# SitaoLuan/ACM-GNN

Hardware: AMD Instinct MI355X
Metric: edges/sec ACM-GCN fwd+bwd on twitch-gamer (higher is better)
Workload: dtype f32; 1 GPU; twitch-gamer-shaped Chung-Lu graph: 168114 nodes, 6797557 undirected edges, nnz(A_low)=13763228, F_in=7, hidden=64, classes=2; 2-layer acmgcnp (variant=0, structure_info=0, attention LayerNorm on), dropout 0.1 (counter-based, masks regenerated in the kernels), AdamW (fused); step = fwd + NLL loss + bwd + optimizer update; parallelism=single-gpu, node_order=degree, launch=hipGraph replay of the captured step (1 consecutive steps per graph), operator_form=pattern-only P + row scale (shared by A_low and A_low^T), full=False, input_pipeline=True, checked=False

## Files before the change

### acm_gnn_amd/_lib.py

```python
import ctypes as C
import os
import threading

from . import build as _build

c_f32p = C.POINTER(C.c_float)
c_i32p = C.POINTER(C.c_int32)

ACM_OK = 0
STATUS_NAMES = {1: "ACM_EINVAL", 2: "ACM_ESHAPE", 3: "ACM_EHIP", 4: "ACM_EUNSUPPORTED", 5: "ACM_ENOMEM"}
ABI_VERSION = 29

EXPORTED_SYMBOLS = (
    "acm_version", "acm_last_error", "acm_tuning_get", "acm_tuning_set", "acm_csr_create", "acm_csr_transpose", "acm_csr_slice_rows",
    "acm_csr_destroy", "acm_csr_info", "acm_csr_build_streams", "acm_csr_build_item_streams", "acm_spmm_workspace_bytes", "acm_gemm_workspace_bytes",
    "acm_gemm", "acm_gemm_blocks", "acm_gemm_drop", "acm_proj3", "acm_gemm_split", "acm_proj_fwd", "acm_proj_fwd_at", "acm_proj_bwd_workspace_bytes", "acm_proj_bwd", "acm_spmm", "acm_spmm_v", "acm_spmm_ex", "acm_cast_bf16", "acm_conv_fwd", "acm_conv_bwd_local_workspace_bytes",
    "acm_conv_bwd_local", "acm_conv_bwd_spmm", "acm_conv_agg_fwd", "acm_conv_agg_bwd_workspace_bytes",
    "acm_conv_agg_bwd", "acm_nll_loss_workspace_bytes", "acm_nll_loss", "acm_adam_step", "acm_dropout",
    "acm_reduce_flush", "acm_conv_fwd_tail_workspace_bytes", "acm_conv_fwd_tail", "acm_shard_plan",
    "acm_conv_acmii_fwd_workspace_bytes", "acm_conv_acmii_fwd", "acm_linear_fwd", "acm_bias_act", "acm_bias_act_bwd_workspace_bytes", "acm_bias_act_bwd",
    "acm_acmii_table_bytes", "acm_acmii_table", "acm_conv_acmii_v_fwd", "acm_conv_acmii_v_bwd_workspace_bytes", "acm_conv_acmii_v_bwd",
    "acm_linear_bwd_workspace_bytes", "acm_linear_bwd", "acm_linear_fwd_add", "acm_linear_bwd_recompute",
    "acm_small_step_workspace_bytes", "acm_small_step", "acm_small_step_has_hidden", "acm_conv_head_fwd", "acm_conv_aggw_fwd", "acm_conv_aggw_bwd_workspace_bytes", "acm_conv_aggw_bwd",
    "acm_eval_metrics_workspace_bytes", "acm_eval_metrics",
    "acm_bce_loss_workspace_bytes", "acm_bce_loss", "acm_rocauc_scores", "acm_rocauc_workspace_bytes", "acm_rocauc",
    "acm_homophily_workspace_bytes", "acm_homophily_census", "acm_class_means_workspace_bytes", "acm_class_means", "acm_class_score",
    "acm_synth_regular", "acm_synth_uniform", "acm_synth_random_plan", "acm_synth_draw", "acm_synth_select_workspace_bytes", "acm_synth_select",
    "acm_synth_inter_count", "acm_synth_emit",
    "acm_gcn_fwd", "acm_gcn_bwd_workspace_bytes", "acm_gcn_bwd", "acm_gemm_act",
    "acm_select_step", "acm_copy_if",
    "acm_small_batch_table_bytes", "acm_small_batch_bind", "acm_small_batch_step", "acm_eval_metrics_batch", "acm_select_step_batch",
    "acm_bnorm_stats_workspace_bytes", "acm_bnorm_stats", "acm_bnorm_fold", "acm_bnorm_param_bwd", "acm_bnorm_bwd_workspace_bytes", "acm_bnorm_bwd",
    "acm_proj_blocks_fwd", "acm_proj_blocks_bwd_workspace_bytes", "acm_proj_blocks_bwd",
    "acm_csr_build_loss_rows", "acm_csr_loss_rows_info", "acm_conv_fwd_tail_rows",
)
LOSS_ROWS_SYMBOLS = ("acm_csr_build_loss_rows", "acm_csr_loss_rows_info", "acm_conv_fwd_tail_rows")


class Dropout(C.Structure):
    _fields_ = [("p", C.c_float), ("tag", C.c_int32), ("seed", C.c_uint64), ("step", C.c_void_p),
                ("row_offset", C.c_int64), ("step_offset", C.c_int64)]


class CsrInfo(C.Structure):
    _fields_ = [("n_rows", C.c_int64), ("n_cols", C.c_int64), ("nnz", C.c_int64),
                ("n_items", C.c_int64), ("n_long_rows", C.c_int64), ("n_partial_slots", C.c_int64),
                ("chunk", C.c_int32), ("max_degree", C.c_int32),
                ("indptr", C.c_void_p), ("indices", C.c_void_p), ("vals", C.c_void_p),
                ("src_pos", C.c_void_p),
                ("stream_steps", C.c_int64), ("stream_slices", C.c_int64),
                ("stream_waves", C.c_int32), ("stream_long_rows", C.c_int32),
                ("item_stream_waves", C.c_int32), ("reserved", C.c_int32), ("item_stream_batches", C.c_int64)]


class ConvFwd(C.Structure):
    _fields_ = [("f_out", C.c_int32), ("n_channels", C.c_int32), ("relu_after", C.c_int32),
                ("relu_mlp", C.c_int32), ("layernorm", C.c_int32), ("scale", C.c_float),
                ("row_offset", C.c_int64),
                ("g_low", C.c_void_p), ("ld_g_low", C.c_int64),
                ("g_high", C.c_void_p), ("ld_g_high", C.c_int64),
                ("g_struc", C.c_void_p), ("ld_g_struc", C.c_int64),
                ("s_high", C.c_void_p), ("ld_s_high", C.c_int64),
                ("s_mlp", C.c_void_p), ("ld_s_mlp", C.c_int64),
                ("s_struc", C.c_void_p), ("ld_s_struc", C.c_int64),
                ("deg", C.c_void_p),
                ("att_vec", C.c_void_p * 4), ("ln_weight", C.c_void_p * 4), ("ln_bias", C.c_void_p * 4),
                ("att_mix", C.c_void_p),
                ("out", C.c_void_p), ("ld_out", C.c_int64),
                ("pre", C.c_void_p), ("ld_pre", C.c_int64),
                ("att", C.c_void_p), ("post_scale", C.c_void_p), ("ld_post_scale", C.c_int64), ("post_relu", C.c_int32),
                ("gather_bf16", C.c_int32), ("row_scale", C.c_void_p), ("post_drop", Dropout)]


class ConvBwdLocal(C.Structure):
    _fields_ = [("f_out", C.c_int32), ("n_channels", C.c_int32), ("relu_after", C.c_int32),
                ("relu_mlp", C.c_int32), ("layernorm", C.c_int32), ("scale", C.c_float),
                ("grad_out", C.c_void_p), ("ld_grad_out", C.c_int64),
                ("pre", C.c_void_p), ("ld_pre", C.c_int64),
                ("s_mlp", C.c_void_p), ("ld_s_mlp", C.c_int64),
                ("deg", C.c_void_p),
                ("att_vec", C.c_void_p * 4), ("ln_weight", C.c_void_p * 4), ("ln_bias", C.c_void_p * 4),
                ("att_mix", C.c_void_p),
                ("g_low", C.c_void_p), ("ld_g_low", C.c_int64),
                ("g_high", C.c_void_p), ("ld_g_high", C.c_int64),
                ("g_mlp", C.c_void_p), ("ld_g_mlp", C.c_int64),
                ("g_struc", C.c_void_p), ("ld_g_struc", C.c_int64),
                ("d_att_vec", C.c_void_p * 4), ("d_ln_weight", C.c_void_p * 4),
                ("d_ln_bias", C.c_void_p * 4), ("d_att_mix", C.c_void_p),
                ("post_scale", C.c_void_p), ("ld_post_scale", C.c_int64), ("post_relu", C.c_int32),
                ("g_scale", C.c_void_p), ("post_drop", Dropout), ("defer", C.c_void_p)]


class ConvBwdSpmm(C.Structure):
    _fields_ = [("f_out", C.c_int32), ("row_offset", C.c_int64),
                ("g_low", C.c_void_p), ("ld_g_low", C.c_int64),
                ("g_high", C.c_void_p), ("ld_g_high", C.c_int64),
                ("g_struc", C.c_void_p), ("ld_g_struc", C.c_int64),
                ("s_high", C.c_void_p), ("ld_s_high", C.c_int64),
                ("s_struc", C.c_void_p), ("ld_s_struc", C.c_int64),
                ("inv_deg", C.c_void_p),
                ("mask_low", C.c_void_p), ("ld_mask_low", C.c_int64),
                ("mask_high", C.c_void_p), ("ld_mask_high", C.c_int64),
                ("dz_low", C.c_void_p), ("ld_dz_low", C.c_int64),
                ("dz_high", C.c_void_p), ("ld_dz_high", C.c_int64),
                ("d_struc", C.c_void_p), ("ld_d_struc", C.c_int64), ("self_scale", C.c_void_p),
                ("gather_bf16", C.c_int32)]


class ConvAggFwd(C.Structure):
    _fields_ = [("f_in", C.c_int32), ("f_pad", C.c_int32), ("f_out", C.c_int32), ("relu_after", C.c_int32),
                ("relu_mlp", C.c_int32), ("layernorm", C.c_int32), ("scale", C.c_float),
                ("xg", C.c_void_p), ("ld_xg", C.c_int64),
                ("xs", C.c_void_p), ("ld_xs", C.c_int64),
                ("w_low", C.c_void_p), ("w_high", C.c_void_p), ("w_mlp", C.c_void_p), ("ld_w", C.c_int64),
                ("att_vec", C.c_void_p * 4), ("ln_weight", C.c_void_p * 4), ("ln_bias", C.c_void_p * 4),
                ("att_mix", C.c_void_p),
                ("out", C.c_void_p), ("ld_out", C.c_int64),
                ("agg", C.c_void_p), ("ld_agg", C.c_int64),
                ("att", C.c_void_p), ("post_scale", C.c_void_p), ("ld_post_scale", C.c_int64), ("post_relu", C.c_int32),
                ("n_channels", C.c_int32), ("sg", C.c_void_p), ("ld_sg", C.c_int64), ("sg_bf16", C.c_int32),
                ("ss", C.c_void_p), ("ld_ss", C.c_int64), ("deg", C.c_void_p),
                ("ps", C.c_void_p), ("ld_ps", C.c_int64), ("row_scale", C.c_void_p), ("post_drop", Dropout),
                ("head_stats", C.c_void_p), ("ld_head_stats", C.c_int64),
                ("next_w_low", C.c_void_p), ("next_w_high", C.c_void_p), ("next_w_mlp", C.c_void_p), ("next_ld_w", C.c_int64),
                ("next_f", C.c_int32), ("next_relu", C.c_int32),
                ("next_zlh", C.c_void_p), ("ld_next_zlh", C.c_int64), ("next_zi", C.c_void_p), ("ld_next_zi", C.c_int64),
                ("agg_given", C.c_int32), ("reserved0", C.c_int32),
                ("agg_copy", C.c_void_p), ("ld_agg_copy", C.c_int64), ("xs_copy", C.c_void_p), ("ld_xs_copy", C.c_int64),
                ("next_x", C.c_void_p), ("ld_next_x", C.c_int64), ("next_drop", Dropout)]


class ConvAggBwd(C.Structure):
    _fields_ = [("f_in", C.c_int32), ("f_pad", C.c_int32), ("f_out", C.c_int32), ("relu_after", C.c_int32),
                ("relu_mlp", C.c_int32), ("layernorm", C.c_int32), ("scale", C.c_float),
                ("grad_out", C.c_void_p), ("ld_grad_out", C.c_int64),
                ("agg", C.c_void_p), ("ld_agg", C.c_int64),
                ("xs", C.c_void_p), ("ld_xs", C.c_int64),
                ("w_low", C.c_void_p), ("w_high", C.c_void_p), ("w_mlp", C.c_void_p), ("ld_w", C.c_int64),
                ("att_vec", C.c_void_p * 4), ("ln_weight", C.c_void_p * 4), ("ln_bias", C.c_void_p * 4),
                ("att_mix", C.c_void_p),
                ("d_params", C.c_void_p), ("post_scale", C.c_void_p), ("ld_post_scale", C.c_int64), ("post_relu", C.c_int32),
                ("n_channels", C.c_int32), ("ps", C.c_void_p), ("ld_ps", C.c_int64),
                ("ss", C.c_void_p), ("ld_ss", C.c_int64), ("deg", C.c_void_p),
                ("g_struc", C.c_void_p), ("ld_g_struc", C.c_int64), ("g_struc_scale", C.c_void_p),
                ("post_drop", Dropout), ("defer", C.c_void_p),
                ("head_stats", C.c_void_p), ("ld_head_stats", C.c_int64),
                ("out", C.c_void_p), ("ld_out", C.c_int64),
                ("next_a", C.c_void_p), ("next_xg", C.c_void_p), ("ld_next_xg", C.c_int64),
                ("next_row_scale", C.c_void_p), ("next_agg", C.c_void_p), ("ld_next_agg", C.c_int64),
                ("proj_dz", C.c_void_p), ("ld_proj_dz", C.c_int64),
                ("proj_w_low", C.c_void_p), ("proj_w_high", C.c_void_p), ("proj_w_mlp", C.c_void_p), ("proj_ld_w", C.c_int64),
                ("proj_f", C.c_int32), ("proj_d_w", C.c_void_p)]


class ConvAcmiiFwd(C.Structure):
    _fields_ = [("f_in", C.c_int32), ("f_pad", C.c_int32), ("f_out", C.c_int32), ("layernorm", C.c_int32),
                ("scale", C.c_float),
                ("xg", C.c_void_p), ("ld_xg", C.c_int64), ("xs", C.c_void_p), ("ld_xs", C.c_int64),
                ("w_low", C.c_void_p), ("w_high", C.c_void_p), ("w_mlp", C.c_void_p), ("ld_w", C.c_int64),
                ("att_vec", C.c_void_p * 4), ("ln_weight", C.c_void_p * 4), ("ln_bias", C.c_void_p * 4),
                ("att_mix", C.c_void_p),
                ("out", C.c_void_p), ("ld_out", C.c_int64), ("pre", C.c_void_p), ("ld_pre", C.c_int64),
                ("att", C.c_void_p), ("zlh", C.c_void_p), ("ld_zlh", C.c_int64), ("zi", C.c_void_p), ("ld_zi", C.c_int64),
                ("post_scale", C.c_void_p), ("ld_post_scale", C.c_int64), ("post_relu", C.c_int32),
                ("row_scale", C.c_void_p), ("post_drop", Dropout),
                ("n_channels", C.c_int32), ("ps", C.c_void_p), ("ld_ps", C.c_int64), ("ss", C.c_void_p), ("ld_ss", C.c_int64),
                ("deg", C.c_void_p)]


class ConvAcmiiBwd(C.Structure):
    _fields_ = [("f_in", C.c_int32), ("table", C.c_void_p),
                ("g_low", C.c_void_p), ("ld_g_low", C.c_int64), ("g_high", C.c_void_p), ("ld_g_high", C.c_int64),
                ("g_mlp", C.c_void_p), ("ld_g_mlp", C.c_int64), ("x", C.c_void_p), ("ld_x", C.c_int64),
                ("self_offset", C.c_int64), ("row_scale", C.c_void_p),
                ("d_w_low", C.c_void_p), ("d_w_high", C.c_void_p), ("d_w_mlp", C.c_void_p), ("ld_dw", C.c_int64),
                ("defer", C.c_void_p)]


class Loss(C.Structure):
    _fields_ = [("n_classes", C.c_int32), ("labels", C.c_void_p), ("row_weight", C.c_void_p),
                ("loss", C.c_void_p), ("dlogits", C.c_void_p), ("ld_dlogits", C.c_int64)]


class ReduceSeg(C.Structure):
    _fields_ = [("partial", C.c_void_p), ("nblk", C.c_int32), ("row_stride", C.c_int32),
                ("q0", C.c_int32), ("len", C.c_int32), ("dst", C.c_void_p),
                ("inner", C.c_int32), ("col_block", C.c_int32),
                ("outer_stride", C.c_int64), ("block_stride", C.c_int64),
                ("elem_stride", C.c_int32), ("reserved", C.c_int32)]


class ReduceList(C.Structure):
    _fields_ = [("n", C.c_int32), ("cap", C.c_int32), ("segs", C.POINTER(ReduceSeg))]


PROJ_BLOCKS_MAX = 8


class ProjBlocks(C.Structure):
    _fields_ = [("n_blocks", C.c_int32), ("f", C.c_int32), ("f_block", C.c_int32), ("f_in", C.c_int32),
                ("w_low", C.c_void_p), ("w_high", C.c_void_p), ("w_mlp", C.c_void_p), ("ldw", C.c_int64),
                ("h", C.c_void_p * PROJ_BLOCKS_MAX), ("ld_h", C.c_int64 * PROJ_BLOCKS_MAX),
                ("width", C.c_int32 * PROJ_BLOCKS_MAX), ("row0", C.c_int32 * PROJ_BLOCKS_MAX),
                ("d_h", C.c_void_p * PROJ_BLOCKS_MAX), ("ld_dh", C.c_int64 * PROJ_BLOCKS_MAX)]


class SpmmOpts(C.Structure):
    _fields_ = [("vals", C.c_void_p), ("row_scale", C.c_void_p), ("sub", C.c_void_p), ("ld_sub", C.c_int64),
                ("sub_scale", C.c_void_p), ("relu", C.c_int32), ("g_bf16", C.c_int32)]


class GcnFwd(C.Structure):
    _fields_ = [("width", C.c_int32), ("relu", C.c_int32), ("z", C.c_void_p), ("ld_z", C.c_int64), ("y", C.c_void_p), ("ld_y", C.c_int64),
                ("row_scale", C.c_void_p), ("drop", Dropout), ("f_next", C.c_int32), ("reserved", C.c_int32),
                ("w_next", C.c_void_p), ("ld_w_next", C.c_int64), ("z_next", C.c_void_p), ("ld_z_next", C.c_int64)]


class GcnBwd(C.Structure):
    _fields_ = [("width", C.c_int32), ("hidden", C.c_int32), ("dy", C.c_void_p), ("ld_dy", C.c_int64), ("h", C.c_void_p), ("ld_h", C.c_int64),
                ("w2", C.c_void_p), ("ld_w2", C.c_int64), ("keep_scale", C.c_float), ("relu", C.c_int32),
                ("g", C.c_void_p), ("ld_g", C.c_int64), ("dz", C.c_void_p), ("ld_dz", C.c_int64),
                ("d_w2", C.c_void_p), ("ld_dw2", C.c_int64), ("defer", C.c_void_p)]


class AdamTensor(C.Structure):
    _fields_ = [("param", C.c_void_p), ("grad", C.c_void_p), ("exp_avg", C.c_void_p), ("exp_avg_sq", C.c_void_p),
                ("step", C.c_void_p), ("numel", C.c_int64)]


class AdamConfig(C.Structure):
    _fields_ = [("lr", C.c_double), ("beta1", C.c_double), ("beta2", C.c_double), ("eps", C.c_double),
                ("weight_decay", C.c_double), ("decoupled", C.c_int32), ("also_advance", C.c_void_p),
                ("arrive", C.c_void_p), ("pending", C.c_void_p)]


class Select(C.Structure):
    _fields_ = [("rule", C.c_int32), ("early_stopping", C.c_int32), ("epochs", C.c_int32), ("reserved", C.c_int32),
                ("result", C.c_void_p), ("result_f64", C.c_void_p), ("train_loss", C.c_void_p),
                ("ctrl", C.c_void_p), ("best", C.c_void_p), ("history", C.c_void_p)]


class EvalMetricsSlot(C.Structure):
    _fields_ = [("logits", C.c_void_p), ("weights", C.c_void_p), ("labels", C.c_void_p), ("out", C.c_void_p),
                ("workspace", C.c_void_p)]


class CopyTensor(C.Structure):
    _fields_ = [("src", C.c_void_p), ("dst", C.c_void_p), ("numel", C.c_int64)]


SMALL_ROLES = 17
SR_W_LOW, SR_W_HIGH, SR_W_MLP, SR_V_LOW, SR_V_HIGH, SR_V_MLP, SR_V_STRUC = range(7)
SR_LNW_LOW, SR_LNW_HIGH, SR_LNW_MLP, SR_LNW_STRUC, SR_LNB_LOW, SR_LNB_HIGH, SR_LNB_MLP, SR_LNB_STRUC, SR_MIX, SR_STRUC = range(7, 17)


class SmallStep(C.Structure):
    _fields_ = [("n_classes", C.c_int32), ("n_channels", C.c_int32), ("relu_before", C.c_int32), ("layernorm", C.c_int32),
                ("scale", C.c_float), ("train", C.c_int32), ("update", C.c_int32), ("hidden", C.c_int32),
                ("t", (AdamTensor * SMALL_ROLES) * 2),
                ("x_vals", C.c_void_p), ("xt_src_pos", C.c_void_p), ("xt_vals", C.c_void_p), ("f_in", C.c_int32), ("reserved1", C.c_int32), ("drop_in", Dropout), ("drop_hidden", Dropout),
                ("row_scale", C.c_void_p), ("labels", C.c_void_p), ("row_weight", C.c_void_p), ("loss", C.c_void_p),
                ("logits", C.c_void_p), ("att1", C.c_void_p), ("att2", C.c_void_p),
                ("lr", C.c_double), ("beta1", C.c_double), ("beta2", C.c_double), ("eps", C.c_double),
                ("weight_decay", C.c_double), ("decoupled", C.c_int32), ("also_advance", C.c_void_p), ("arrive", C.c_void_p),
                ("workspace", C.c_void_p), ("workspace_bytes", C.c_size_t)]


SMALL_BATCH_MAX = 32

_lib = None
_lock = threading.Lock()


def _declare(lib):
    vp, i64, i32, sz = C.c_void_p, C.c_int64, C.c_int, C.c_size_t
    lib.acm_version.restype = C.c_int
    lib.acm_version.argtypes = []
    lib.acm_last_error.restype = C.c_char_p
    lib.acm_last_error.argtypes = []
    lib.acm_csr_create.argtypes = [i64, i64, i64, vp, vp, vp, i32, C.POINTER(vp)]
    lib.acm_csr_transpose.argtypes = [vp, i32, C.POINTER(vp)]
    lib.acm_csr_slice_rows.argtypes = [vp, i64, i64, i32, C.POINTER(vp)]
    lib.acm_csr_destroy.argtypes = [vp]
    lib.acm_csr_destroy.restype = None
    lib.acm_csr_info.argtypes = [vp, C.POINTER(CsrInfo)]
    lib.acm_csr_build_streams.argtypes = [vp, i32, i32]
    lib.acm_csr_build_item_streams.argtypes = [vp, i32]
    lib.acm_shard_plan.argtypes = [i64, vp, i32, i64, vp]
    lib.acm_conv_acmii_fwd_workspace_bytes.argtypes = [vp, C.POINTER(sz)]
    lib.acm_conv_acmii_fwd.argtypes = [vp, C.POINTER(ConvAcmiiFwd), vp, sz, vp]
    lib.acm_acmii_table_bytes.argtypes = [i64, C.POINTER(sz)]
    lib.acm_acmii_table.argtypes = [i64, i32, vp, i64, vp, vp, i64, vp, sz, vp]
    lib.acm_conv_acmii_v_fwd.argtypes = [vp, C.POINTER(ConvAcmiiFwd), vp, vp, sz, vp]
    lib.acm_conv_acmii_v_bwd_workspace_bytes.argtypes = [vp, C.POINTER(sz)]
    lib.acm_conv_acmii_v_bwd.argtypes = [vp, C.POINTER(ConvAcmiiBwd), vp, sz, vp]
    lib.acm_linear_fwd.argtypes = [i64, i64, i64, vp, i64, vp, i64, vp, i32, vp, vp, i64, vp, sz, vp]
    lib.acm_bias_act.argtypes = [i64, i32, vp, i64, vp, i32, vp, vp]
    lib.acm_linear_bwd_workspace_bytes.argtypes = [i64, i32, i32, C.POINTER(sz)]
    lib.acm_linear_bwd.argtypes = [i64, i32, i32, vp, i64, vp, i64, vp, i64, C.c_float, i32, vp, i64, vp, vp, sz, vp, vp]
    lib.acm_linear_fwd_add.argtypes = [i64, i32, i32, vp, i64, vp, i64, vp, i32, vp, vp, i64, vp, i64, vp]
    lib.acm_linear_bwd_recompute.argtypes = [i64, i32, i32, vp, i64, vp, i64, vp, i32, vp, vp, i64, vp, i64, vp, vp, sz, vp, vp]
    lib.acm_bias_act_bwd_workspace_bytes.argtypes = [i64, i32, C.POINTER(sz)]
    lib.acm_bias_act_bwd.argtypes = [i64, i32, vp, i64, vp, i64, C.c_float, i32, vp, i64, vp, vp, sz, vp, vp]
    lib.acm_spmm_workspace_bytes.argtypes = [vp, i32, C.POINTER(sz)]
    lib.acm_gemm_workspace_bytes.argtypes = [i32, i32, i64, i64, i64, C.POINTER(sz)]
    lib.acm_gemm.argtypes = [i32, i32, i64, i64, i64, vp, i64, vp, i64, vp, i64, i32, vp, sz, vp]
    lib.acm_proj_bwd_workspace_bytes.argtypes = [i64, i64, i32, C.POINTER(sz)]
    lib.acm_proj_fwd.argtypes = [i64, i64, i32, vp, i64, vp, vp, vp, i64, i32, vp, i64, vp, i64, vp]
    lib.acm_proj_fwd_at.argtypes = [i64, i64, i32, vp, i64, vp, vp, vp, i64, i32, vp, i64, i64, vp, i64, vp]
    lib.acm_proj_bwd.argtypes = [i64, i64, i32, vp, i64, vp, i64, vp, vp, vp, i64, vp, i64, vp, i64, i64, i64, vp, sz, vp, vp]
    lib.acm_proj_blocks_fwd.argtypes = [i64, C.POINTER(ProjBlocks), vp, i64, i32, i32, vp]
    lib.acm_proj_blocks_bwd_workspace_bytes.argtypes = [i64, C.POINTER(ProjBlocks), C.POINTER(sz)]
    lib.acm_proj_blocks_bwd.argtypes = [i64, C.POINTER(ProjBlocks), vp, i64, vp, i64, i64, i64, vp, sz, vp, vp]
    lib.acm_gemm_split.argtypes = [i32, i32, i64, i64, i64, vp, i64, vp, i64, vp, i64, i64, vp, i64, i32, vp, sz, vp]
    lib.acm_gemm_blocks.argtypes = [i32, i32, i64, i64, i64, vp, i64, vp, i64, vp, i64, i64, i64, i32, vp, sz, vp]
    lib.acm_gemm_drop.argtypes = [i32, i32, i64, i64, i64, vp, i64, vp, i64, vp, i64, i64, i64, i32, C.POINTER(Dropout), vp, sz, vp]
    lib.acm_proj3.argtypes = [i64, i64, vp, i64, vp, vp, vp, i64, i64, i64, vp, i64, i64, vp, i64, i32, C.POINTER(Dropout), vp]
    lib.acm_spmm.argtypes = [vp, vp, i64, i32, vp, i64, vp, sz, vp]
    lib.acm_spmm_v.argtypes = [vp, vp, vp, i64, i32, vp, i64, i32, vp, sz, vp]
    lib.acm_adam_step.argtypes = [i32, vp, vp, vp]
    lib.acm_dropout.argtypes = [i64, i64, vp, i64, vp, i64, i64, vp, vp]
    lib.acm_spmm_ex.argtypes = [vp, vp, i64, i32, vp, i64, vp, vp, sz, vp]
    lib.acm_cast_bf16.argtypes = [i64, i64, vp, i64, vp, i64, vp]
    lib.acm_conv_fwd.argtypes = [vp, C.POINTER(ConvFwd), vp, sz, vp]
    lib.acm_conv_head_fwd.argtypes = [i64, C.POINTER(ConvFwd), vp]
    lib.acm_conv_aggw_bwd_workspace_bytes.argtypes = [i64, i64, C.POINTER(C.c_size_t)]
    lib.acm_conv_aggw_bwd.argtypes = [i64, i64, i64, vp, i64, vp, i64, C.POINTER(ConvBwdLocal), vp, vp, vp, i64, vp, C.c_size_t, vp]
    lib.acm_conv_aggw_fwd.argtypes = [i64, i64, i64, vp, i64, vp, i64, vp, vp, vp, i64, vp, i64, C.POINTER(ConvFwd), vp]
    lib.acm_conv_bwd_local_workspace_bytes.argtypes = [i64, i32, i32, C.POINTER(sz)]
    lib.acm_conv_bwd_local.argtypes = [i64, C.POINTER(ConvBwdLocal), vp, sz, vp]
    lib.acm_conv_bwd_spmm.argtypes = [vp, C.POINTER(ConvBwdSpmm), vp, sz, vp]
    lib.acm_conv_agg_fwd.argtypes = [vp, C.POINTER(ConvAggFwd), vp, sz, vp]
    lib.acm_conv_agg_bwd_workspace_bytes.argtypes = [i64, i32, i32, C.POINTER(sz)]
    lib.acm_conv_agg_bwd.argtypes = [i64, C.POINTER(ConvAggBwd), vp, sz, vp]
    lib.acm_nll_loss_workspace_bytes.argtypes = [i64, C.POINTER(sz)]
    lib.acm_nll_loss.argtypes = [i64, i32, vp, i64, vp, vp, vp, vp, i64, vp, sz, vp, vp]
    lib.acm_eval_metrics_workspace_bytes.argtypes = [i64, i32, C.POINTER(sz)]
    lib.acm_eval_metrics.argtypes = [i64, i32, vp, i64, vp, vp, i64, i32, i32, vp, vp, sz, vp]
    lib.acm_bce_loss_workspace_bytes.argtypes = [i64, C.POINTER(sz)]
    lib.acm_bce_loss.argtypes = [i64, i32, vp, i64, vp, vp, vp, vp, i64, vp, sz, vp, vp]
    lib.acm_rocauc_scores.argtypes = [i64, i32, vp, i64, vp, vp]
    lib.acm_rocauc_workspace_bytes.argtypes = [i64, i32, C.POINTER(sz)]
    lib.acm_rocauc.argtypes = [i64, vp, vp, vp, vp, i64, i32, vp, vp, vp, sz, vp]
    lib.acm_homophily_workspace_bytes.argtypes = [i64, i64, i32, C.POINTER(sz)]
    lib.acm_homophily_census.argtypes = [vp, vp, i64, i32, vp, vp, vp, vp, vp, sz, vp]
    lib.acm_class_means_workspace_bytes.argtypes = [i64, i32, i32, C.POINTER(sz)]
    lib.acm_class_means.argtypes = [i64, i32, i32, vp, i64, vp, vp, i64, vp, vp, sz, vp]
    lib.acm_class_score.argtypes = [i64, i32, i32, vp, i64, vp, i64, vp, vp, vp, vp, vp]
    u64 = C.c_uint64
    lib.acm_synth_regular.argtypes = [i32, i64, i64, i64, u64, u64, i64, i64, vp, vp]
    lib.acm_synth_uniform.argtypes = [i64, i64, u64, u64, i64, vp, i64, vp]
    lib.acm_synth_random_plan.argtypes = [i32, i64, i64, C.c_double, C.POINTER(C.c_int64)]
    lib.acm_synth_draw.argtypes = [i32, i64, i64, i32, i32, u64, u64, i64, vp, vp]
    lib.acm_synth_select_workspace_bytes.argtypes = [i32, i64, C.POINTER(sz)]
    lib.acm_synth_select.argtypes = [i32, i64, vp, vp, vp, vp, i64, vp, vp, vp, vp, sz, vp]
    lib.acm_synth_inter_count.argtypes = [i32, i32, C.c_double, vp, vp, vp]
    lib.acm_synth_emit.argtypes = [i32, i32, i64, i32, i32, vp, vp, i64, vp, vp, vp]
    lib.acm_gcn_fwd.argtypes = [vp, C.POINTER(GcnFwd), vp, sz, vp]
    lib.acm_gcn_bwd_workspace_bytes.argtypes = [vp, i32, i32, C.POINTER(sz)]
    lib.acm_gcn_bwd.argtypes = [vp, C.POINTER(GcnBwd), vp, sz, vp]
    lib.acm_gemm_act.argtypes = [i64, i64, i64, vp, i64, vp, i64, i32, vp, vp, i64, vp, sz, vp]
    lib.acm_select_step.argtypes = [C.POINTER(Select), vp]
    lib.acm_copy_if.argtypes = [i32, vp, vp, vp]
    lib.acm_bnorm_stats_workspace_bytes.argtypes = [i64, i32, C.POINTER(sz)]
    lib.acm_bnorm_stats.argtypes = [i64, i32, vp, i64, vp, vp, C.c_float, C.c_float, i32, vp, vp, vp, vp, vp, sz, vp]
    lib.acm_bnorm_fold.argtypes = [i32, i32, vp, i64, vp, vp, vp, i64, vp, vp]
    lib.acm_bnorm_param_bwd.argtypes = [i32, i32, vp, i64, vp, vp, i64, vp, vp, i64, vp, vp, vp]
    lib.acm_bnorm_bwd_workspace_bytes.argtypes = [i64, i32, C.POINTER(sz)]
    lib.acm_bnorm_bwd.argtypes = [i64, i32, vp, i64, vp, i64, vp, vp, vp, C.c_float, i32, vp, i64, vp, vp, sz, vp, vp]
    lib.acm_reduce_flush.argtypes = [vp, vp]
    lib.acm_conv_fwd_tail_workspace_bytes.argtypes = [i64, i32, i32, C.POINTER(sz)]
    lib.acm_conv_fwd_tail.argtypes = [vp, C.POINTER(ConvFwd), C.POINTER(Loss), C.POINTER(ConvBwdLocal), vp, sz, vp, sz, vp]
    lib.acm_csr_build_loss_rows.argtypes = [vp, vp]
    lib.acm_csr_loss_rows_info.argtypes = [vp, C.POINTER(C.c_int64)]
    lib.acm_conv_fwd_tail_rows.argtypes = lib.acm_conv_fwd_tail.argtypes
    lib.acm_small_step_workspace_bytes.argtypes = [vp, vp, vp, C.POINTER(sz)]
    lib.acm_small_step.argtypes = [vp, vp, vp, C.POINTER(SmallStep), vp]
    lib.acm_small_step_has_hidden.argtypes = [i32]
    lib.acm_small_batch_table_bytes.argtypes = [i32, C.POINTER(sz)]
    lib.acm_small_batch_bind.argtypes = [vp, vp, vp, i32, C.POINTER(C.POINTER(SmallStep)), vp, sz, vp]
    lib.acm_small_batch_step.argtypes = [vp, vp, vp, i32, C.POINTER(SmallStep), vp, vp]
    lib.acm_eval_metrics_batch.argtypes = [i64, i32, i64, i64, i32, i32, i32, vp, sz, vp]
    lib.acm_select_step_batch.argtypes = [i32, vp, vp]
    for name in EXPORTED_SYMBOLS:
        fn = getattr(lib, name)
        if name not in ("acm_version", "acm_last_error", "acm_csr_destroy"):
            fn.restype = C.c_int


def library_path():
    return os.environ.get("ACM_HIP_LIBRARY", _build.LIB_PATH)


def load(build_if_missing=True):
    global _lib
    with _lock:
        if _lib is not None:
            return _lib
        path = library_path()
        if "ACM_HIP_LIBRARY" not in os.environ and build_if_missing:
            try:
                if _build.is_stale():
                    _build.build_library()
            except Exception as exc:
                if not os.path.exists(path):
                    raise RuntimeError(f"libacm_hip.so is not built and cannot be built here: {exc}")
        if not os.path.exists(path):
            raise RuntimeError(f"libacm_hip.so not found at {path}; run `python -m acm_gnn_amd.build`")
        lib = C.CDLL(path)
        _declare(lib)
        ver = lib.acm_version()
        if ver != ABI_VERSION:
            raise RuntimeError(f"libacm_hip.so ABI version {ver} != expected {ABI_VERSION}")
        _lib = lib
        return _lib


def check(status, what=""):
    if status != ACM_OK:
        msg = load().acm_last_error().decode(errors="replace")
        raise RuntimeError(f"{what or 'libacm_hip'} failed with {STATUS_NAMES.get(status, status)}: {msg}")
```

### acm_gnn_amd/csrc/acm_common.h

```cpp
#pragma once

#include <hip/hip_runtime.h>
#include <math.h>
#include <stdint.h>

#include "acm_dispatch.h"
#include "acm_hip.h"
#include "acm_items.h"

#define ACM_WAVE 64
#define ACM_NXCD 8
#define ACM_MIN_CHUNK 128
#define ACM_MAX_CHUNK 1024
#define ACM_GROUPS_IN_FLIGHT 8192
#define ACM_LN_EPS 1e-5f

void acm_set_error(const char* fmt, ...);
const acm_tuning_t& acm_tuning();
#define ACM_ROWS16_EPI 1
#define ACM_ROWS16_BWD 2
#define ACM_ROWS16_LOCAL 4
#define ACM_GEMM_ROWS 1
#define ACM_GEMM_BX3 2
#define ACM_GEMM_BX3_WIDE 4
#define ACM_GEMM_ROWS_ALWAYS 8

#define ACM_CHECK_HIP(expr)                                                            \
    do {                                                                               \
        hipError_t e__ = (expr);                                                       \
        if (e__ != hipSuccess) {                                                       \
            acm_set_error("%s -> %s (%s:%d)", #expr, hipGetErrorString(e__), __FILE__, \
                          __LINE__);                                                   \
            return ACM_EHIP;                                                           \
        }                                                                              \
    } while (0)

#define ACM_REQUIRE(cond, code, ...)    \
    do {                                \
        if (!(cond)) {                  \
            acm_set_error(__VA_ARGS__); \
            return (code);              \
        }                               \
    } while (0)

#define ACM_STREAM_SENTINEL 0x07FFFFFF
#define ACM_STREAM_PAD_STEPS 8
struct AcmStreams {
    int32_t* ids;
    int32_t* waves;
    int32_t* items;
    AcmLongRow* long_rows;
    int32_t* long_index;
    int32_t* counters;
    float* slots;
    int64_t total_steps, n_slices, n_long, n_slots;
    int32_t n_waves, lmax;
};

#define ACM_ITEM_STREAM_PAD 8
struct AcmItemStreams {
    int32_t* ids;
    int32_t* quads;
    int32_t* waves;
    int64_t total_batches, n_quads;
    int32_t n_waves;
};

struct AcmLossRows {
    AcmItem* items;
    AcmLongRow* long_rows;
    int32_t* long_index;
    int64_t n_items, n_long, n_slots, n_windows, n_multi;
    uint8_t* keep;
    int64_t kept_rows, kept_edges;
};

struct acm_csr {
    int64_t n_rows, n_cols, nnz;
    int32_t chunk, max_degree;
    int32_t* indptr;
    int32_t* indices;
    float* vals;
    int32_t* src_pos;
    AcmItem* items;
    int64_t n_items;
    AcmLongRow* long_rows;
    int32_t* long_index;
    int64_t n_long;
    int64_t n_slots;
    int64_t n_windows;
    int64_t n_multi;
    AcmStreams* streams;
    AcmItemStreams* item_streams;
    AcmLossRows* loss_rows;
    int device;
};

struct StreamView {
    const int32_t* ids;
    const int32_t* waves;
    const int32_t* items;
    const AcmLongRow* long_rows;
    const int32_t* long_index;
    int32_t* counters;
    float* slots;
    unsigned ids_bytes, slots_bytes;
    int n_waves;
};

struct CsrView {
    const AcmItem* items;
    int n_items;
    const AcmLongRow* long_rows;
    const int32_t* long_index;
    int n_long;
    int n_windows;
    int n_multi;
    const int32_t* indices;
    const float* vals;
};

struct GatherOverride {
    CsrView view;
    int64_t n_slots;
};

int acm_reduce_emit(acm_reduce_list_t* defer, const acm_reduce_seg_t* segs, int n, hipStream_t st);
int acm_reduce_check_segment(const acm_reduce_seg_t& sg, int index);

int acm_spmm_internal(const acm_csr* a, const void* G, int64_t ldg, int width, float* Y, int64_t ldy,
                      const acm_spmm_opts_t* o, void* workspace, size_t workspace_bytes, acm_stream_t stream,
                      bool* defer_fixup);
int acm_bwd_local_reduce(const acm_conv_bwd_local_t* p, const float* partial, int nblk, hipStream_t st);
int acm_bwd_local16(const acm_conv_bwd_local_t* p, int64_t n_rows, float* partial, int max_blocks, hipStream_t s);
int acm_agg_epi16(const acm_conv_agg_fwd_t* p, int64_t n_rows, bool* next_done, hipStream_t s);
struct GatherRole;
int acm_agg_bwd16(const acm_conv_agg_bwd_t* p, int64_t n_rows, float* partial, int max_blocks, hipStream_t s, const GatherRole* gr,
                  int gather_blocks);
int acm_acmii_fixup_launch(const acm_csr_t* a, const acm_conv_acmii_fwd_t* p, const float* partial, hipStream_t s);
bool acm_gemm_rows_nn_ok(int64_t M, int64_t N, int64_t K, const float* B, int64_t ldb);
int acm_gemm_rows_nn(int64_t M, int64_t N, int64_t K, const float* A, int64_t lda, const float* B, int64_t ldb, float* C,
                     int64_t ldc, int relu, const acm_dropout_t* drop, hipStream_t st);
bool acm_gemm_rows_tn_ok(int64_t n_rows, int64_t K, int64_t N);
int acm_gemm_rows_tn_blocks(int64_t n_rows);
int acm_gemm_rows_tn(int64_t n_rows, int64_t K, int64_t N, const float* X, int64_t ldx, const float* Dz, int64_t lddz,
                     float* slabs, int blocks, const acm_dropout_t* drop, hipStream_t st);
bool acm_gemm_bx3_nn_ok(int64_t M, int64_t N, int64_t K, const float* A, int64_t lda);
int acm_gemm_bx3_nn(int64_t M, int64_t N, int64_t K, const float* A, int64_t lda, const float* B, int64_t ldb, float* C,
                    int64_t ldc, int relu, const acm_dropout_t* drop, hipStream_t st);
bool acm_gemm_bx3_tn_ok(int64_t n_rows, int64_t K, int64_t N);
int acm_gemm_bx3_tn_blocks(int64_t n_rows, int64_t K);
int acm_gemm_bx3_tn(int64_t n_rows, int64_t K, int64_t N, const float* X, int64_t ldx, const float* Dz, int64_t lddz,
                    float* slabs, int blocks, const acm_dropout_t* drop, hipStream_t st);
int acm_linear_fwd_narrow(int64_t n_rows, int64_t f_in, int64_t f_out, const float* X, int64_t ldx, const float* W, int64_t ldw,
                          const float* bias, int relu, const acm_dropout_t* drop, float* Y, int64_t ldy, hipStream_t s,
                          const float* add, int64_t ld_add);

static inline CsrView acm_view(const acm_csr* a) {
    CsrView v;
    v.items = a->items;
    v.n_items = (int)a->n_items;
    v.long_rows = a->long_rows;
    v.long_index = a->long_index;
    v.n_long = (int)a->n_long;
    v.n_windows = (int)a->n_windows;
    v.n_multi = (int)a->n_multi;
    v.indices = a->indices;
    v.vals = a->vals;
    return v;
}

#ifdef __HIPCC__
template <int CTRL>
__device__ __forceinline__ float acm_dpp(float v) {
    return __int_as_float(__builtin_amdgcn_update_dpp(0, __float_as_int(v), CTRL, 0xf, 0xf, false));
}
typedef unsigned acm_u32x2 __attribute__((ext_vector_type(2)));
template <int W>
__device__ __forceinline__ float acm_group_sum(float v) {
    static_assert(W == 1 || W == 2 || W == 4 || W == 8 || W == 16 || W == 32 || W == 64, "group width");
    if (W >= 2) v += acm_dpp<0xB1>(v);
    if (W >= 4) v += acm_dpp<0x4E>(v);
    if (W >= 8) v += acm_dpp<0x141>(v);
    if (W >= 16) v += acm_dpp<0x140>(v);
    if (W >= 32) {
        const acm_u32x2 r = __builtin_amdgcn_permlane16_swap(__float_as_uint(v), __float_as_uint(v), false, false);
        v = __uint_as_float(r[0]) + __uint_as_float(r[1]);
    }
    if (W >= 64) {
        const acm_u32x2 r = __builtin_amdgcn_permlane32_swap(__float_as_uint(v), __float_as_uint(v), false, false);
        v = __uint_as_float(r[0]) + __uint_as_float(r[1]);
    }
    return v;
}

__device__ __forceinline__ float acm_cross_row_sum(float v) {
    acm_u32x2 r = __builtin_amdgcn_permlane16_swap(__float_as_uint(v), __float_as_uint(v), false, false);
    v = __uint_as_float(r[0]) + __uint_as_float(r[1]);
    r = __builtin_amdgcn_permlane32_swap(__float_as_uint(v), __float_as_uint(v), false, false);
    return __uint_as_float(r[0]) + __uint_as_float(r[1]);
}

__device__ __forceinline__ int acm_row_bcast(int v, int u) {
#define ACM_BC(U) case U: return __builtin_amdgcn_update_dpp(0, v, 0x150 + U, 0xf, 0xf, false)
    switch (u & 15) {
        ACM_BC(0); ACM_BC(1); ACM_BC(2); ACM_BC(3); ACM_BC(4); ACM_BC(5); ACM_BC(6); ACM_BC(7);
        ACM_BC(8); ACM_BC(9); ACM_BC(10); ACM_BC(11); ACM_BC(12); ACM_BC(13); ACM_BC(14);
        default: return __builtin_amdgcn_update_dpp(0, v, 0x15F, 0xf, 0xf, false);
    }
#undef ACM_BC
}

__device__ __forceinline__ int acm_uniform(int v) { return __builtin_amdgcn_readfirstlane(v); }
__device__ __forceinline__ float acm_lane_f(float v, int lane) {
    return __int_as_float(__builtin_amdgcn_readlane(__float_as_int(v), lane));
}

__device__ __forceinline__ float acm_nll_row(int C, const float* zi, int yi, float wi, float* di) {
    if (wi == 0.f) {
        for (int c = 0; c < C; ++c) di[c] = 0.f;
        return 0.f;
    }
    float m = -INFINITY;
    for (int c = 0; c < C; ++c) m = fmaxf(m, zi[c]);
    float s = 0.f;
    for (int c = 0; c < C; ++c) s += expf(zi[c] - m);
    const float lse = m + logf(s);
    const float inv = 1.0f / s;
    const float zy = zi[yi];
    for (int c = 0; c < C; ++c) di[c] = wi * (expf(zi[c] - m) * inv - (c == yi ? 1.f : 0.f));
    return wi * (lse - zy);
}

__device__ __forceinline__ float acm_bce_row(int C, const float* zi, int64_t yi, float wi, float* di) {
    if (wi == 0.f) {
        if (di)
            for (int c = 0; c < C; ++c) di[c] = 0.f;
        return 0.f;
    }
    const float s = wi / (float)C;
    float acc = 0.f;
    for (int c = 0; c < C; ++c) {
        const float z = zi[c];
        const bool hit = (int64_t)c == yi;
        const float e = expf(-fabsf(z));
        acc += fmaxf(z, 0.f) - (hit ? z : 0.f) + log1pf(e);
        if (di) {
            const float r = 1.0f / (1.0f + e);
            const float sig = z >= 0.f ? r : e * r;
            di[c] = s * (sig - (hit ? 1.f : 0.f));
        }
    }
    return s * acc;
}

struct AcmDropCtx {
    unsigned k0, k1, c2, c3, thresh, tag16;
    float inv_keep;
    long row_offset;
    bool on;
};

__device__ __forceinline__ AcmDropCtx acm_drop_ctx(const acm_dropout_t& d) {
    AcmDropCtx c;
    c.on = d.p > 0.f;
    const unsigned long long step = c.on ? (unsigned long long)(d.step[0] + d.step_offset) : 0ull;
    c.k0 = (unsigned)d.seed;
    c.k1 = (unsigned)(d.seed >> 32);
    c.c2 = (unsigned)step;
    c.c3 = (unsigned)(step >> 32);
    const double t = (double)d.p * 4294967296.0;
    c.thresh = t >= 4294967295.0 ? 0xFFFFFFFFu : (unsigned)t;
    c.tag16 = ((unsigned)d.tag) << 16;
    c.inv_keep = 1.0f / (1.0f - d.p);
    c.row_offset = (long)d.row_offset;
    return c;
}

__device__ __forceinline__ void acm_philox7(const AcmDropCtx& c, long row, int block, unsigned (&w)[4]) {
    unsigned x0 = (unsigned)(row + c.row_offset), x1 = (unsigned)block | c.tag16, x2 = c.c2, x3 = c.c3;
    unsigned k0 = c.k0, k1 = c.k1;
#pragma unroll
    for (int r = 0; r < 7; ++r) {
        const unsigned long long q0 = (unsigned long long)0xD2511F53u * x0, q1 = (unsigned long long)0xCD9E8D57u * x2;
        const unsigned hi0 = (unsigned)(q0 >> 32), lo0 = (unsigned)q0;
        const unsigned hi1 = (unsigned)(q1 >> 32), lo1 = (unsigned)q1;
        x0 = hi1 ^ x1 ^ k0;
        x1 = lo1;
        x2 = hi0 ^ x3 ^ k1;
        x3 = lo0;
        k0 += 0x9E3779B9u;
        k1 += 0xBB67AE85u;
    }
    w[0] = x0, w[1] = x1, w[2] = x2, w[3] = x3;
}

__device__ __forceinline__ float acm_drop1(const AcmDropCtx& c, long row, int col) {
    if (!c.on) return 1.f;
    unsigned w[4];
    acm_philox7(c, row, (col & 15) + 16 * (col >> 6), w);
    const int q = (col >> 4) & 3;
    const unsigned v = q == 0 ? w[0] : (q == 1 ? w[1] : (q == 2 ? w[2] : w[3]));
    return v >= c.thresh ? c.inv_keep : 0.f;
}

__device__ __forceinline__ void acm_drop4(const AcmDropCtx& c, long row, int m, float (&f)[4]) {
    if (!c.on) {
        f[0] = f[1] = f[2] = f[3] = 1.f;
        return;
    }
    unsigned w[4];
    acm_philox7(c, row, m, w);
#pragma unroll
    for (int i = 0; i < 4; ++i) f[i] = w[i] >= c.thresh ? c.inv_keep : 0.f;
}

#endif
```

### acm_gnn_amd/csrc/acm_csr.cpp

```cpp
#include <stdarg.h>
#include <stdio.h>
#include <string.h>

#include <stdlib.h>

#include <algorithm>
#include <functional>
#include <new>
#include <queue>
#include <string>
#include <utility>
#include <vector>

#include "acm_common.h"

static thread_local char g_err[512] = "";

void acm_set_error(const char* fmt, ...) {
    va_list ap;
    va_start(ap, fmt);
    vsnprintf(g_err, sizeof(g_err), fmt, ap);
    va_end(ap);
}

extern "C" int acm_version(void) { return ACM_ABI_VERSION; }
extern "C" const char* acm_last_error(void) { return g_err; }

namespace {
const acm_tuning_t kTuningDefaults = {0, 0, -1, 7, 1, 7, {0}};
struct TuningField { const char* name; int32_t acm_tuning_t::*field; };
const TuningField kTuningFields[] = {{"chunk", &acm_tuning_t::chunk},           {"wide_form", &acm_tuning_t::wide_form},
                                     {"bwd_split", &acm_tuning_t::bwd_split},   {"rows16", &acm_tuning_t::rows16},
                                     {"agg_fused", &acm_tuning_t::agg_fused},   {"gemm_forms", &acm_tuning_t::gemm_forms}};
const char* const kHostKeys[] = {"rewrites", "implicit", "relabel", "pipeline", "csr_features", "small_step", "mlp_stack", "loss_rows"};

const char* tuning_invalid(const acm_tuning_t& t) {
    if (t.chunk != 0 && (t.chunk < 8 || t.chunk > 4096 || (t.chunk & (t.chunk - 1)))) return "chunk";
    if (t.wide_form < 0 || t.wide_form > 3) return "wide_form";
    if (t.bwd_split < -1 || t.bwd_split > 1) return "bwd_split";
    if (t.rows16 < 0 || t.rows16 > 7) return "rows16";
    if (t.agg_fused < 0 || t.agg_fused > 1) return "agg_fused";
    if (t.gemm_forms < 0 || t.gemm_forms > 15) return "gemm_forms";
    return nullptr;
}

acm_tuning_t tuning_from_environment() {
    acm_tuning_t t = kTuningDefaults;
    const char* env = getenv("ACM_TUNING");
    if (!env) return t;
    std::string text(env);
    size_t pos = 0;
    while (pos < text.size()) {
        size_t end = text.find(',', pos);
        if (end == std::string::npos) end = text.size();
        const std::string item = text.substr(pos, end - pos);
        pos = end + 1;
        if (item.empty()) continue;
        const size_t eq = item.find('=');
        const std::string key = item.substr(0, eq), val = eq == std::string::npos ? "" : item.substr(eq + 1);
        bool known = false;
        for (const char* h : kHostKeys) known = known || key == h;
        for (const TuningField& f : kTuningFields) {
            if (key != f.name) continue;
            known = true;
            char* stop = nullptr;
            const long v = strtol(val.c_str(), &stop, 0);
            acm_tuning_t probe = t;
            probe.*(f.field) = (int32_t)v;
            if (val.empty() || *stop || tuning_invalid(probe)) fprintf(stderr, "libacm_hip: ACM_TUNING: bad value '%s' ignored\n", item.c_str());
            else t = probe;
        }
        if (!known) fprintf(stderr, "libacm_hip: ACM_TUNING: unknown key '%s' ignored\n", key.c_str());
    }
    return t;
}
const acm_tuning_t g_tuning_loaded = tuning_from_environment();
acm_tuning_t g_tuning = g_tuning_loaded;
}

const acm_tuning_t& acm_tuning() { return g_tuning; }

extern "C" int acm_tuning_get(acm_tuning_t* out) {
    ACM_REQUIRE(out, ACM_EINVAL, "acm_tuning_get: NULL argument");
    *out = g_tuning;
    return ACM_OK;
}

extern "C" int acm_tuning_set(const acm_tuning_t* in) {
    if (!in) {
        g_tuning = g_tuning_loaded;
        return ACM_OK;
    }
    const char* bad = tuning_invalid(*in);
    ACM_REQUIRE(!bad, ACM_EINVAL, "acm_tuning_set: field '%s' out of range", bad);
    g_tuning = *in;
    for (int32_t& r : g_tuning.reserved) r = 0;
    return ACM_OK;
}

namespace {

void free_streams(AcmStreams* t) {
    if (!t) return;
    for (void* q : {(void*)t->ids, (void*)t->waves, (void*)t->items, (void*)t->long_rows,
                    (void*)t->long_index, (void*)t->counters, (void*)t->slots})
        if (q) (void)hipFree(q);
    delete t;
}

void free_item_streams(AcmItemStreams* t) {
    if (!t) return;
    for (void* q : {(void*)t->ids, (void*)t->quads, (void*)t->waves})
        if (q) (void)hipFree(q);
    delete t;
}

void free_loss_rows(AcmLossRows* t) {
    if (!t) return;
    for (void* q : {(void*)t->items, (void*)t->long_rows, (void*)t->long_index, (void*)t->keep})
        if (q) (void)hipFree(q);
    delete t;
}

void free_handle(acm_csr* a) {
    if (!a) return;
    free_loss_rows(a->loss_rows);
    if (a->indptr) (void)hipFree(a->indptr);
    if (a->indices) (void)hipFree(a->indices);
    if (a->vals) (void)hipFree(a->vals);
    if (a->long_index) (void)hipFree(a->long_index);
    if (a->src_pos) (void)hipFree(a->src_pos);
    if (a->items) (void)hipFree(a->items);
    if (a->long_rows) (void)hipFree(a->long_rows);
    free_streams(a->streams);
    free_item_streams(a->item_streams);
    delete a;
}


int finish_handle(acm_csr* a, const std::vector<int32_t>& h_indptr, int chunk) {
    const int env_chunk = acm_tuning().chunk;
    int auto_chunk = ACM_MIN_CHUNK;
    while (auto_chunk < ACM_MAX_CHUNK && 2 * (int64_t)auto_chunk <= a->nnz / ACM_GROUPS_IN_FLIGHT) auto_chunk *= 2;
    a->chunk = chunk > 0 ? chunk : (env_chunk > 0 ? env_chunk : auto_chunk);
    std::vector<AcmItem> items;
    std::vector<AcmLongRow> longs;
    build_items(h_indptr, a->chunk, items, longs, a->n_slots, a->max_degree, a->n_windows, a->n_multi);
    a->n_items = (int64_t)items.size();
    a->n_long = (int64_t)longs.size();
    if (a->n_items) {
        ACM_CHECK_HIP(hipMalloc((void**)&a->items, items.size() * sizeof(AcmItem)));
        ACM_CHECK_HIP(hipMemcpy(a->items, items.data(), items.size() * sizeof(AcmItem),
                                hipMemcpyHostToDevice));
    }
    if (a->n_long) {
        ACM_CHECK_HIP(hipMalloc((void**)&a->long_rows, longs.size() * sizeof(AcmLongRow)));
        ACM_CHECK_HIP(hipMemcpy(a->long_rows, longs.data(), longs.size() * sizeof(AcmLongRow),
                                hipMemcpyHostToDevice));
        std::vector<int32_t> index((size_t)a->n_rows, -1);
        for (size_t i = 0; i < longs.size(); ++i) index[(size_t)longs[i].row] = (int32_t)i;
        ACM_CHECK_HIP(hipMalloc((void**)&a->long_index, index.size() * sizeof(int32_t)));
        ACM_CHECK_HIP(hipMemcpy(a->long_index, index.data(), index.size() * sizeof(int32_t), hipMemcpyHostToDevice));
    }
    return ACM_OK;
}

acm_csr* new_handle(int64_t n_rows, int64_t n_cols, int64_t nnz) {
    acm_csr* a = new (std::nothrow) acm_csr();
    if (!a) return nullptr;
    memset(a, 0, sizeof(*a));
    a->n_rows = n_rows;
    a->n_cols = n_cols;
    a->nnz = nnz;
    (void)hipGetDevice(&a->device);
    return a;
}

int alloc_arrays(acm_csr* a, bool with_vals = true) {
    ACM_CHECK_HIP(hipMalloc((void**)&a->indptr, (size_t)(a->n_rows + 1) * sizeof(int32_t)));
    const size_t m = (size_t)std::max<int64_t>(a->nnz, 1);
    ACM_CHECK_HIP(hipMalloc((void**)&a->indices, m * sizeof(int32_t)));
    if (with_vals) ACM_CHECK_HIP(hipMalloc((void**)&a->vals, m * sizeof(float)));
    return ACM_OK;
}

}

extern "C" int acm_csr_create(int64_t n_rows, int64_t n_cols, int64_t nnz,
                              const int32_t* indptr_dev, const int32_t* indices_dev,
                              const float* vals_dev, int chunk, acm_csr_t** out) {
    ACM_REQUIRE(out, ACM_EINVAL, "acm_csr_create: out is NULL");
    *out = nullptr;
    ACM_REQUIRE(indptr_dev, ACM_EINVAL, "acm_csr_create: indptr is NULL");
    ACM_REQUIRE(nnz == 0 || indices_dev, ACM_EINVAL, "acm_csr_create: indices NULL with nnz > 0");
    ACM_REQUIRE(n_rows >= 0 && n_cols >= 0 && nnz >= 0, ACM_ESHAPE, "acm_csr_create: negative size");
    ACM_REQUIRE(n_rows < INT32_MAX && n_cols < INT32_MAX && nnz < INT32_MAX, ACM_EUNSUPPORTED,
                "acm_csr_create: sizes must fit int32 (rows %lld cols %lld nnz %lld)",
                (long long)n_rows, (long long)n_cols, (long long)nnz);
    ACM_CHECK_HIP(hipDeviceSynchronize());
    std::vector<int32_t> h_indptr((size_t)n_rows + 1);
    ACM_CHECK_HIP(hipMemcpy(h_indptr.data(), indptr_dev, h_indptr.size() * sizeof(int32_t),
                            hipMemcpyDeviceToHost));
    ACM_REQUIRE(h_indptr[0] == 0 && h_indptr[n_rows] == nnz, ACM_ESHAPE,
                "acm_csr_create: indptr[0]=%d indptr[n]=%d but nnz=%lld", h_indptr[0],
                h_indptr[n_rows], (long long)nnz);
    for (int64_t r = 0; r < n_rows; ++r)
        ACM_REQUIRE(h_indptr[r] <= h_indptr[r + 1], ACM_ESHAPE,
                    "acm_csr_create: indptr not monotone at row %lld", (long long)r);
    if (nnz) {
        std::vector<int32_t> h_idx((size_t)nnz);
        ACM_CHECK_HIP(hipMemcpy(h_idx.data(), indices_dev, (size_t)nnz * sizeof(int32_t),
                                hipMemcpyDeviceToHost));
        for (int64_t k = 0; k < nnz; ++k)
            ACM_REQUIRE(h_idx[k] >= 0 && h_idx[k] < n_cols, ACM_ESHAPE,
                        "acm_csr_create: column id %d out of range at position %lld", h_idx[k],
                        (long long)k);
    }
    acm_csr* a = new_handle(n_rows, n_cols, nnz);
    ACM_REQUIRE(a, ACM_ENOMEM, "acm_csr_create: host allocation failed");
    int st = alloc_arrays(a, vals_dev != nullptr);
    if (st == ACM_OK) {
        hipError_t e = hipMemcpy(a->indptr, indptr_dev, (size_t)(n_rows + 1) * sizeof(int32_t),
                                 hipMemcpyDeviceToDevice);
        if (e == hipSuccess && nnz)
            e = hipMemcpy(a->indices, indices_dev, (size_t)nnz * sizeof(int32_t),
                          hipMemcpyDeviceToDevice);
        if (e == hipSuccess && nnz && vals_dev)
            e = hipMemcpy(a->vals, vals_dev, (size_t)nnz * sizeof(float), hipMemcpyDeviceToDevice);
        if (e != hipSuccess) {
            acm_set_error("acm_csr_create: device copy failed: %s", hipGetErrorString(e));
            st = ACM_EHIP;
        }
    }
    if (st == ACM_OK) st = finish_handle(a, h_indptr, chunk);
    if (st != ACM_OK) {
        free_handle(a);
        return st;
    }
    *out = a;
    return ACM_OK;
}

extern "C" int acm_csr_transpose(const acm_csr_t* a, int chunk, acm_csr_t** out) {
    ACM_REQUIRE(a && out, ACM_EINVAL, "acm_csr_transpose: NULL argument");
    *out = nullptr;
    ACM_CHECK_HIP(hipDeviceSynchronize());
    const int64_t n = a->n_rows, m = a->n_cols, nnz = a->nnz;
    std::vector<int32_t> ip((size_t)n + 1), ix((size_t)nnz);
    std::vector<float> v((size_t)nnz);
    ACM_CHECK_HIP(hipMemcpy(ip.data(), a->indptr, ip.size() * sizeof(int32_t), hipMemcpyDeviceToHost));
    if (nnz) {
        ACM_CHECK_HIP(hipMemcpy(ix.data(), a->indices, (size_t)nnz * sizeof(int32_t), hipMemcpyDeviceToHost));
        if (a->vals) ACM_CHECK_HIP(hipMemcpy(v.data(), a->vals, (size_t)nnz * sizeof(float), hipMemcpyDeviceToHost));
    }
    std::vector<int32_t> tp((size_t)m + 1, 0), tx((size_t)nnz), tpos((size_t)nnz);
    std::vector<float> tv((size_t)nnz);
    for (int64_t k = 0; k < nnz; ++k) ++tp[(size_t)ix[k] + 1];
    for (int64_t c = 0; c < m; ++c) tp[c + 1] += tp[c];
    std::vector<int32_t> cur(tp.begin(), tp.end() - 1);
    for (int64_t r = 0; r < n; ++r)
        for (int32_t k = ip[r]; k < ip[r + 1]; ++k) {
            const int32_t pos = cur[ix[k]]++;
            tx[pos] = (int32_t)r;
            tv[pos] = v[k];
            tpos[pos] = k;
        }
    acm_csr* t = new_handle(m, n, nnz);
    ACM_REQUIRE(t, ACM_ENOMEM, "acm_csr_transpose: host allocation failed");
    int st = alloc_arrays(t, a->vals != nullptr);
    if (st == ACM_OK) {
        hipError_t e = hipMemcpy(t->indptr, tp.data(), tp.size() * sizeof(int32_t), hipMemcpyHostToDevice);
        if (e == hipSuccess && nnz)
            e = hipMemcpy(t->indices, tx.data(), (size_t)nnz * sizeof(int32_t), hipMemcpyHostToDevice);
        if (e == hipSuccess && nnz && t->vals)
            e = hipMemcpy(t->vals, tv.data(), (size_t)nnz * sizeof(float), hipMemcpyHostToDevice);
        if (e == hipSuccess) e = hipMalloc((void**)&t->src_pos, (size_t)(nnz > 0 ? nnz : 1) * sizeof(int32_t));
        if (e == hipSuccess && nnz)
            e = hipMemcpy(t->src_pos, tpos.data(), (size_t)nnz * sizeof(int32_t), hipMemcpyHostToDevice);
        if (e != hipSuccess) {
            acm_set_error("acm_csr_transpose: upload failed: %s", hipGetErrorString(e));
            st = ACM_EHIP;
        }
    }
    if (st == ACM_OK) st = finish_handle(t, tp, chunk);
    if (st != ACM_OK) {
        free_handle(t);
        return st;
    }
    *out = t;
    return ACM_OK;
}

extern "C" int acm_csr_slice_rows(const acm_csr_t* a, int64_t row_begin, int64_t row_end, int chunk,
                                  acm_csr_t** out) {
    ACM_REQUIRE(a && out, ACM_EINVAL, "acm_csr_slice_rows: NULL argument");
    *out = nullptr;
    ACM_REQUIRE(0 <= row_begin && row_begin <= row_end && row_end <= a->n_rows, ACM_ESHAPE,
                "acm_csr_slice_rows: bad range [%lld,%lld) of %lld rows", (long long)row_begin,
                (long long)row_end, (long long)a->n_rows);
    ACM_CHECK_HIP(hipDeviceSynchronize());
    const int64_t n = row_end - row_begin;
    std::vector<int32_t> ip((size_t)n + 1);
    ACM_CHECK_HIP(hipMemcpy(ip.data(), a->indptr + row_begin, ip.size() * sizeof(int32_t),
                            hipMemcpyDeviceToHost));
    const int32_t base = ip[0];
    for (auto& x : ip) x -= base;
    const int64_t nnz = ip[n];
    acm_csr* s = new_handle(n, a->n_cols, nnz);
    ACM_REQUIRE(s, ACM_ENOMEM, "acm_csr_slice_rows: host allocation failed");
    int st = alloc_arrays(s, a->vals != nullptr);
    if (st == ACM_OK) {
        hipError_t e = hipMemcpy(s->indptr, ip.data(), ip.size() * sizeof(int32_t), hipMemcpyHostToDevice);
        if (e == hipSuccess && nnz)
            e = hipMemcpy(s->indices, a->indices + base, (size_t)nnz * sizeof(int32_t), hipMemcpyDeviceToDevice);
        if (e == hipSuccess && nnz && a->vals)
            e = hipMemcpy(s->vals, a->vals + base, (size_t)nnz * sizeof(float), hipMemcpyDeviceToDevice);
        if (e != hipSuccess) {
            acm_set_error("acm_csr_slice_rows: copy failed: %s", hipGetErrorString(e));
            st = ACM_EHIP;
        }
    }
    if (st == ACM_OK) st = finish_handle(s, ip, chunk);
    if (st != ACM_OK) {
        free_handle(s);
        return st;
    }
    *out = s;
    return ACM_OK;
}

extern "C" void acm_csr_destroy(acm_csr_t* a) { free_handle(a); }

extern "C" int acm_shard_plan(int64_t n_rows, const int64_t* indptr, int world, int64_t row_cost, int64_t* bounds) {
    ACM_REQUIRE(indptr && bounds, ACM_EINVAL, "acm_shard_plan: NULL argument");
    ACM_REQUIRE(n_rows >= 0 && world >= 1 && row_cost >= 0, ACM_ESHAPE, "acm_shard_plan: n_rows %lld world %d row_cost %lld",
                (long long)n_rows, world, (long long)row_cost);
    ACM_REQUIRE(indptr[0] == 0, ACM_EINVAL, "acm_shard_plan: indptr[0] must be 0");
    auto cost = [&](int64_t r) { return (__int128)indptr[r] + (__int128)row_cost * r; };
    const __int128 total = cost(n_rows);
    bounds[0] = 0;
    for (int p = 1; p < world; ++p) {
        const __int128 target = total * p / world;
        int64_t lo = bounds[p - 1], hi = n_rows;
        while (lo < hi) {
            const int64_t mid = lo + (hi - lo) / 2;
            if (cost(mid) >= target) hi = mid; else lo = mid + 1;
        }
        int64_t r = lo;
        if (r > bounds[p - 1] && target - cost(r - 1) < cost(r) - target) --r;
        bounds[p] = r;
    }
    bounds[world] = n_rows;
    return ACM_OK;
}


namespace {

template <class T>
int upload(T** dev, const std::vector<T>& host, size_t min_elems = 1) {
    const size_t n = std::max(host.size(), min_elems);
    ACM_CHECK_HIP(hipMalloc((void**)dev, n * sizeof(T)));
    if (!host.empty()) ACM_CHECK_HIP(hipMemcpy(*dev, host.data(), host.size() * sizeof(T), hipMemcpyHostToDevice));
    return ACM_OK;
}

}

extern "C" int acm_csr_build_streams(acm_csr_t* a, int n_waves, int lmax) {
    ACM_REQUIRE(a, ACM_EINVAL, "acm_csr_build_streams: NULL handle");
    if (a->streams) return ACM_OK;
    ACM_REQUIRE(a->vals == nullptr, ACM_EUNSUPPORTED, "acm_csr_build_streams: pattern-only operators only");
    ACM_REQUIRE(a->n_cols < ACM_STREAM_SENTINEL, ACM_EUNSUPPORTED, "acm_csr_build_streams: %lld columns", (long long)a->n_cols);
    if (lmax <= 0) lmax = 512;
    ACM_REQUIRE(lmax % 32 == 0 && lmax <= 4096, ACM_EINVAL, "acm_csr_build_streams: lmax %d must be a multiple of 32, at most 4096", lmax);
    ACM_CHECK_HIP(hipDeviceSynchronize());
    const int64_t n = a->n_rows, nnz = a->nnz;
    std::vector<int32_t> ip((size_t)n + 1), ix((size_t)nnz);
    ACM_CHECK_HIP(hipMemcpy(ip.data(), a->indptr, ip.size() * sizeof(int32_t), hipMemcpyDeviceToHost));
    if (nnz) ACM_CHECK_HIP(hipMemcpy(ix.data(), a->indices, (size_t)nnz * sizeof(int32_t), hipMemcpyDeviceToHost));
    struct Item { int32_t row, begin, len, slot; };
    std::vector<Item> items;
    items.reserve((size_t)n + (size_t)(nnz / lmax) + 16);
    std::vector<AcmLongRow> longs;
    int64_t n_slots = 0;
    for (int64_t r = 0; r < n; ++r) {
        const int32_t b = ip[r], deg = ip[r + 1] - ip[r];
        if (deg <= lmax) {
            items.push_back({(int32_t)r, b, deg, -1});
            continue;
        }
        const int32_t pieces = (deg + lmax - 1) / lmax;
        const int32_t per = (((deg + pieces - 1) / pieces) + 31) / 32 * 32;
        AcmLongRow lr = {(int32_t)r, (int32_t)n_slots, 0, 0};
        for (int32_t q = 0; q * per < deg; ++q) items.push_back({(int32_t)r, b + q * per, std::min(per, deg - q * per), (int32_t)n_slots++});
        lr.slot_end = (int32_t)n_slots;
        longs.push_back(lr);
    }
    std::stable_sort(items.begin(), items.end(), [](const Item& x, const Item& y) { return x.len > y.len; });
    const int64_t n_items = (int64_t)items.size(), n_slices = (n_items + 3) / 4;
    std::vector<int32_t> sl_steps((size_t)n_slices);
    int64_t total_steps = 0;
    for (int64_t s = 0; s < n_slices; ++s) {
        int32_t longest = 0;
        for (int64_t i = s * 4; i < std::min(n_items, s * 4 + 4); ++i) longest = std::max(longest, items[(size_t)i].len);
        sl_steps[(size_t)s] = std::max(1, (longest + 31) / 32);
        total_steps += sl_steps[(size_t)s];
    }
    ACM_REQUIRE((total_steps + ACM_STREAM_PAD_STEPS) * 512 < (int64_t)0xFFFFFFF0u, ACM_EUNSUPPORTED,
                "acm_csr_build_streams: %lld steps exceed 32-bit stream offsets", (long long)total_steps);
    if (n_waves <= 0) {
        int cus = 256;
        (void)hipDeviceGetAttribute(&cus, hipDeviceAttributeMultiprocessorCount, a->device);
        n_waves = cus * 4 * 5;
    }
    if ((int64_t)n_waves > n_slices) n_waves = (int)std::max<int64_t>(n_slices, 1);
    n_waves = (n_waves + 3) / 4 * 4;
    const int64_t epi_cost = 1;
    std::vector<int32_t> wave_of((size_t)n_slices);
    {
        typedef std::pair<int64_t, int32_t> Load;
        std::priority_queue<Load, std::vector<Load>, std::greater<Load>> heap;
        for (int32_t w = 0; w < n_waves; ++w) heap.push({0, w});
        for (int64_t s = 0; s < n_slices; ++s) {
            Load l = heap.top();
            heap.pop();
            wave_of[(size_t)s] = l.second;
            l.first += 4 * (int64_t)sl_steps[(size_t)s] + epi_cost;
            heap.push(l);
        }
    }
    std::vector<int32_t> count((size_t)n_waves + 1, 0);
    for (int64_t s = 0; s < n_slices; ++s) ++count[(size_t)wave_of[(size_t)s] + 1];
    for (int32_t w = 0; w < n_waves; ++w) count[(size_t)w + 1] += count[(size_t)w];
    std::vector<int32_t> pos_of((size_t)n_slices), cur(count.begin(), count.end() - 1);
    for (int64_t s = 0; s < n_slices; ++s) pos_of[(size_t)s] = cur[(size_t)wave_of[(size_t)s]]++;
    {
        {
            std::vector<int32_t> slice_at((size_t)n_slices);
            for (int64_t s = 0; s < n_slices; ++s) slice_at[(size_t)pos_of[(size_t)s]] = (int32_t)s;
            for (int32_t w = 0; w < n_waves; ++w) {
                const int32_t b = count[(size_t)w], m = count[(size_t)w + 1] - b;
                uint64_t state = 0x9E3779B97F4A7C15ull * (uint64_t)(w + 1);
                for (int32_t i = m - 1; i > 0; --i) {
                    state = state * 6364136223846793005ull + 1442695040888963407ull;
                    const int32_t j = (int32_t)((state >> 33) % (uint64_t)(i + 1));
                    std::swap(slice_at[(size_t)(b + i)], slice_at[(size_t)(b + j)]);
                }
            }
            for (int64_t q = 0; q < n_slices; ++q) pos_of[(size_t)slice_at[(size_t)q]] = (int32_t)q;
        }
    }
    std::vector<int32_t> h_steps((size_t)n_slices + 2, 1), h_items(((size_t)n_slices + 2) * 16, -1), step_base((size_t)n_slices + 1, 0);
    for (int64_t s = 0; s < n_slices; ++s) h_steps[(size_t)pos_of[(size_t)s]] = sl_steps[(size_t)s];
    for (int64_t q = 0; q < n_slices; ++q) step_base[(size_t)q + 1] = step_base[(size_t)q] + h_steps[(size_t)q];
    std::vector<int32_t> h_waves((size_t)n_waves * 4);
    for (int32_t w = 0; w < n_waves; ++w) {
        const int32_t b = count[(size_t)w], e = count[(size_t)w + 1];
        h_waves[(size_t)w * 4 + 0] = b;
        h_waves[(size_t)w * 4 + 1] = e;
        h_waves[(size_t)w * 4 + 2] = step_base[(size_t)b];
        h_waves[(size_t)w * 4 + 3] = step_base[(size_t)e] - step_base[(size_t)b];
    }
    std::vector<int32_t> h_ids(((size_t)total_steps + ACM_STREAM_PAD_STEPS) * 128, ACM_STREAM_SENTINEL);
    for (int64_t s = 0; s < n_slices; ++s) {
        const size_t q = (size_t)pos_of[(size_t)s];
        for (int g = 0; g < 4; ++g) {
            const int64_t i = s * 4 + g;
            if (i >= n_items) break;
            const Item& it = items[(size_t)i];
            h_items[q * 16 + 4 * g + 0] = it.row;
            h_items[q * 16 + 4 * g + 1] = it.slot;
            int32_t* dst = h_ids.data() + (size_t)step_base[q] * 128 + (size_t)g * 32;
            for (int32_t k = 0; k < it.len; ++k) dst[(size_t)(k >> 5) * 128 + (k & 31)] = ix[(size_t)it.begin + k];
        }
    }
    for (size_t q = 0; q < (size_t)n_slices + 2; ++q)
        for (int g = 0; g < 4; ++g) h_items[q * 16 + 4 * g + 2] = h_steps[q], h_items[q * 16 + 4 * g + 3] = 0;
    AcmStreams* t = new (std::nothrow) AcmStreams();
    ACM_REQUIRE(t, ACM_ENOMEM, "acm_csr_build_streams: host allocation failed");
    memset(t, 0, sizeof(*t));
    t->total_steps = total_steps;
    t->n_slices = n_slices;
    t->n_long = (int64_t)longs.size();
    t->n_slots = n_slots;
    t->n_waves = n_waves;
    t->lmax = lmax;
    int st = upload(&t->ids, h_ids);
    if (st == ACM_OK) st = upload(&t->waves, h_waves);
    if (st == ACM_OK) st = upload(&t->items, h_items);
    if (st == ACM_OK && !longs.empty()) {
        st = upload(&t->long_rows, longs);
        std::vector<int32_t> index((size_t)n, -1);
        for (size_t i = 0; i < longs.size(); ++i) index[(size_t)longs[i].row] = (int32_t)i;
        if (st == ACM_OK) st = upload(&t->long_index, index);
        if (st == ACM_OK && hipMalloc((void**)&t->counters, longs.size() * sizeof(int32_t)) != hipSuccess) st = ACM_EHIP;
        if (st == ACM_OK && hipMemset(t->counters, 0, longs.size() * sizeof(int32_t)) != hipSuccess) st = ACM_EHIP;
        if (st == ACM_OK && hipMalloc((void**)&t->slots, (size_t)n_slots * 8 * sizeof(float)) != hipSuccess) st = ACM_EHIP;
        if (st == ACM_EHIP) acm_set_error("acm_csr_build_streams: device allocation failed");
    }
    if (st != ACM_OK) {
        free_streams(t);
        return st;
    }
    a->streams = t;
    return ACM_OK;
}

extern "C" int acm_csr_build_item_streams(acm_csr_t* a, int n_waves) {
    ACM_REQUIRE(a, ACM_EINVAL, "acm_csr_build_item_streams: NULL handle");
    if (a->item_streams) return ACM_OK;
    ACM_REQUIRE(a->vals == nullptr, ACM_EUNSUPPORTED, "acm_csr_build_item_streams: pattern-only operators only");
    ACM_REQUIRE(a->n_items > 0 && a->nnz > 0, ACM_EUNSUPPORTED, "acm_csr_build_item_streams: empty operator");
    ACM_REQUIRE(a->n_cols < ((int64_t)1 << 31) - 1, ACM_EUNSUPPORTED, "acm_csr_build_item_streams: %lld columns", (long long)a->n_cols);
    ACM_CHECK_HIP(hipDeviceSynchronize());
    const int64_t n_items = a->n_items, nnz = a->nnz;
    std::vector<AcmItem> items((size_t)n_items);
    std::vector<AcmLongRow> longs((size_t)a->n_long);
    std::vector<int32_t> ix((size_t)nnz), lidx;
    ACM_CHECK_HIP(hipMemcpy(items.data(), a->items, items.size() * sizeof(AcmItem), hipMemcpyDeviceToHost));
    ACM_CHECK_HIP(hipMemcpy(ix.data(), a->indices, ix.size() * sizeof(int32_t), hipMemcpyDeviceToHost));
    if (a->n_long) {
        ACM_REQUIRE(a->long_index, ACM_EUNSUPPORTED, "acm_csr_build_item_streams: handle without a long-row index");
        lidx.resize((size_t)a->n_rows);
        ACM_CHECK_HIP(hipMemcpy(longs.data(), a->long_rows, longs.size() * sizeof(AcmLongRow), hipMemcpyDeviceToHost));
        ACM_CHECK_HIP(hipMemcpy(lidx.data(), a->long_index, lidx.size() * sizeof(int32_t), hipMemcpyDeviceToHost));
    }
    const int64_t n_quads = (n_items + 3) / 4;
    std::vector<int32_t> qb((size_t)n_quads, 0);
    int64_t total = 0;
    for (int64_t i = 0; i < n_items; ++i) {
        const int32_t nb = (items[(size_t)i].end - items[(size_t)i].begin + 31) / 32;
        qb[(size_t)(i / 4)] += nb;
        total += nb;
    }
    ACM_REQUIRE((total + ACM_ITEM_STREAM_PAD) * 128 < ((int64_t)1 << 32), ACM_EUNSUPPORTED,
                "acm_csr_build_item_streams: %lld batches exceed 32-bit stream offsets", (long long)total);
    if (n_waves <= 0) {
        int cus = 256;
        (void)hipDeviceGetAttribute(&cus, hipDeviceAttributeMultiprocessorCount, a->device);
        n_waves = cus * 8;
    }
    if ((int64_t)n_waves > n_quads) n_waves = (int)n_quads;
    n_waves = (n_waves + 3) / 4 * 4;
    const int64_t quad_cost = 10;
    std::vector<int32_t> order((size_t)n_quads), wave_of((size_t)n_quads);
    for (int64_t q = 0; q < n_quads; ++q) order[(size_t)q] = (int32_t)q;
    std::stable_sort(order.begin(), order.end(), [&](int32_t x, int32_t y) { return qb[(size_t)x] > qb[(size_t)y]; });
    {
        typedef std::pair<int64_t, int32_t> Load;
        std::priority_queue<Load, std::vector<Load>, std::greater<Load>> heap;
        for (int32_t w = 0; w < n_waves; ++w) heap.push({0, w});
        for (int64_t o = 0; o < n_quads; ++o) {
            Load l = heap.top();
            heap.pop();
            wave_of[(size_t)order[(size_t)o]] = l.second;
            l.first += qb[(size_t)order[(size_t)o]] + quad_cost;
            heap.push(l);
        }
    }
    std::vector<int32_t> count((size_t)n_waves + 1, 0);
    for (int64_t q = 0; q < n_quads; ++q) ++count[(size_t)wave_of[(size_t)q] + 1];
    for (int32_t w = 0; w < n_waves; ++w) count[(size_t)w + 1] += count[(size_t)w];
    std::vector<int32_t> cur(count.begin(), count.end() - 1), quad_at((size_t)n_quads);
    for (int64_t o = 0; o < n_quads; ++o) quad_at[(size_t)cur[(size_t)wave_of[(size_t)order[(size_t)o]]]++] = order[(size_t)o];
    const int32_t zero_row = (int32_t)a->n_cols;
    std::vector<int32_t> h_quads((size_t)n_quads * 16, 0), h_waves((size_t)n_waves * 4, 0),
        h_ids(((size_t)total + ACM_ITEM_STREAM_PAD) * 32, zero_row);
    int64_t batch = 0;
    for (int32_t w = 0; w < n_waves; ++w) {
        h_waves[(size_t)w * 4 + 0] = count[(size_t)w];
        h_waves[(size_t)w * 4 + 1] = count[(size_t)w + 1];
        h_waves[(size_t)w * 4 + 2] = (int32_t)batch;
        for (int32_t pos = count[(size_t)w]; pos < count[(size_t)w + 1]; ++pos) {
            const int64_t q = quad_at[(size_t)pos];
            for (int g = 0; g < 4; ++g) {
                int32_t* d = h_quads.data() + (size_t)pos * 16 + 4 * g;
                const int64_t i = q * 4 + g;
                d[1] = -1;
                if (i >= n_items) continue;
                const AcmItem& it = items[(size_t)i];
                const int32_t len = it.end - it.begin, nb = (len + 31) / 32;
                bool owner = it.slot < 0;
                if (!owner) owner = longs[(size_t)lidx[(size_t)it.row]].slot_begin == it.slot;
                d[0] = it.row, d[1] = it.slot, d[2] = nb, d[3] = 1 | (owner ? 2 : 0);
                for (int32_t k = 0; k < len; ++k) h_ids[(size_t)batch * 32 + (size_t)k] = ix[(size_t)it.begin + (size_t)k];
                batch += nb;
            }
        }
        h_waves[(size_t)w * 4 + 3] = (int32_t)batch - h_waves[(size_t)w * 4 + 2];
    }
    AcmItemStreams* t = new (std::nothrow) AcmItemStreams();
    ACM_REQUIRE(t, ACM_ENOMEM, "acm_csr_build_item_streams: host allocation failed");
    memset(t, 0, sizeof(*t));
    t->total_batches = total;
    t->n_quads = n_quads;
    t->n_waves = n_waves;
    int st = upload(&t->ids, h_ids);
    if (st == ACM_OK) st = upload(&t->quads, h_quads);
    if (st == ACM_OK) st = upload(&t->waves, h_waves);
    if (st != ACM_OK) {
        free_item_streams(t);
        return st;
    }
    a->item_streams = t;
    return ACM_OK;
}

extern "C" int acm_csr_build_loss_rows(acm_csr_t* a, const uint8_t* keep_dev) {
    ACM_REQUIRE(a && keep_dev, ACM_EINVAL, "acm_csr_build_loss_rows: NULL argument");
    ACM_REQUIRE(a->n_rows == a->n_cols, ACM_EUNSUPPORTED, "acm_csr_build_loss_rows: a square operator (%lld x %lld)",
                (long long)a->n_rows, (long long)a->n_cols);
    ACM_CHECK_HIP(hipDeviceSynchronize());
    const int64_t n = a->n_rows;
    std::vector<int32_t> ip((size_t)n + 1);
    std::vector<uint8_t> keep((size_t)std::max<int64_t>(n, 1), 0);
    ACM_CHECK_HIP(hipMemcpy(ip.data(), a->indptr, ip.size() * sizeof(int32_t), hipMemcpyDeviceToHost));
    if (n) ACM_CHECK_HIP(hipMemcpy(keep.data(), keep_dev, (size_t)n, hipMemcpyDeviceToHost));
    AcmLossRowsHost h;
    acm_loss_rows_host(ip, keep.data(), a->chunk, h);
    AcmLossRows* t = new (std::nothrow) AcmLossRows();
    ACM_REQUIRE(t, ACM_ENOMEM, "acm_csr_build_loss_rows: host allocation failed");
    memset(t, 0, sizeof(*t));
    t->n_items = (int64_t)h.items.size();
    t->n_long = (int64_t)h.longs.size();
    t->n_slots = h.n_slots;
    t->n_windows = h.n_windows;
    t->n_multi = h.n_multi;
    t->kept_rows = h.kept_rows;
    t->kept_edges = h.kept_edges;
    int st = upload(&t->keep, keep);
    if (st == ACM_OK) st = upload(&t->items, h.items);
    if (st == ACM_OK && !h.longs.empty()) st = upload(&t->long_rows, h.longs);
    if (st == ACM_OK && !h.longs.empty()) st = upload(&t->long_index, h.long_index);
    if (st != ACM_OK) {
        free_loss_rows(t);
        return st;
    }
    free_loss_rows(a->loss_rows);
    a->loss_rows = t;
    return ACM_OK;
}

extern "C" int acm_csr_loss_rows_info(const acm_csr_t* a, int64_t* out) {
    ACM_REQUIRE(a && out, ACM_EINVAL, "acm_csr_loss_rows_info: NULL argument");
    const AcmLossRows* t = a->loss_rows;
    out[0] = t ? t->kept_rows : 0;
    out[1] = t ? t->n_items : 0;
    out[2] = t ? t->n_slots : 0;
    out[3] = t ? t->kept_edges : 0;
    return ACM_OK;
}

extern "C" int acm_csr_info(const acm_csr_t* a, acm_csr_info_t* info) {
    ACM_REQUIRE(a && info, ACM_EINVAL, "acm_csr_info: NULL argument");
    info->n_rows = a->n_rows;
    info->n_cols = a->n_cols;
    info->nnz = a->nnz;
    info->n_items = a->n_items;
    info->n_long_rows = a->n_long;
    info->n_partial_slots = a->n_slots;
    info->chunk = a->chunk;
    info->max_degree = a->max_degree;
    info->indptr = a->indptr;
    info->indices = a->indices;
    info->vals = a->vals;
    info->src_pos = a->src_pos;
    info->stream_steps = a->streams ? a->streams->total_steps : 0;
    info->stream_slices = a->streams ? a->streams->n_slices : 0;
    info->stream_waves = a->streams ? a->streams->n_waves : 0;
    info->stream_long_rows = a->streams ? (int32_t)a->streams->n_long : 0;
    info->item_stream_waves = a->item_streams ? a->item_streams->n_waves : 0;
    info->reserved = 0;
    info->item_stream_batches = a->item_streams ? a->item_streams->total_batches : 0;
    return ACM_OK;
}

extern "C" int acm_spmm_workspace_bytes(const acm_csr_t* a, int width, size_t* bytes) {
    ACM_REQUIRE(a && bytes, ACM_EINVAL, "acm_spmm_workspace_bytes: NULL argument");
    ACM_REQUIRE(width > 0, ACM_ESHAPE, "acm_spmm_workspace_bytes: width must be positive");
    *bytes = (size_t)a->n_slots * (size_t)width * sizeof(float);
    return ACM_OK;
}
```

### acm_gnn_amd/csrc/acm_gather_device.h

```cpp
#pragma once
#include <type_traits>

#include "acm_conv_device.h"

template <class L>
struct Owns {
    static __device__ __forceinline__ bool lane_stores(const L&) { return true; }
};
template <int FP>
struct Owns<LaySerial<FP>> {
    static __device__ __forceinline__ bool lane_stores(const LaySerial<FP>& l) { return l.lead; }
};
template <>
struct Owns<LayPair32> {
    static __device__ __forceinline__ bool lane_stores(const LayPair32& l) { return l.lane < 32; }
};
template <int NB>
struct Owns<LayVec16<NB>> {
    static __device__ __forceinline__ bool lane_stores(const LayVec16<NB>& l) { return l.lane < 16; }
};

template <bool BF16>
__device__ __forceinline__ float load_gathered(const float* rowp_f32_units, long row_elems, int col) {
    if (BF16) {
        const unsigned short* p = reinterpret_cast<const unsigned short*>(rowp_f32_units) + row_elems + col;
        return __uint_as_float(((unsigned)*p) << 16);
    }
    return rowp_f32_units[row_elems + col];
}

template <int NREG, int NG, int UNR, bool BF16>
__device__ __forceinline__ void gather_wide(const GatherSrc& g, int F, const int32_t* __restrict__ indices,
                                            const float* __restrict__ vals, int begin, int end,
                                            int lane, float (&acc)[NG][NREG]) {
    for (int base = begin; base < end; base += 64) {
        const int kk = base + lane;
        int my_j = 0;
        float my_a = 0.f;
        if (kk < end) {
            my_j = indices[kk];
            my_a = vals ? vals[kk] : 1.f;
        }
        const int cnt = min(64, end - base);
        int t = 0;
        for (; t + UNR <= cnt; t += UNR) {
            float z[UNR][NG][NREG];
            float a[UNR];
#pragma unroll
            for (int u = 0; u < UNR; ++u) {
                const int j = __builtin_amdgcn_readlane(my_j, t + u);
                a[u] = acm_lane_f(my_a, t + u);
#pragma unroll
                for (int c = 0; c < NG; ++c) {
                    const long roff = (long)j * g.ld[c];
#pragma unroll
                    for (int r = 0; r < NREG; ++r) {
                        const int col = lane + 64 * r;
                        z[u][c][r] = (col < F) ? load_gathered<BF16>(g.p[c], roff, col) : 0.f;
                    }
                }
            }
#pragma unroll
            for (int u = 0; u < UNR; ++u)
#pragma unroll
                for (int c = 0; c < NG; ++c)
#pragma unroll
                    for (int r = 0; r < NREG; ++r) acc[c][r] = fmaf(a[u], z[u][c][r], acc[c][r]);
        }
        for (; t < cnt; ++t) {
            const int j = __builtin_amdgcn_readlane(my_j, t);
            const float a = acm_lane_f(my_a, t);
#pragma unroll
            for (int c = 0; c < NG; ++c) {
                const long roff = (long)j * g.ld[c];
#pragma unroll
                for (int r = 0; r < NREG; ++r) {
                    const int col = lane + 64 * r;
                    const float z = (col < F) ? load_gathered<BF16>(g.p[c], roff, col) : 0.f;
                    acc[c][r] = fmaf(a, z, acc[c][r]);
                }
            }
        }
    }
}

template <int NREG, int NG, class Epi, bool BF16 = false>
__global__ __launch_bounds__(256) void spmm_wide_kernel(CsrView csr, GatherSrc g, int F,
                                                        typename Epi::Args ea, float* __restrict__ partial) {
    const int lane = threadIdx.x & 63;
    const int w = acm_uniform(blockIdx.x * 4 + (threadIdx.x >> 6));
    if (w >= csr.n_items) return;
    const AcmItem it = csr.items[w];
    const int row = acm_uniform(it.row), begin = acm_uniform(it.begin), end = acm_uniform(it.end),
              slot = acm_uniform(it.slot);
    float acc[NG][NREG];
#pragma unroll
    for (int c = 0; c < NG; ++c)
#pragma unroll
        for (int r = 0; r < NREG; ++r) acc[c][r] = 0.f;
    constexpr int UNR = (NG * NREG >= 8) ? 2 : (NG * NREG >= 4 ? 4 : 8);
    gather_wide<NREG, NG, UNR, BF16>(g, F, csr.indices, csr.vals, begin, end, lane, acc);
    if (slot < 0) {
        LayWide<NREG> lay{lane};
        Epi::template apply<LayWide<NREG>, NG>(ea, row, lay, F, acc);
    } else {
        float* ps = partial + (long)slot * (NG * F);
#pragma unroll
        for (int c = 0; c < NG; ++c)
#pragma unroll
            for (int r = 0; r < NREG; ++r) {
                const int col = lane + 64 * r;
                if (col < F) ps[c * F + col] = acc[c][r];
            }
    }
}

template <int NG, class Epi, bool BF16>
__global__ __launch_bounds__(256) void spmm_pair_kernel(CsrView csr, GatherSrc g, int F, typename Epi::Args ea,
                                                        float* __restrict__ partial) {
    const int lane = threadIdx.x & 63, half = lane >> 5, l32 = lane & 31;
    const int w = acm_uniform(blockIdx.x * 4 + (threadIdx.x >> 6));
    if (w >= csr.n_items) return;
    const AcmItem it = csr.items[w];
    const int row = acm_uniform(it.row), begin = acm_uniform(it.begin), end = acm_uniform(it.end),
              slot = acm_uniform(it.slot);
    float acc[NG][2];
#pragma unroll
    for (int c = 0; c < NG; ++c) acc[c][0] = acc[c][1] = 0.f;
    const bool col_ok = 2 * l32 < F;
    constexpr int UNR = 4;
    for (int base = begin; base < end; base += 64) {
        const int kk = base + lane;
        int my_j = 0;
        float my_a = 0.f;
        if (kk < end) {
            my_j = csr.indices[kk];
            my_a = csr.vals ? csr.vals[kk] : 1.f;
        }
        const int cnt = min(64, end - base);
        for (int t = 0; t < cnt; t += 2 * UNR) {
            unsigned zz[UNR][NG];
            float2 zf[UNR][NG];
            float a[UNR];
            bool ok[UNR];
#pragma unroll
            for (int u = 0; u < UNR; ++u) {
                const int t0 = t + 2 * u;
                const bool have0 = t0 < cnt, have1 = t0 + 1 < cnt;
                const int j0 = __builtin_amdgcn_readlane(my_j, have0 ? t0 : 0);
                const int j1 = __builtin_amdgcn_readlane(my_j, have1 ? t0 + 1 : 0);
                const float a0 = acm_lane_f(my_a, have0 ? t0 : 0), a1 = acm_lane_f(my_a, have1 ? t0 + 1 : 0);
                const int j = half ? j1 : j0;
                a[u] = half ? a1 : a0;
                ok[u] = (half ? have1 : have0) && col_ok;
#pragma unroll
                for (int c = 0; c < NG; ++c) {
                    if (BF16) {
                        const unsigned* rowp = reinterpret_cast<const unsigned*>(
                            reinterpret_cast<const unsigned short*>(g.p[c]) + (long)j * g.ld[c]);
                        zz[u][c] = rowp[col_ok ? l32 : 0];
                    } else {
                        const float2* rowp = reinterpret_cast<const float2*>(g.p[c] + (long)j * g.ld[c]);
                        zf[u][c] = rowp[col_ok ? l32 : 0];
                    }
                }
            }
#pragma unroll
            for (int u = 0; u < UNR; ++u)
#pragma unroll
                for (int c = 0; c < NG; ++c) {
                    const float lo = BF16 ? __uint_as_float(zz[u][c] << 16) : zf[u][c].x;
                    const float hi = BF16 ? __uint_as_float(zz[u][c] & 0xFFFF0000u) : zf[u][c].y;
                    acc[c][0] = ok[u] ? fmaf(a[u], lo, acc[c][0]) : acc[c][0];
                    acc[c][1] = ok[u] ? fmaf(a[u], hi, acc[c][1]) : acc[c][1];
                }
        }
    }
#pragma unroll
    for (int c = 0; c < NG; ++c)
#pragma unroll
        for (int i = 0; i < 2; ++i) {
            const acm_u32x2 r = __builtin_amdgcn_permlane32_swap(__float_as_uint(acc[c][i]), __float_as_uint(acc[c][i]),
                                                                 false, false);
            acc[c][i] = __uint_as_float(r[0]) + __uint_as_float(r[1]);
        }
    if (slot < 0) {
        LayPair32 lay{lane};
        Epi::template apply<LayPair32, NG>(ea, row, lay, F, acc);
    } else if (lane < 32) {
        float* ps = partial + (long)slot * (NG * F);
#pragma unroll
        for (int c = 0; c < NG; ++c)
#pragma unroll
            for (int i = 0; i < 2; ++i) {
                const int col = 2 * l32 + i;
                if (col < F) ps[c * F + col] = acc[c][i];
            }
    }
}

template <int NG, int NB, int UNR, int BLK, bool B16 = false>
__device__ __forceinline__ void gather_vec_block(const GatherSrc& g, const unsigned (&ldb)[3], const unsigned (&blk_off)[NB],
                                                 unsigned ok_mask, int my_j, float my_a, float (&acc)[NG][4 * NB]) {
    float4 z[UNR][NG][NB];
    float a[UNR];
#pragma unroll
    for (int uu = 0; uu < UNR; ++uu) {
        const unsigned j = (unsigned)acm_row_bcast(my_j, BLK * UNR + uu);
        a[uu] = __int_as_float(acm_row_bcast(__float_as_int(my_a), BLK * UNR + uu));
#pragma unroll
        for (int c = 0; c < NG; ++c) {
            const char* rp = reinterpret_cast<const char*>(g.p[c]) + (size_t)(j * ldb[c]);
#pragma unroll
            for (int b = 0; b < NB; ++b) {
                if (B16) {
                    const uint2 w = *reinterpret_cast<const uint2*>(rp + blk_off[b]);
                    z[uu][c][b] = make_float4(__uint_as_float(w.x << 16), __uint_as_float(w.x & 0xFFFF0000u),
                                              __uint_as_float(w.y << 16), __uint_as_float(w.y & 0xFFFF0000u));
                } else {
                    z[uu][c][b] = *reinterpret_cast<const float4*>(rp + blk_off[b]);
                }
            }
        }
    }
#pragma unroll
    for (int uu = 0; uu < UNR; ++uu) {
        const float av = a[uu];
#pragma unroll
        for (int c = 0; c < NG; ++c)
#pragma unroll
            for (int b = 0; b < NB; ++b) {
                const bool live = ((ok_mask >> b) & 1u) && av != 0.f;
                acc[c][4 * b + 0] = live ? fmaf(av, z[uu][c][b].x, acc[c][4 * b + 0]) : acc[c][4 * b + 0];
                acc[c][4 * b + 1] = live ? fmaf(av, z[uu][c][b].y, acc[c][4 * b + 1]) : acc[c][4 * b + 1];
                acc[c][4 * b + 2] = live ? fmaf(av, z[uu][c][b].z, acc[c][4 * b + 2]) : acc[c][4 * b + 2];
                acc[c][4 * b + 3] = live ? fmaf(av, z[uu][c][b].w, acc[c][4 * b + 3]) : acc[c][4 * b + 3];
            }
    }
}

template <int NG, int NB, class Epi, bool B16 = false>
__global__ __launch_bounds__(256) void spmm_vec_kernel(CsrView csr, GatherSrc g, int F, typename Epi::Args ea,
                                                       float* __restrict__ partial) {
    constexpr int UNR = (NG * NB >= 4) ? 2 : 4;
    const int lane = threadIdx.x & 63, m = lane & 15, q = lane >> 4;
    const int w = acm_uniform(blockIdx.x * 4 + (threadIdx.x >> 6));
    if (w >= csr.n_items) return;
    const AcmItem it = csr.items[w];
    const int row = acm_uniform(it.row), begin = acm_uniform(it.begin), end = acm_uniform(it.end),
              slot = acm_uniform(it.slot);
    float acc[NG][4 * NB];
#pragma unroll
    for (int c = 0; c < NG; ++c)
#pragma unroll
        for (int i = 0; i < 4 * NB; ++i) acc[c][i] = 0.f;
    unsigned blk_off[NB], ok_mask = 0;
#pragma unroll
    for (int b = 0; b < NB; ++b) {
        const bool ok = 64 * b + 4 * m < F;
        blk_off[b] = ok ? (B16 ? 128u * b + 8u * m : 256u * b + 16u * m) : 0u;
        ok_mask |= ok ? (1u << b) : 0u;
    }
    unsigned ldb[3];
#pragma unroll
    for (int c = 0; c < 3; ++c) ldb[c] = c < NG ? (unsigned)g.ld[c] * (B16 ? 2u : 4u) : 0u;
    const int pos = 4 * m + q;
    for (int base = begin; base < end; base += 64) {
        const int cnt = min(64, end - base);
        int my_j = 0;
        float my_a = 0.f;
        if (pos < cnt) {
            my_j = csr.indices[base + pos];
            my_a = csr.vals ? csr.vals[base + pos] : 1.f;
        }
        const int steps = (cnt + 3) >> 2;
#define ACM_VEC_BLK(B)                                                                                          \
        if (B * UNR < steps) gather_vec_block<NG, NB, UNR, B, B16>(g, ldb, blk_off, ok_mask, my_j, my_a, acc)
        ACM_VEC_BLK(0);
        ACM_VEC_BLK(1);
        ACM_VEC_BLK(2);
        ACM_VEC_BLK(3);
        if (UNR == 2) {
            ACM_VEC_BLK(4);
            ACM_VEC_BLK(5);
            ACM_VEC_BLK(6);
            ACM_VEC_BLK(7);
        }
#undef ACM_VEC_BLK
    }
#pragma unroll
    for (int c = 0; c < NG; ++c)
#pragma unroll
        for (int i = 0; i < 4 * NB; ++i) acc[c][i] = acm_cross_row_sum(acc[c][i]);
    if (slot < 0) {
        LayVec16<NB> lay{lane};
        Epi::template apply<LayVec16<NB>, NG>(ea, row, lay, F, acc);
    } else if (q == 0) {
        float* ps = partial + (long)slot * (NG * F);
#pragma unroll
        for (int c = 0; c < NG; ++c)
#pragma unroll
            for (int i = 0; i < 4 * NB; ++i) {
                const int col = 64 * (i >> 2) + 4 * m + (i & 3);
                if (col < F) ps[c * F + col] = acc[c][i];
            }
    }
}

template <int NREG, int NG, class Epi>
__global__ __launch_bounds__(256) void spmm_fixup_kernel(CsrView csr, int F, typename Epi::Args ea,
                                                         const float* __restrict__ partial) {
    const int lane = threadIdx.x & 63;
    const int w = acm_uniform(blockIdx.x * 4 + (threadIdx.x >> 6));
    if (w >= csr.n_long) return;
    const AcmLongRow lr = csr.long_rows[w];
    const int row = acm_uniform(lr.row), sb = acm_uniform(lr.slot_begin), se = acm_uniform(lr.slot_end);
    float acc[NG][NREG];
#pragma unroll
    for (int c = 0; c < NG; ++c)
#pragma unroll
        for (int r = 0; r < NREG; ++r) acc[c][r] = 0.f;
    int s = sb;
    for (; s + 4 <= se; s += 4) {
        float v[4][NG][NREG];
#pragma unroll
        for (int u = 0; u < 4; ++u) {
            const float* ps = partial + (long)(s + u) * (NG * F);
#pragma unroll
            for (int c = 0; c < NG; ++c)
#pragma unroll
                for (int r = 0; r < NREG; ++r) {
                    const int col = lane + 64 * r;
                    v[u][c][r] = col < F ? ps[c * F + col] : 0.f;
                }
        }
#pragma unroll
        for (int u = 0; u < 4; ++u)
#pragma unroll
            for (int c = 0; c < NG; ++c)
#pragma unroll
                for (int r = 0; r < NREG; ++r) acc[c][r] += v[u][c][r];
    }
    for (; s < se; ++s) {
        const float* ps = partial + (long)s * (NG * F);
#pragma unroll
        for (int c = 0; c < NG; ++c)
#pragma unroll
            for (int r = 0; r < NREG; ++r) {
                const int col = lane + 64 * r;
                if (col < F) acc[c][r] += ps[c * F + col];
            }
    }
    LayWide<NREG> lay{lane};
    Epi::template apply<LayWide<NREG>, NG>(ea, row, lay, F, acc);
}

template <int FP>
__device__ __forceinline__ void load_row(const float* __restrict__ p, int F, bool vec, float (&z)[FP]) {
    if (vec) {
        if (FP == 2) {
            const float2 v = *reinterpret_cast<const float2*>(p);
            z[0] = v.x;
            z[1] = v.y;
        } else {
#pragma unroll
            for (int q = 0; q < FP / 4; ++q) {
                const float4 v = reinterpret_cast<const float4*>(p)[q];
                z[4 * q + 0] = v.x;
                z[4 * q + 1] = v.y;
                z[4 * q + 2] = v.z;
                z[4 * q + 3] = v.w;
            }
        }
    } else {
#pragma unroll
        for (int f = 0; f < FP; ++f) z[f] = (f < F) ? p[f] : 0.f;
    }
}

constexpr int NARROW_MAX_BLOCKS = 8192;
constexpr int NARROW_U = 2;

template <int FP, int NG, int GS, bool MERGED, class Epi, int U = NARROW_U>
__global__ __launch_bounds__(256) void spmm_narrow_kernel(CsrView csr, GatherSrc g, int F, int vecmask,
                                                               typename Epi::Args ea, float* __restrict__ partial) {
    constexpr int GPB = 256 / GS;
    constexpr bool COOP = GS == ACM_WINDOW && GPB == ACM_WINDOW;
    __shared__ float coop_lds[COOP ? ACM_WINDOW * NG * FP : 1];
    const int gl = threadIdx.x % GS;
    const int G = gridDim.x * GPB;
    int w = blockIdx.x * GPB + threadIdx.x / GS;
    if (w >= csr.n_items) return;
    AcmItem it = csr.items[w];
    int k0 = it.begin;
    const bool unit = csr.vals == nullptr;
    bool v[U];
    int j[U];
    float a[U];
#pragma unroll
    for (int u = 0; u < U; ++u) {
        const int k = k0 + gl + u * GS;
        v[u] = k < it.end;
        j[u] = v[u] ? csr.indices[k] : 0;
        a[u] = v[u] ? (unit ? 1.f : csr.vals[k]) : 0.f;
    }
    while (true) {
        const int wn = w + G;
        const bool has_next = wn < csr.n_items;
        AcmItem itn = it;
        if (has_next) itn = csr.items[wn];
        float acc[NG][FP];
#pragma unroll
        for (int c = 0; c < NG; ++c)
#pragma unroll
            for (int f = 0; f < FP; ++f) acc[c][f] = 0.f;
        while (true) {
            float z[U][NG][FP];
#pragma unroll
            for (int u = 0; u < U; ++u) {
                if (MERGED) {
                    float t[2 * FP];
                    load_row<2 * FP>(g.p[0] + (long)j[u] * g.ld[0], 2 * FP, true, t);
#pragma unroll
                    for (int f = 0; f < FP; ++f) {
                        z[u][0][f] = t[f];
                        if (NG > 1) z[u][1 % NG][f] = t[FP + f];
                    }
#pragma unroll
                    for (int c = 2; c < NG; ++c) load_row<FP>(g.p[c] + (long)j[u] * g.ld[c], F, (vecmask >> c) & 1, z[u][c]);
                } else {
#pragma unroll
                    for (int c = 0; c < NG; ++c) load_row<FP>(g.p[c] + (long)j[u] * g.ld[c], F, (vecmask >> c) & 1, z[u][c]);
                }
            }
            const int k1 = k0 + U * GS;
            const bool more = k1 < it.end;
            const int pb = more ? k1 : itn.begin;
            const int pe = more ? it.end : (has_next ? itn.end : pb);
            bool nv[U];
            int nj[U];
            float na[U];
#pragma unroll
            for (int u = 0; u < U; ++u) {
                const int k = pb + gl + u * GS;
                nv[u] = k < pe;
                nj[u] = nv[u] ? csr.indices[k] : 0;
                na[u] = nv[u] ? (unit ? 1.f : csr.vals[k]) : 0.f;
            }
#pragma unroll
            for (int c = 0; c < NG; ++c)
#pragma unroll
                for (int f = 0; f < FP; ++f)
#pragma unroll
                    for (int u = 0; u < U; ++u) acc[c][f] = v[u] ? fmaf(a[u], z[u][c][f], acc[c][f]) : acc[c][f];
#pragma unroll
            for (int u = 0; u < U; ++u) j[u] = nj[u], a[u] = na[u], v[u] = nv[u];
            if (!more) break;
            k0 = k1;
        }
#pragma unroll
        for (int c = 0; c < NG; ++c)
#pragma unroll
            for (int f = 0; f < FP; ++f) acc[c][f] = acm_group_sum<GS>(acc[c][f]);
        if (COOP && w / ACM_WINDOW < csr.n_windows) {
            const int g = threadIdx.x / GS;
            if (gl == 0) {
#pragma unroll
                for (int c = 0; c < NG; ++c)
#pragma unroll
                    for (int f = 0; f < FP; ++f) coop_lds[(g * NG + c) * FP + f] = acc[c][f];
            }
            __syncthreads();
            const AcmLongRow lr = csr.long_rows[csr.long_index[it.row]];
            const bool multi = lr.windows > 1;
            if (multi ? g == 0 : it.slot == lr.slot_begin) {
                const int pieces = multi ? ACM_WINDOW : lr.slot_end - lr.slot_begin;
#pragma unroll
                for (int c = 0; c < NG; ++c)
#pragma unroll
                    for (int f = 0; f < FP; ++f) {
                        float t = 0.f;
                        for (int q = 0; q < pieces; ++q) t += coop_lds[((g + q) * NG + c) * FP + f];
                        acc[c][f] = t;
                    }
                if (!multi) {
                    LaySerial<FP> lay{gl == 0};
                    Epi::template apply<LaySerial<FP>, NG>(ea, it.row, lay, F, acc);
                } else if (gl == 0) {
                    float* ps = partial + (long)it.slot * (NG * F);
#pragma unroll
                    for (int c = 0; c < NG; ++c)
#pragma unroll
                        for (int f = 0; f < FP; ++f)
                            if (f < F) ps[c * F + f] = acc[c][f];
                }
            }
            __syncthreads();
        } else if (it.slot < 0) {
            LaySerial<FP> lay{gl == 0};
            Epi::template apply<LaySerial<FP>, NG>(ea, it.row, lay, F, acc);
        } else if (gl == 0) {
            float* ps = partial + (long)it.slot * (NG * F);
#pragma unroll
            for (int c = 0; c < NG; ++c)
#pragma unroll
                for (int f = 0; f < FP; ++f)
                    if (f < F) ps[c * F + f] = acc[c][f];
        }
        if (!has_next) break;
        it = itn;
        w = wn;
        k0 = it.begin;
    }
}

template <int FP, int NG, class Epi>
__global__ __launch_bounds__(256) void spmm_fixup_narrow_kernel(CsrView csr, int F, typename Epi::Args ea,
                                                                const float* __restrict__ partial) {
    const int m = threadIdx.x & 15;
    const int w = blockIdx.x * 16 + (threadIdx.x >> 4);
    if (w >= csr.n_long) return;
    const AcmLongRow lr = csr.long_rows[w];
    float acc[NG][FP];
#pragma unroll
    for (int c = 0; c < NG; ++c)
#pragma unroll
        for (int f = 0; f < FP; ++f) acc[c][f] = 0.f;
    for (int s = lr.slot_begin + m; s < lr.slot_end; s += 16) {
        const float* ps = partial + (long)s * (NG * F);
#pragma unroll
        for (int c = 0; c < NG; ++c)
#pragma unroll
            for (int f = 0; f < FP; ++f)
                if (f < F) acc[c][f] += ps[c * F + f];
    }
#pragma unroll
    for (int c = 0; c < NG; ++c)
#pragma unroll
        for (int f = 0; f < FP; ++f) acc[c][f] = acm_group_sum<16>(acc[c][f]);
    LaySerial<FP> lay{m == 0};
    Epi::template apply<LaySerial<FP>, NG>(ea, lr.row, lay, F, acc);
}

template <int FP, int NG, class Epi>
__global__ __launch_bounds__(256) void spmm_fixup_windows_kernel(CsrView csr, int F, typename Epi::Args ea,
                                                                 const float* __restrict__ partial) {
    const int m = threadIdx.x & 15;
    const int w = blockIdx.x * 16 + (threadIdx.x >> 4);
    if (w >= csr.n_long) return;
    const AcmLongRow lr = csr.long_rows[w];
    if (lr.windows <= 1) return;
    float acc[NG][FP];
    const float* ps = partial + (long)(lr.slot_begin + ACM_WINDOW * m) * (NG * F);
#pragma unroll
    for (int c = 0; c < NG; ++c)
#pragma unroll
        for (int f = 0; f < FP; ++f) acc[c][f] = (m < lr.windows && f < F) ? ps[c * F + f] : 0.f;
#pragma unroll
    for (int c = 0; c < NG; ++c)
#pragma unroll
        for (int f = 0; f < FP; ++f) acc[c][f] = acm_group_sum<16>(acc[c][f]);
    LaySerial<FP> lay{m == 0};
    Epi::template apply<LaySerial<FP>, NG>(ea, lr.row, lay, F, acc);
}

template <class Epi>
__global__ __launch_bounds__(256) void spmm_narrow_pair3_kernel(CsrView csr, const float* __restrict__ table, typename Epi::Args ea,
                                                                float* __restrict__ partial) {
    constexpr int FP = 2, NG = 3, GPB = 16, U = 4, STEP = 8 * U;
    static_assert(GPB == ACM_WINDOW, "one window of work items per workgroup round");
    __shared__ float coop[ACM_WINDOW * 8];
    const int gl = threadIdx.x & 15, e = gl >> 1, h = gl & 1;
    const int G = gridDim.x * GPB;
    int w = blockIdx.x * GPB + (threadIdx.x >> 4);
    if (w >= csr.n_items) return;
    const bool unit = csr.vals == nullptr;
    const float* th = table + 4 * h;
    AcmItem it = csr.items[w];
    int k0 = it.begin;
    int j[U];
    float a[U];
    bool v[U];
#pragma unroll
    for (int u = 0; u < U; ++u) {
        const int k = k0 + e + 8 * u;
        v[u] = k < it.end;
        j[u] = v[u] ? csr.indices[k] : 0;
        a[u] = v[u] ? (unit ? 1.f : csr.vals[k]) : 0.f;
    }
    while (true) {
        const int wn = w + G;
        const bool has_next = wn < csr.n_items;
        AcmItem itn = it;
        if (has_next) itn = csr.items[wn];
        float acc[4] = {0.f, 0.f, 0.f, 0.f};
        while (true) {
            float4 z[U];
#pragma unroll
            for (int u = 0; u < U; ++u) z[u] = *reinterpret_cast<const float4*>(th + (long)j[u] * 8);
            const int k1 = k0 + STEP;
            const bool more = k1 < it.end;
            const int pb = more ? k1 : itn.begin;
            const int pe = more ? it.end : (has_next ? itn.end : pb);
            int nj[U];
            float na[U];
            bool nv[U];
#pragma unroll
            for (int u = 0; u < U; ++u) {
                const int k = pb + e + 8 * u;
                nv[u] = k < pe;
                nj[u] = nv[u] ? csr.indices[k] : 0;
                na[u] = nv[u] ? (unit ? 1.f : csr.vals[k]) : 0.f;
            }
#pragma unroll
            for (int u = 0; u < U; ++u) {
                acc[0] = v[u] ? fmaf(a[u], z[u].x, acc[0]) : acc[0];
                acc[1] = v[u] ? fmaf(a[u], z[u].y, acc[1]) : acc[1];
                acc[2] = v[u] ? fmaf(a[u], z[u].z, acc[2]) : acc[2];
                acc[3] = v[u] ? fmaf(a[u], z[u].w, acc[3]) : acc[3];
            }
#pragma unroll
            for (int u = 0; u < U; ++u) j[u] = nj[u], a[u] = na[u], v[u] = nv[u];
            if (!more) break;
            k0 = k1;
        }
#pragma unroll
        for (int i = 0; i < 4; ++i) {
            acc[i] += acm_dpp<0x4E>(acc[i]);
            acc[i] += acm_dpp<0x124>(acc[i]);
            acc[i] += acm_dpp<0x128>(acc[i]);
        }
        bool finish = it.slot < 0;
        if (w / ACM_WINDOW < csr.n_windows) {
            const int g = threadIdx.x >> 4;
            if (gl < 2) {
#pragma unroll
                for (int i = 0; i < 4; ++i) coop[g * 8 + 4 * h + i] = acc[i];
            }
            __syncthreads();
            const AcmLongRow lr = csr.long_rows[csr.long_index[it.row]];
            const bool multi = lr.windows > 1;
            finish = multi ? g == 0 : it.slot == lr.slot_begin;
            if (finish && gl < 2) {
                const int pieces = multi ? ACM_WINDOW : lr.slot_end - lr.slot_begin;
#pragma unroll
                for (int i = 0; i < 4; ++i) {
                    float t = 0.f;
                    for (int q = 0; q < pieces; ++q) t += coop[(g + q) * 8 + 4 * h + i];
                    acc[i] = t;
                }
                if (multi) {
                    float* ps = partial + (long)it.slot * (NG * FP) + 4 * h;
                    ps[0] = acc[0], ps[1] = acc[1];
                    if (h == 0) ps[2] = acc[2], ps[3] = acc[3];
                }
            }
            if (multi) finish = false;
            __syncthreads();
        }
        const float s0 = acm_dpp<0xB1>(acc[0]), s1 = acm_dpp<0xB1>(acc[1]);
        if (finish) {
            float out[NG][FP] = {{acc[0], acc[1]}, {acc[2], acc[3]}, {s0, s1}};
            LaySerial<FP> lay{gl == 0};
            Epi::template apply<LaySerial<FP>, NG>(ea, it.row, lay, 2, out);
        }
        if (!has_next) break;
        it = itn;
        w = wn;
        k0 = it.begin;
    }
}

template <int V>
using acm_int = std::integral_constant<int, V>;
inline auto acm_fp_of(int F) { return acm_one_of<2, 4, 8>(F <= 2 ? 2 : (F <= 4 ? 4 : 8)); }
inline int acm_fp(int F) { return acm_fp_of(F).v; }
inline auto acm_nreg_of(int F) { return acm_one_of<1, 2, 4>(F <= 64 ? 1 : (F <= 128 ? 2 : 4)); }
inline auto acm_nb_of(int F) { return acm_one_of<1, 2, 3, 4>(F <= 64 ? 1 : (F <= 128 ? 2 : (F <= 192 ? 3 : 4))); }
inline auto acm_k_of(int k) { return acm_one_of<3, 4>(k); }
inline auto acm_lanes_of(int lanes) { return acm_one_of<8, 16, 32>(lanes); }

inline int narrow_lanes(int64_t n_rows, int64_t nnz) {
    const double avg = (double)nnz / (double)(n_rows > 0 ? n_rows : 1);
    return avg <= 12.0 ? 8 : (avg <= 160.0 ? 16 : 32);
}
inline bool narrow_finishes_long_rows(const acm_csr* a) { return narrow_lanes(a->n_rows, a->nnz) == ACM_WINDOW; }

struct GatherForm {
    enum Kind { NARROW, PAIR3, VEC16, VEC, PAIR_BF16, PAIR_F32, WIDE } kind;
    int lanes;
    int vecmask;
    bool merged;
};

inline GatherForm choose_gather_form(int64_t n_rows, int64_t n_cols, int64_t nnz, int64_t n_long, const int32_t* long_index,
                                     const GatherSrc& g, int NG, int F, bool bf16, int form, bool fused_head) {
    GatherForm f = {GatherForm::WIDE, 0, 0, false};
    if (F <= 8) {
        const int FP = acm_fp(F);
        for (int c = 0; c < NG; ++c) {
            const size_t al = (FP == 2) ? 8 : 16;
            const bool ok = (F == FP || g.ld[c] >= FP) && (((uintptr_t)g.p[c]) % al == 0) &&
                            ((g.ld[c] * sizeof(float)) % al == 0);
            f.vecmask |= ok ? (1 << c) : 0;
        }
        f.lanes = narrow_lanes(n_rows, nnz);
        if (NG == 3 && F == 2 && f.lanes == 16 && !bf16 && g.p[1] == g.p[0] + 2 && g.p[2] == g.p[0] + 4 && g.ld[0] == 8 && g.ld[1] == 8 &&
            g.ld[2] == 8 && ((uintptr_t)g.p[0]) % 32 == 0 && (n_long == 0 || long_index != nullptr)) {
            f.kind = GatherForm::PAIR3;
            return f;
        }
        f.merged = NG >= 2 && g.p[1] == g.p[0] + FP && g.ld[0] == g.ld[1] &&
                   ((uintptr_t)g.p[0]) % (8 * FP) == 0 && (g.ld[0] * sizeof(float)) % (8 * FP) == 0;
        f.kind = GatherForm::NARROW;
        return f;
    }
    bool pair32 = !bf16 && F > 32 && F <= 64 && F % 2 == 0 && (size_t)n_cols * F * NG * sizeof(float) <= (8u << 20);
    for (int c = 0; c < NG && pair32; ++c) pair32 = ((uintptr_t)g.p[c]) % 8 == 0 && g.ld[c] % 2 == 0;
    const bool l2_resident = (size_t)n_cols * F * NG * sizeof(float) <= (8u << 20);
    bool vec = !bf16 && F % 4 == 0 && form != 1 &&
               ((NG == 1 && nnz >= 16 * n_rows) || (l2_resident && NG > 1 && nnz >= 4 * n_rows) || form == 2);
    for (int c = 0; c < NG && vec; ++c)
        vec = ((uintptr_t)g.p[c]) % 16 == 0 && g.ld[c] % 4 == 0 &&
              (uint64_t)n_cols * (uint64_t)g.ld[c] * 4u < (1ull << 32);
    if (vec && form != 3) pair32 = false;
    const bool head_beyond_cache = fused_head && (size_t)n_cols * F * NG * 2u > ((size_t)256 << 20);
    bool vec16 = bf16 && F % 4 == 0 && form != 1 && form != 3 &&
                 ((NG == 1 && nnz >= 16 * n_rows) || (NG > 1 && nnz >= 4 * n_rows && !head_beyond_cache) ||
                  form == 2);
    for (int c = 0; c < NG && vec16; ++c)
        vec16 = ((uintptr_t)g.p[c]) % 8 == 0 && g.ld[c] % 4 == 0 && (uint64_t)n_cols * (uint64_t)g.ld[c] * 2u < (1ull << 32);
    f.kind = vec16 ? GatherForm::VEC16 : (vec && !pair32) ? GatherForm::VEC : bf16 ? GatherForm::PAIR_BF16 : pair32 ? GatherForm::PAIR_F32 : GatherForm::WIDE;
    return f;
}

template <class E, class = void> struct epi_wide_only : std::false_type {};
template <class E> struct epi_wide_only<E, std::void_t<decltype(E::kWideOnly)>> : std::bool_constant<E::kWideOnly> {};

template <int NG, class Epi>
void launch_pair3(int grid, hipStream_t st, const CsrView& v, const float* table, const typename Epi::Args& ea, float* partial) {
    if constexpr (NG == 3) hipLaunchKernelGGL((spmm_narrow_pair3_kernel<Epi>), dim3(grid), dim3(256), 0, st, v, table, ea, partial);
}

template <int NG, class Epi>
int finish_window_rows(const acm_csr* a, const CsrView& v, int F, const typename Epi::Args& ea, const float* partial, hipStream_t st) {
    if (v.n_multi == 0) return ACM_OK;
    const int grid = (int)((v.n_long + 15) / 16);
    acm_pick([&](auto fp) {
        hipLaunchKernelGGL((spmm_fixup_windows_kernel<fp(), NG, Epi>), dim3(grid), dim3(256), 0, st, v, F, ea, partial);
        return ACM_OK;
    }, acm_fp_of(F));
    ACM_CHECK_HIP(hipGetLastError());
    return ACM_OK;
}

template <int NG, class Epi>
int launch_gather(const acm_csr* a, const GatherSrc& g, int F, const typename Epi::Args& ea,
                  void* workspace, size_t ws_bytes, hipStream_t st, const char* who,
                  const float* vals_override = nullptr, bool bf16 = false, bool defer_fixup = false,
                  const GatherOverride* over = nullptr) {
    const int64_t n_slots = over ? over->n_slots : a->n_slots;
    const size_t need = (size_t)n_slots * (size_t)(NG * F) * sizeof(float);
    ACM_REQUIRE(ws_bytes >= need && (need == 0 || workspace), ACM_ENOMEM,
                "%s: workspace %zu B < required %zu B", who, ws_bytes, need);
    float* partial = (float*)workspace;
    CsrView v = over ? over->view : acm_view(a);
    if (vals_override) v.vals = vals_override;
    const int64_t n_items = v.n_items, n_long = v.n_long;
    if (n_items == 0) return ACM_OK;
    ACM_REQUIRE(!bf16 || (F > 8 && F <= 64 && F % 2 == 0), ACM_EUNSUPPORTED,
                "%s: bf16 gathered operands are implemented for even 8 < F <= 64", who);
    if (bf16) {
        bool aligned = true;
        for (int c = 0; c < NG; ++c) aligned = aligned && ((uintptr_t)g.p[c]) % 4 == 0 && g.ld[c] % 2 == 0;
        ACM_REQUIRE(aligned, ACM_EINVAL, "%s: bf16 operands must be 4-byte aligned with an even leading dimension", who);
    }
    ACM_REQUIRE(F <= 256, ACM_EUNSUPPORTED, "%s: F = %d > 256 columns per channel", who, F);
    const GatherForm form = choose_gather_form(a->n_rows, a->n_cols, a->nnz, a->n_long, a->long_index, g, NG, F, bf16,
                                               acm_tuning().wide_form, Epi::kFusedHead);
    auto wide = [&](auto kernel) { hipLaunchKernelGGL(kernel, dim3((int)((n_items + 3) / 4)), dim3(256), 0, st, v, g, F, ea, partial); };
    if constexpr (epi_wide_only<Epi>::value)
        ACM_REQUIRE(F > 8, ACM_EUNSUPPORTED, "%s: this epilogue exists for more than 8 columns (got %d)", who, F);
    int rc = ACM_OK;
    switch (form.kind) {
    case GatherForm::PAIR3: {
      if constexpr (!epi_wide_only<Epi>::value) {
        int grid = (int)((n_items + 15) / 16);
        if (grid > NARROW_MAX_BLOCKS) grid = NARROW_MAX_BLOCKS;
        launch_pair3<NG, Epi>(grid, st, v, g.p[0], ea, partial);
        ACM_CHECK_HIP(hipGetLastError());
        return finish_window_rows<NG, Epi>(a, v, F, ea, partial, st);
      }
      break;
    }
    case GatherForm::NARROW:
      if constexpr (!epi_wide_only<Epi>::value)
        rc = acm_pick([&](auto fp, auto gs) {
            constexpr int FP = decltype(fp)::value, GS = decltype(gs)::value, gpb = 256 / GS;
            int grid = (int)((n_items + gpb - 1) / gpb);
            if (grid > NARROW_MAX_BLOCKS) grid = NARROW_MAX_BLOCKS;
            if (form.merged)
                hipLaunchKernelGGL((spmm_narrow_kernel<FP, NG, GS, (NG >= 2), Epi>), dim3(grid), dim3(256), 0, st, v, g, F,
                                   form.vecmask, ea, partial);
            else
                hipLaunchKernelGGL((spmm_narrow_kernel<FP, NG, GS, false, Epi>), dim3(grid), dim3(256), 0, st, v, g, F,
                                   form.vecmask, ea, partial);
            return ACM_OK;
        }, acm_fp_of(F), acm_lanes_of(form.lanes));
        break;
    case GatherForm::VEC16: wide(spmm_vec_kernel<NG, 1, Epi, true>); break;
    case GatherForm::VEC: acm_pick([&](auto nb) { wide(spmm_vec_kernel<NG, nb(), Epi>); return ACM_OK; }, acm_nb_of(F)); break;
    case GatherForm::PAIR_BF16: wide(spmm_pair_kernel<NG, Epi, true>); break;
    case GatherForm::PAIR_F32: wide(spmm_pair_kernel<NG, Epi, false>); break;
    case GatherForm::WIDE: acm_pick([&](auto nreg) { wide(spmm_wide_kernel<nreg(), NG, Epi>); return ACM_OK; }, acm_nreg_of(F)); break;
    }
    ACM_REQUIRE(rc == ACM_OK, ACM_EUNSUPPORTED, "%s: no narrow gather for %d lanes per item", who, form.lanes);
    ACM_CHECK_HIP(hipGetLastError());
    if constexpr (!epi_wide_only<Epi>::value)
        if (F <= 8 && narrow_finishes_long_rows(a)) return finish_window_rows<NG, Epi>(a, v, F, ea, partial, st);
    if (defer_fixup || !n_long) return ACM_OK;
    if (F <= 8) {
      if constexpr (!epi_wide_only<Epi>::value)
        acm_pick([&](auto fp) {
            hipLaunchKernelGGL((spmm_fixup_narrow_kernel<fp(), NG, Epi>), dim3((int)((n_long + 15) / 16)), dim3(256), 0, st, v, F, ea,
                               partial);
            return ACM_OK;
        }, acm_fp_of(F));
    } else {
        acm_pick([&](auto nreg) {
            hipLaunchKernelGGL((spmm_fixup_kernel<nreg(), NG, Epi>), dim3((int)((n_long + 3) / 4)), dim3(256), 0, st, v, F, ea, partial);
            return ACM_OK;
        }, acm_nreg_of(F));
    }
    ACM_CHECK_HIP(hipGetLastError());
    return ACM_OK;
}
```

### acm_gnn_amd/csrc/acm_gcn.hip

```cpp
#include "acm_gather_device.h"

namespace {

struct EpiGcnFwd {
    static constexpr bool kFusedHead = false;
    static constexpr bool kWideOnly = true;
    struct Args {
        float* y;
        long ldy;
        int relu, col0;
        const float* row_scale;
        acm_dropout_t drop;
        const float* w_next;
        long ld_w;
        int f_next;
        float* z_next;
        long ld_zn;
    };
    template <class L, int NG>
    static __device__ __forceinline__ void apply(const Args& a, int row, const L& lay, int F, const float (&acc)[NG][L::NV]) {
        const float os = a.row_scale ? a.row_scale[row] : 1.f;
        const AcmDropCtx dc = acm_drop_ctx(a.drop);
        const bool stores = Owns<L>::lane_stores(lay);
        float v[L::NV];
#pragma unroll
        for (int i = 0; i < L::NV; ++i) {
            const int col = lay.col(i);
            const bool ok = col < F;
            float t = os * acc[0][i];
            if (a.relu) t = fmaxf(t, 0.f);
            if (dc.on && ok) t *= acm_drop1(dc, row, a.col0 + col);
            v[i] = ok ? t : 0.f;
            if (ok && stores) a.y[(long)row * a.ldy + col] = t;
        }
        if (a.f_next > 0) {
            for (int j = 0; j < a.f_next; ++j) {
                float part = 0.f;
#pragma unroll
                for (int i = 0; i < L::NV; ++i) {
                    const int col = lay.col(i);
                    if (col < F) part = fmaf(v[i], a.w_next[(long)(a.col0 + col) * a.ld_w + j], part);
                }
                const float t = lay.rsum(part);
                if (stores && lay.leader()) a.z_next[(long)row * a.ld_zn + j] = t;
            }
        }
    }
};

struct GcnBwdRec {
    const float* h;
    long ldh;
    const float* w2;
    long ldw2;
    float keep_scale;
    int relu, hidden;
    float* g;
    long ldg;
    float* dz;
    long lddz;
    float* part;
    long group_stride;
};

struct EpiGcnBwd {
    struct Args {
        const GcnBwdRec* rec;
        int gs, slab_base;
    };
    template <class L, int NG>
    static __device__ __forceinline__ void apply(const Args& k, int row, const L&, int F, const float (&acc)[NG][L::NV]) {
        const GcnBwdRec a = *k.rec;
        const int tid = blockIdx.x * 256 + threadIdx.x;
        const int gl = tid % k.gs;
        float* ps = a.part + (long)(k.slab_base + tid / k.gs) * 32;
        if (gl == 0 && a.dz) {
#pragma unroll
            for (int c = 0; c < L::NV; ++c)
                if (c < F) a.dz[(long)row * a.lddz + c] = acc[0][c];
        }
        for (int hc = gl; hc < a.hidden; hc += k.gs) {
            const float hv = a.h[(long)row * a.ldh + hc];
            float dh = 0.f;
#pragma unroll
            for (int c = 0; c < L::NV; ++c)
                if (c < F) dh = fmaf(acc[0][c], a.w2[(long)hc * a.ldw2 + c], dh);
            float gv = dh;
            if (a.relu) gv = hv > 0.f ? dh * a.keep_scale : 0.f;
            else if (a.keep_scale != 1.f) gv = hv != 0.f ? dh * a.keep_scale : 0.f;
            a.g[(long)row * a.ldg + hc] = gv;
#pragma unroll
            for (int c = 0; c < L::NV; ++c)
                if (c < F) {
                    const int q = hc * F + c;
                    float* p = ps + (long)(q >> 5) * a.group_stride + (q & 31);
                    *p = fmaf(hv, acc[0][c], *p);
                }
        }
    }
};

__global__ __launch_bounds__(256) void gcn_bwd_prepare_kernel(GcnBwdRec r, GcnBwdRec* dst, float4* slabs, long n4) {
    if (blockIdx.x == 0 && threadIdx.x == 0) *dst = r;
    for (long q = (long)blockIdx.x * 256 + threadIdx.x; q < n4; q += (long)gridDim.x * 256) slabs[q] = make_float4(0.f, 0.f, 0.f, 0.f);
}

constexpr size_t GCN_BWD_REC_BYTES = 256;
constexpr int GCN_BWD_MAX_BLOCKS = 256;
constexpr int GCN_BWD_MAX_HIDDEN = 256;

struct GcnBwdPlan {
    int gs, grid, fix_blocks;
    long slabs, groups;
    size_t gather_bytes, partial_bytes;
};

GcnBwdPlan gcn_bwd_plan(const acm_csr* a, int width, int hidden) {
    GcnBwdPlan p;
    p.gs = narrow_lanes(a->n_rows, a->nnz);
    if (acm_fp(width) == 8 && p.gs == 16) p.gs = 32;
    const int gpb = 256 / p.gs;
    long grid = (a->n_items + gpb - 1) / gpb;
    if (grid > GCN_BWD_MAX_BLOCKS) grid = GCN_BWD_MAX_BLOCKS;
    if (grid < 1) grid = 1;
    p.grid = (int)grid;
    const bool fix = p.gs == ACM_WINDOW ? a->n_multi > 0 : a->n_long > 0;
    p.fix_blocks = fix ? (int)((a->n_long + 15) / 16) : 0;
    p.slabs = (long)p.grid * gpb + (long)p.fix_blocks * 16;
    p.groups = ((long)hidden * width + 31) / 32;
    p.gather_bytes = (((size_t)a->n_slots * (size_t)width * sizeof(float)) + 255) / 256 * 256;
    p.partial_bytes = (size_t)p.groups * (size_t)p.slabs * 32 * sizeof(float);
    return p;
}

int check_drop(const acm_dropout_t& d, const char* who) {
    ACM_REQUIRE(d.p == 0.f || (d.p > 0.f && d.p < 1.f && d.step), ACM_EINVAL, "%s: bad dropout spec", who);
    return ACM_OK;
}

}

extern "C" int acm_gcn_fwd(const acm_csr_t* a, const acm_gcn_fwd_t* p, void* workspace, size_t workspace_bytes,
                           acm_stream_t stream) {
    ACM_REQUIRE(p, ACM_EINVAL, "acm_gcn_fwd: NULL parameter block");
    ACM_REQUIRE(p->width > 0 && p->ld_z >= p->width && p->ld_y >= p->width, ACM_ESHAPE,
                "acm_gcn_fwd: width %d ld_z %lld ld_y %lld", p->width, (long long)p->ld_z, (long long)p->ld_y);
    ACM_REQUIRE(p->f_next >= 0 && p->f_next <= 8, ACM_EUNSUPPORTED, "acm_gcn_fwd: f_next %d (the fused projection takes 0..8 columns)",
                p->f_next);
    ACM_REQUIRE(p->f_next == 0 || p->width <= 256, ACM_EUNSUPPORTED, "acm_gcn_fwd: the fused projection needs width <= 256 (got %d)",
                p->width);
    ACM_REQUIRE(p->f_next == 0 || (p->ld_w_next >= p->f_next && p->ld_z_next >= p->f_next), ACM_ESHAPE,
                "acm_gcn_fwd: ld_w_next %lld ld_z_next %lld below f_next %d", (long long)p->ld_w_next, (long long)p->ld_z_next, p->f_next);
    ACM_REQUIRE(a && p->z && p->y && (p->f_next == 0 || (p->w_next && p->z_next)), ACM_EINVAL, "acm_gcn_fwd: NULL argument");
    const int st = check_drop(p->drop, "acm_gcn_fwd");
    if (st != ACM_OK) return st;
    if (!p->relu && p->drop.p == 0.f && p->f_next == 0) {
        const acm_spmm_opts_t o = {nullptr, p->row_scale, nullptr, 0, nullptr, 0, 0};
        return acm_spmm_internal(a, p->z, p->ld_z, p->width, p->y, p->ld_y, &o, workspace, workspace_bytes, stream, nullptr);
    }
    ACM_REQUIRE(p->width > 8, ACM_EUNSUPPORTED, "acm_gcn_fwd: a post-op (ReLU / dropout / next projection) needs more than 8 columns "
                "(got %d): compose acm_spmm_ex + acm_bias_act + acm_gemm", p->width);
    int wd = 0;
    for (int c0 = 0; c0 < p->width; c0 += wd) {
        const int left = p->width - c0;
        wd = left <= 256 ? left : (left - 256 <= 8 ? 128 : 256);
        const GatherSrc g = {{p->z + c0, nullptr, nullptr}, {(long)p->ld_z, 0, 0}};
        const EpiGcnFwd::Args ea = {p->y + c0, (long)p->ld_y, p->relu, c0, p->row_scale, p->drop,
                                    p->f_next ? p->w_next : nullptr, (long)p->ld_w_next, p->f_next, p->z_next, (long)p->ld_z_next};
        const int rc = launch_gather<1, EpiGcnFwd>(a, g, wd, ea, workspace, workspace_bytes, (hipStream_t)stream, "acm_gcn_fwd");
        if (rc != ACM_OK) return rc;
    }
    return ACM_OK;
}

static int gcn_bwd_check(const acm_gcn_bwd_t* p) {
    ACM_REQUIRE(p, ACM_EINVAL, "acm_gcn_bwd: NULL parameter block");
    ACM_REQUIRE(p->width >= 1 && p->width <= 8, ACM_EUNSUPPORTED,
                "acm_gcn_bwd: width %d (a narrow dY of 1..8 columns; wider layers compose acm_spmm_ex and the GEMMs)", p->width);
    ACM_REQUIRE(p->hidden >= 1 && p->hidden <= GCN_BWD_MAX_HIDDEN, ACM_EUNSUPPORTED, "acm_gcn_bwd: hidden %d (1..%d)", p->hidden,
                GCN_BWD_MAX_HIDDEN);
    return ACM_OK;
}

extern "C" int acm_gcn_bwd_workspace_bytes(const acm_csr_t* a_t, int width, int hidden, size_t* bytes) {
    const acm_gcn_bwd_t shape = {width, hidden};
    const int st = gcn_bwd_check(&shape);
    if (st != ACM_OK) return st;
    ACM_REQUIRE(a_t && bytes, ACM_EINVAL, "acm_gcn_bwd_workspace_bytes: NULL argument");
    const GcnBwdPlan pl = gcn_bwd_plan(a_t, width, hidden);
    *bytes = pl.gather_bytes + GCN_BWD_REC_BYTES + pl.partial_bytes;
    return ACM_OK;
}

extern "C" int acm_gcn_bwd(const acm_csr_t* a, const acm_gcn_bwd_t* p, void* workspace, size_t workspace_bytes,
                           acm_stream_t stream) {
    int st = gcn_bwd_check(p);
    if (st != ACM_OK) return st;
    ACM_REQUIRE(p->ld_dy >= p->width && p->ld_h >= p->hidden && p->ld_g >= p->hidden && p->ld_w2 >= p->width &&
                    p->ld_dw2 >= p->width && (!p->dz || p->ld_dz >= p->width) && p->keep_scale >= 1.f, ACM_ESHAPE,
                "acm_gcn_bwd: leading dimensions (ld_dy %lld ld_h %lld ld_g %lld ld_w2 %lld ld_dw2 %lld ld_dz %lld) / keep_scale",
                (long long)p->ld_dy, (long long)p->ld_h, (long long)p->ld_g, (long long)p->ld_w2, (long long)p->ld_dw2,
                (long long)p->ld_dz);
    ACM_REQUIRE(a && p->dy && p->h && p->w2 && p->g && p->d_w2, ACM_EINVAL, "acm_gcn_bwd: NULL argument");
    const int F = p->width;
    const GcnBwdPlan pl = gcn_bwd_plan(a, F, p->hidden);
    const size_t need = pl.gather_bytes + GCN_BWD_REC_BYTES + pl.partial_bytes;
    ACM_REQUIRE(workspace && workspace_bytes >= need && ((uintptr_t)workspace) % 16 == 0, ACM_ENOMEM,
                "acm_gcn_bwd: workspace %zu B < required %zu B (or not 16-byte aligned)", workspace_bytes, need);
    static_assert(sizeof(GcnBwdRec) <= GCN_BWD_REC_BYTES, "record slot");
    hipStream_t s = (hipStream_t)stream;
    float* partial = (float*)workspace;
    GcnBwdRec* rec = (GcnBwdRec*)((char*)workspace + pl.gather_bytes);
    float* slabs = (float*)((char*)rec + GCN_BWD_REC_BYTES);
    {
        const GcnBwdRec r = {p->h, (long)p->ld_h, p->w2, (long)p->ld_w2, p->keep_scale, p->relu, p->hidden, p->g, (long)p->ld_g,
                             p->dz, (long)p->ld_dz, slabs, pl.slabs * 32};
        const long n4 = (long)(pl.partial_bytes / 16);
        long blocks = (n4 + 255) / 256;
        blocks = blocks < 1 ? 1 : (blocks > 1024 ? 1024 : blocks);
        hipLaunchKernelGGL(gcn_bwd_prepare_kernel, dim3((unsigned)blocks), dim3(256), 0, s, r, rec, (float4*)slabs, n4);
        ACM_CHECK_HIP(hipGetLastError());
    }
    if (a->n_items > 0) {
        const CsrView v = acm_view(a);
        const GatherSrc g = {{p->dy, nullptr, nullptr}, {(long)p->ld_dy, 0, 0}};
        const GatherForm form = choose_gather_form(a->n_rows, a->n_cols, a->nnz, a->n_long, a->long_index, g, 1, F, false, 0, false);
        EpiGcnBwd::Args ea = {rec, pl.gs, 0};
        const int rc = acm_pick([&](auto fp, auto gs) {
            constexpr int FP = decltype(fp)::value, GS = decltype(gs)::value;
            if constexpr (!(FP == 8 && GS == 16))
                hipLaunchKernelGGL((spmm_narrow_kernel<FP, 1, GS, false, EpiGcnBwd>), dim3(pl.grid), dim3(256), 0, s, v, g, F,
                                   form.vecmask, ea, partial);
            return ACM_OK;
        }, acm_fp_of(F), acm_lanes_of(pl.gs));
        ACM_REQUIRE(rc == ACM_OK, ACM_EUNSUPPORTED, "acm_gcn_bwd: no narrow gather for %d lanes per item", pl.gs);
        ACM_CHECK_HIP(hipGetLastError());
        if (pl.fix_blocks) {
            ea.gs = 16;
            ea.slab_base = pl.grid * (256 / pl.gs);
            const bool windows = pl.gs == ACM_WINDOW;
            acm_pick([&](auto fp) {
                if (windows)
                    hipLaunchKernelGGL((spmm_fixup_windows_kernel<fp(), 1, EpiGcnBwd>), dim3(pl.fix_blocks), dim3(256), 0, s, v, F, ea, partial);
                else
                    hipLaunchKernelGGL((spmm_fixup_narrow_kernel<fp(), 1, EpiGcnBwd>), dim3(pl.fix_blocks), dim3(256), 0, s, v, F, ea, partial);
                return ACM_OK;
            }, acm_fp_of(F));
            ACM_CHECK_HIP(hipGetLastError());
        }
    }
    const int len = p->hidden * F;
    const acm_reduce_seg_t seg = {slabs, (int)pl.slabs, 32, 0, len, p->d_w2, F, 0, p->ld_dw2, 0, (int)(pl.slabs * 32), 0};
    return acm_reduce_emit(p->defer, &seg, 1, s);
}
```

### acm_gnn_amd/csrc/acm_items.h

```cpp
#pragma once
#include <stdint.h>

#include <algorithm>
#include <vector>

#define ACM_WINDOW 16

struct AcmItem {
    int32_t row, begin, end, slot;
};
struct AcmLongRow {
    int32_t row, slot_begin, slot_end, windows;
};

inline void build_items(const std::vector<int32_t>& indptr, int chunk, std::vector<AcmItem>& items,
                        std::vector<AcmLongRow>& longs, int64_t& n_slots, int32_t& max_deg, int64_t& n_windows, int64_t& n_multi,
                        const uint8_t* keep = nullptr) {
    const int64_t n = (int64_t)indptr.size() - 1;
    items.clear();
    longs.clear();
    items.reserve(n + n / 8);
    n_slots = 0;
    max_deg = 0;
    n_multi = 0;
    for (int64_t r = 0; r < n; ++r) {
        const int32_t b = indptr[r], e = indptr[r + 1];
        const int32_t deg = e - b;
        max_deg = std::max(max_deg, deg);
        if (deg <= chunk || (keep && !keep[r])) continue;
        int32_t pieces = (deg + chunk - 1) / chunk;
        int32_t windows = 0;
        if (pieces > ACM_WINDOW && (deg + ACM_WINDOW - 1) / ACM_WINDOW > 4 * chunk) {
            windows = (deg + 2 * ACM_WINDOW * chunk - 1) / (2 * ACM_WINDOW * chunk);
            if (windows > ACM_WINDOW) windows = ACM_WINDOW;
            pieces = windows * ACM_WINDOW;
        } else if (pieces > ACM_WINDOW) {
            pieces = ACM_WINDOW;
        }
        const int32_t room = ACM_WINDOW - (int32_t)(items.size() % ACM_WINDOW);
        if ((room < pieces || windows) && room < ACM_WINDOW) {
            AcmLongRow& prev = longs.back();
            for (int32_t q = 0; q < room; ++q) items.push_back({prev.row, indptr[prev.row + 1], indptr[prev.row + 1], (int32_t)n_slots++});
            prev.slot_end = (int32_t)n_slots;
        }
        const int32_t per = (deg + pieces - 1) / pieces;
        AcmLongRow lr = {(int32_t)r, (int32_t)n_slots, 0, windows};
        for (int32_t q = 0; q < pieces; ++q) {
            const int32_t s = std::min(e, b + q * per);
            items.push_back({(int32_t)r, s, std::min(e, s + per), (int32_t)n_slots++});
        }
        lr.slot_end = (int32_t)n_slots;
        n_multi += windows > 1;
        longs.push_back(lr);
    }
    if (!longs.empty() && items.size() % ACM_WINDOW) {
        AcmLongRow& prev = longs.back();
        while (items.size() % ACM_WINDOW) items.push_back({prev.row, indptr[prev.row + 1], indptr[prev.row + 1], (int32_t)n_slots++});
        prev.slot_end = (int32_t)n_slots;
    }
    n_windows = (int64_t)items.size() / ACM_WINDOW;
    for (int64_t r = 0; r < n; ++r)
        if (indptr[r + 1] - indptr[r] <= chunk && !(keep && !keep[r])) items.push_back({(int32_t)r, indptr[r], indptr[r + 1], -1});
}

struct AcmLossRowsHost {
    std::vector<AcmItem> items;
    std::vector<AcmLongRow> longs;
    std::vector<int32_t> long_index;
    int64_t n_slots = 0, n_windows = 0, n_multi = 0;
    int64_t kept_rows = 0, kept_edges = 0;
};

inline void acm_loss_rows_host(const std::vector<int32_t>& indptr, const uint8_t* keep, int chunk, AcmLossRowsHost& out) {
    const int64_t n = (int64_t)indptr.size() - 1;
    out = AcmLossRowsHost();
    for (int64_t r = 0; r < n; ++r)
        if (keep[r]) {
            ++out.kept_rows;
            out.kept_edges += indptr[r + 1] - indptr[r];
        }
    int32_t max_deg = 0;
    build_items(indptr, chunk, out.items, out.longs, out.n_slots, max_deg, out.n_windows, out.n_multi, keep);
    if (!out.longs.empty()) {
        out.long_index.assign((size_t)n, -1);
        for (size_t i = 0; i < out.longs.size(); ++i) out.long_index[(size_t)out.longs[i].row] = (int32_t)i;
    }
}
```

### acm_gnn_amd/tuning.py

```python
import contextlib
import ctypes as C
import os
import threading

KERNEL_KEYS = ("chunk", "wide_form", "bwd_split", "rows16", "agg_fused", "gemm_forms")
HOST_DEFAULTS = {"rewrites": 15, "implicit": 1, "relabel": -1, "pipeline": 8192, "csr_features": 256, "small_step": 16384,
                 "mlp_stack": 1, "loss_rows": 1}
HOST_RANGES = {"rewrites": (0, 15), "implicit": (0, 1), "relabel": (-1, 1), "pipeline": (0, 1 << 31), "csr_features": (0, 1 << 31),
               "small_step": (0, 16384), "mlp_stack": (0, 1), "loss_rows": (0, 1)}

REWRITE_AGG_FIRST = 1
REWRITE_ACMII_RECOMPUTE = 2
REWRITE_ACMII_MASK = 4
REWRITE_AGGW_FUSED = 8
ROWS16_EPI, ROWS16_BWD, ROWS16_LOCAL = 1, 2, 4
GEMM_ROWS, GEMM_BX3, GEMM_BX3_WIDE, GEMM_ROWS_ALWAYS = 1, 2, 4, 8


class Tuning(C.Structure):
    _fields_ = [(k, C.c_int32) for k in KERNEL_KEYS] + [("reserved", C.c_int32 * 10)]


class _Host:
    __slots__ = tuple(HOST_DEFAULTS)

    def __init__(self, **kw):
        for k, v in HOST_DEFAULTS.items():
            setattr(self, k, int(kw.get(k, v)))

    def as_dict(self):
        return {k: getattr(self, k) for k in HOST_DEFAULTS}


def parse(text):
    kern, host = {}, {}
    for item in (text or "").split(","):
        item = item.strip()
        if not item:
            continue
        key, sep, val = item.partition("=")
        if not sep:
            raise ValueError(f"ACM_TUNING: '{item}' is not key=value")
        try:
            v = int(val, 0)
        except ValueError:
            raise ValueError(f"ACM_TUNING: '{item}': the value must be an integer") from None
        if key in KERNEL_KEYS:
            kern[key] = v
        elif key in HOST_DEFAULTS:
            lo, hi = HOST_RANGES[key]
            if not lo <= v <= hi:
                raise ValueError(f"ACM_TUNING: {key}={v} outside {lo}..{hi}")
            host[key] = v
        else:
            raise ValueError(f"ACM_TUNING: unknown key '{key}' (known: {', '.join(KERNEL_KEYS + tuple(HOST_DEFAULTS))})")
    return kern, host


def parse_lenient(text, report=None):
    import sys
    report = report or (lambda msg: sys.stderr.write(f"acm_gnn_amd: {msg} (ignored)\n"))
    kern, host = {}, {}
    for item in (text or "").split(","):
        if not item.strip():
            continue
        try:
            k, h = parse(item)
        except ValueError as exc:
            report(str(exc))
            continue
        kern.update(k)
        host.update(h)
    return kern, host


LEGACY_ENV = ("ACM_GATHER_DTYPE", "ACM_EVAL_AGG_CACHE", "ACM_CHUNK", "ACM_WIDE_FORM", "ACM_BWD_SPLIT", "ACM_AGG_FUSED", "ACM_PIPELINE",
              "ACM_IMPLICIT", "ACM_RELABEL", "ACM_REWRITES", "ACM_ROWS16", "ACM_GEMM_FORMS")


def _report_legacy(environ, report=None):
    import sys
    report = report or (lambda msg: sys.stderr.write(f"acm_gnn_amd: {msg}\n"))
    found = [k for k in LEGACY_ENV if k in environ]
    if found:
        report(f"{', '.join(found)}: environment switches of earlier rounds are no longer read; use ACM_TUNING=\"key=value,...\"")
    return found


_LOADED_HOST = parse_lenient(os.environ.get("ACM_TUNING", ""))[1]
_report_legacy(os.environ)
HOST = _Host(**_LOADED_HOST)
_lock = threading.RLock()
_kernel_cache = None
_kernel_touched = False


def kernel():
    global _kernel_cache
    if _kernel_cache is None:
        from . import _lib
        t = Tuning()
        _lib.check(_lib.load().acm_tuning_get(C.byref(t)), "acm_tuning_get")
        _kernel_cache = {k: int(getattr(t, k)) for k in KERNEL_KEYS}
    return _kernel_cache


def set_kernel(**kw):
    global _kernel_cache, _kernel_touched
    from . import _lib
    with _lock:
        _kernel_touched = True
        cur = dict(kernel())
        for k, v in kw.items():
            if k not in KERNEL_KEYS:
                raise KeyError(k)
            cur[k] = int(v)
        t = Tuning()
        for k, v in cur.items():
            setattr(t, k, v)
        _lib.check(_lib.load().acm_tuning_set(C.byref(t)), "acm_tuning_set")
        _kernel_cache = None


def apply(**kw):
    host_kw = {k: v for k, v in kw.items() if k in HOST_DEFAULTS}
    kern_kw = {k: v for k, v in kw.items() if k in KERNEL_KEYS}
    unknown = set(kw) - set(host_kw) - set(kern_kw)
    if unknown:
        raise KeyError(f"unknown tuning switch(es): {sorted(unknown)}")
    for k, v in host_kw.items():
        lo, hi = HOST_RANGES[k]
        if not lo <= int(v) <= hi:
            raise ValueError(f"{k}={v} outside {lo}..{hi}")
    with _lock:
        for k, v in host_kw.items():
            setattr(HOST, k, int(v))
        if kern_kw:
            set_kernel(**kern_kw)


def reset(kernel_too=True):
    global _kernel_cache, _kernel_touched
    with _lock:
        for k, v in HOST_DEFAULTS.items():
            setattr(HOST, k, int(_LOADED_HOST.get(k, v)))
        if kernel_too and _kernel_touched:
            from . import _lib
            _lib.check(_lib.load().acm_tuning_set(None), "acm_tuning_set")
            _kernel_touched = False
        _kernel_cache = None


def invalidate():
    global _kernel_cache
    _kernel_cache = None


def gemm_forms():
    return kernel()["gemm_forms"]


@contextlib.contextmanager
def override(**kw):
    host_kw = {k: v for k, v in kw.items() if k in HOST_DEFAULTS}
    kern_kw = {k: v for k, v in kw.items() if k in KERNEL_KEYS}
    unknown = set(kw) - set(host_kw) - set(kern_kw)
    if unknown:
        raise KeyError(f"unknown tuning switch(es): {sorted(unknown)}")
    for k, v in host_kw.items():
        lo, hi = HOST_RANGES[k]
        if not lo <= int(v) <= hi:
            raise ValueError(f"{k}={v} outside {lo}..{hi}")
    with _lock:
        old_host = HOST.as_dict()
        old_kern = dict(kernel()) if kern_kw else None
        try:
            for k, v in host_kw.items():
                setattr(HOST, k, int(v))
            if kern_kw:
                set_kernel(**kern_kw)
            yield
        finally:
            for k, v in old_host.items():
                setattr(HOST, k, v)
            if old_kern is not None:
                set_kernel(**old_kern)


def env_for_child(**kw):
    cur = dict(HOST.as_dict())
    try:
        cur.update(kernel())
    except Exception:
        pass
    cur.update({k: int(v) for k, v in kw.items()})
    return ",".join(f"{k}={v}" for k, v in cur.items())
```

### include/acm_hip.h

```cpp
#ifndef ACM_HIP_H
#define ACM_HIP_H

#include <stddef.h>
#include <stdint.h>

#ifdef __cplusplus
extern "C" {
#endif

#define ACM_ABI_VERSION 29

typedef enum {
    ACM_OK = 0,
    ACM_EINVAL = 1,
    ACM_ESHAPE = 2,
    ACM_EHIP = 3,
    ACM_EUNSUPPORTED = 4,
    ACM_ENOMEM = 5,
} acm_status_t;

typedef struct acm_csr acm_csr_t;
typedef void* acm_stream_t;

int acm_version(void);
const char* acm_last_error(void);

typedef struct {
    int32_t chunk;
    int32_t wide_form;
    int32_t bwd_split;
    int32_t rows16;
    int32_t agg_fused;
    int32_t gemm_forms;
    int32_t reserved[10];
} acm_tuning_t;
int acm_tuning_get(acm_tuning_t* out);
int acm_tuning_set(const acm_tuning_t* in);

int acm_csr_create(int64_t n_rows, int64_t n_cols, int64_t nnz,
                   const int32_t* indptr_dev, const int32_t* indices_dev,
                   const float* vals_dev, int chunk, acm_csr_t** out);
int acm_csr_transpose(const acm_csr_t* a, int chunk, acm_csr_t** out);
int acm_csr_slice_rows(const acm_csr_t* a, int64_t row_begin, int64_t row_end,
                       int chunk, acm_csr_t** out);
void acm_csr_destroy(acm_csr_t* a);

int acm_shard_plan(int64_t n_rows, const int64_t* indptr_host, int world, int64_t row_cost,
                   int64_t* bounds_host);

typedef struct {
    int64_t n_rows, n_cols, nnz;
    int64_t n_items;
    int64_t n_long_rows;
    int64_t n_partial_slots;
    int32_t chunk;
    int32_t max_degree;
    const int32_t* indptr;
    const int32_t* indices;
    const float* vals;
    const int32_t* src_pos;
    int64_t stream_steps;
    int64_t stream_slices;
    int32_t stream_waves;
    int32_t stream_long_rows;
    int32_t item_stream_waves;
    int32_t reserved;
    int64_t item_stream_batches;
} acm_csr_info_t;
int acm_csr_info(const acm_csr_t* a, acm_csr_info_t* info);

int acm_csr_build_streams(acm_csr_t* a, int n_waves, int lmax);

int acm_csr_build_item_streams(acm_csr_t* a, int n_waves);

int acm_csr_build_loss_rows(acm_csr_t* a, const uint8_t* keep_dev);
int acm_csr_loss_rows_info(const acm_csr_t* a, int64_t* out);

int acm_spmm_workspace_bytes(const acm_csr_t* a, int width, size_t* bytes);

int acm_gemm_workspace_bytes(int transA, int transB, int64_t M, int64_t N, int64_t K,
                             size_t* bytes);
int acm_gemm(int transA, int transB, int64_t M, int64_t N, int64_t K,
             const float* A, int64_t lda, const float* B, int64_t ldb,
             float* C, int64_t ldc, int relu, void* workspace, size_t workspace_bytes,
             acm_stream_t stream);

int acm_gemm_blocks(int transA, int transB, int64_t M, int64_t N, int64_t K,
                    const float* A, int64_t lda, const float* B, int64_t ldb,
                    float* C, int64_t ldc, int64_t c_col_block, int64_t c_block_stride, int relu,
                    void* workspace, size_t workspace_bytes, acm_stream_t stream);

typedef struct {
    float    p;
    int32_t  tag;
    uint64_t seed;
    const int64_t* step;
    int64_t  row_offset;
    int64_t  step_offset;
} acm_dropout_t;

int acm_dropout(int64_t n_rows, int64_t n_cols, const float* src, int64_t ld_src,
                float* dst, int64_t ld_dst, int64_t dst_cols, const acm_dropout_t* d, acm_stream_t stream);

int acm_gemm_drop(int transA, int transB, int64_t M, int64_t N, int64_t K,
                  const float* A, int64_t lda, const float* B, int64_t ldb,
                  float* C, int64_t ldc, int64_t c_col_block, int64_t c_block_stride, int relu,
                  const acm_dropout_t* a_drop, void* workspace, size_t workspace_bytes, acm_stream_t stream);

int acm_proj3(int64_t n_rows, int64_t K, const float* X, int64_t ldx,
              const float* w_low, const float* w_high, const float* w_mlp, int64_t ld_w, int64_t f, int64_t f_block,
              float* C, int64_t ldc, int64_t split_col, float* C2, int64_t ldc2, int relu,
              const acm_dropout_t* x_drop, acm_stream_t stream);

typedef struct {
    const float* partial;
    int32_t nblk, row_stride;
    int32_t q0, len;
    float*  dst;
    int32_t inner;
    int32_t col_block;
    int64_t outer_stride, block_stride;
    int32_t elem_stride;
    int32_t reserved;
} acm_reduce_seg_t;

typedef struct {
    int32_t n, cap;
    acm_reduce_seg_t* segs;
} acm_reduce_list_t;

int acm_reduce_flush(acm_reduce_list_t* list, acm_stream_t stream);

int acm_gemm_split(int transA, int transB, int64_t M, int64_t N, int64_t K,
                   const float* A, int64_t lda, const float* B, int64_t ldb,
                   float* C, int64_t ldc, int64_t split_col, float* C2, int64_t ldc2, int relu,
                   void* workspace, size_t workspace_bytes, acm_stream_t stream);

int acm_proj_fwd(int64_t n_rows, int64_t f_in, int f_out, const float* X, int64_t ldx,
                 const float* w_low, const float* w_high, const float* w_mlp, int64_t ldw, int relu,
                 float* Z_lh, int64_t ld_lh, float* Z_i, int64_t ld_i, acm_stream_t stream);
int acm_proj_fwd_at(int64_t n_rows, int64_t f_in, int f_out, const float* X, int64_t ldx,
                    const float* w_low, const float* w_high, const float* w_mlp, int64_t ldw, int relu,
                    float* Z_lh, int64_t ld_lh, int64_t h_col, float* Z_i, int64_t ld_i, acm_stream_t stream);
int acm_proj_bwd_workspace_bytes(int64_t n_rows, int64_t f_in, int n_out, size_t* bytes);
int acm_proj_bwd(int64_t n_rows, int64_t f_in, int n_out, const float* X, int64_t ldx,
                 const float* dZ, int64_t lddz, const float* w_low, const float* w_high, const float* w_mlp, int64_t ldw,
                 float* dX, int64_t lddx, float* dW, int64_t lddw, int64_t dw_col_block, int64_t dw_block_stride,
                 void* workspace, size_t workspace_bytes, acm_reduce_list_t* defer, acm_stream_t stream);

#define ACM_PROJ_BLOCKS_MAX 8
typedef struct {
    int32_t n_blocks;
    int32_t f, f_block;
    int32_t f_in;
    const float* w_low;
    const float* w_high;
    const float* w_mlp;
    int64_t ldw;
    const float* h[ACM_PROJ_BLOCKS_MAX];
    int64_t ld_h[ACM_PROJ_BLOCKS_MAX];
    int32_t width[ACM_PROJ_BLOCKS_MAX];
    int32_t row0[ACM_PROJ_BLOCKS_MAX];
    float* d_h[ACM_PROJ_BLOCKS_MAX];
    int64_t ld_dh[ACM_PROJ_BLOCKS_MAX];
} acm_proj_blocks_t;
int acm_proj_blocks_fwd(int64_t n_rows, const acm_proj_blocks_t* p, float* Z, int64_t ldz, int accumulate, int relu,
                        acm_stream_t stream);
int acm_proj_blocks_bwd_workspace_bytes(int64_t n_rows, const acm_proj_blocks_t* p, size_t* bytes);
int acm_proj_blocks_bwd(int64_t n_rows, const acm_proj_blocks_t* p, const float* dZ, int64_t lddz, float* dW, int64_t lddw,
                        int64_t dw_col_block, int64_t dw_block_stride, void* workspace, size_t workspace_bytes,
                        acm_reduce_list_t* defer, acm_stream_t stream);

int acm_linear_fwd(int64_t n_rows, int64_t f_in, int64_t f_out, const float* X, int64_t ldx,
                   const float* W, int64_t ldw, const float* bias, int relu, const acm_dropout_t* drop,
                   float* Y, int64_t ldy, void* workspace, size_t workspace_bytes, acm_stream_t stream);
int acm_bias_act(int64_t n_rows, int f, float* Y, int64_t ldy, const float* bias, int relu,
                 const acm_dropout_t* drop, acm_stream_t stream);
int acm_bias_act_bwd_workspace_bytes(int64_t n_rows, int f, size_t* bytes);
int acm_bias_act_bwd(int64_t n_rows, int f, const float* Y, int64_t ldy, const float* dY, int64_t lddy,
                     float keep_scale, int relu, float* G, int64_t ldg, float* d_bias,
                     void* workspace, size_t workspace_bytes, acm_reduce_list_t* defer, acm_stream_t stream);
int acm_linear_bwd_workspace_bytes(int64_t n_rows, int f_in, int f_out, size_t* bytes);
int acm_linear_bwd(int64_t n_rows, int f_in, int f_out, const float* X, int64_t ldx, const float* Y, int64_t ldy,
                   const float* dY, int64_t lddy, float keep_scale, int relu, float* dW, int64_t lddw, float* d_bias,
                   void* workspace, size_t workspace_bytes, acm_reduce_list_t* defer, acm_stream_t stream);
int acm_linear_fwd_add(int64_t n_rows, int f_in, int f_out, const float* X, int64_t ldx, const float* W, int64_t ldw,
                       const float* bias, int relu, const acm_dropout_t* drop, const float* add, int64_t ld_add,
                       float* Y, int64_t ldy, acm_stream_t stream);
int acm_linear_bwd_recompute(int64_t n_rows, int f_in, int f_out, const float* X, int64_t ldx, const float* W, int64_t ldw,
                             const float* bias, int relu, const acm_dropout_t* drop, const float* dY, int64_t lddy,
                             float* dW, int64_t lddw, float* d_bias, void* workspace, size_t workspace_bytes,
                             acm_reduce_list_t* defer, acm_stream_t stream);

int acm_spmm(const acm_csr_t* a, const float* G, int64_t ldg, int width,
             float* Y, int64_t ldy, void* workspace, size_t workspace_bytes,
             acm_stream_t stream);

int acm_spmm_v(const acm_csr_t* a, const float* vals, const float* G, int64_t ldg, int width,
               float* Y, int64_t ldy, int relu, void* workspace, size_t workspace_bytes,
               acm_stream_t stream);

typedef struct {
    const float* vals;
    const float* row_scale;
    const float* sub; int64_t ld_sub;
    const float* sub_scale;
    int32_t relu;
    int32_t g_bf16;
} acm_spmm_opts_t;

int acm_spmm_ex(const acm_csr_t* a, const void* G, int64_t ldg, int width, float* Y, int64_t ldy,
                const acm_spmm_opts_t* opts, void* workspace, size_t workspace_bytes, acm_stream_t stream);

int acm_cast_bf16(int64_t n_rows, int64_t n_cols, const float* src, int64_t ld_src,
                  uint16_t* dst, int64_t ld_dst, acm_stream_t stream);

typedef struct {
    int32_t f_out;
    int32_t n_channels;
    int32_t relu_after;
    int32_t relu_mlp;
    int32_t layernorm;
    float   scale;
    int64_t row_offset;

    const float* g_low;   int64_t ld_g_low;
    const float* g_high;  int64_t ld_g_high;
    const float* g_struc; int64_t ld_g_struc;
    const float* s_high;  int64_t ld_s_high;
    const float* s_mlp;   int64_t ld_s_mlp;
    const float* s_struc; int64_t ld_s_struc;
    const float* deg;

    const float* att_vec[4];
    const float* ln_weight[4];
    const float* ln_bias[4];
    const float* att_mix;

    float* out;  int64_t ld_out;
    float* pre;  int64_t ld_pre;
    float* att;
    const float* post_scale; int64_t ld_post_scale;
    int32_t post_relu;
    int32_t gather_bf16;
    const float* row_scale;
    acm_dropout_t post_drop;
} acm_conv_fwd_t;

int acm_conv_fwd(const acm_csr_t* a_low, const acm_conv_fwd_t* p,
                 void* workspace, size_t workspace_bytes, acm_stream_t stream);

int acm_conv_head_fwd(int64_t n_rows, const acm_conv_fwd_t* p, acm_stream_t stream);

int acm_conv_aggw_fwd(int64_t n_rows, int64_t f_in, int64_t f_pad, const float* agg, int64_t ld_agg, const float* xs,
                      int64_t ld_xs, const float* w_low, const float* w_high, const float* w_mlp, int64_t ld_w,
                      float* zi, int64_t ld_zi, const acm_conv_fwd_t* p, acm_stream_t stream);

typedef struct {
    int32_t f_out, n_channels, relu_after, relu_mlp, layernorm;
    float   scale;
    const float* grad_out; int64_t ld_grad_out;
    const float* pre;      int64_t ld_pre;
    const float* s_mlp;    int64_t ld_s_mlp;
    const float* deg;
    const float* att_vec[4];
    const float* ln_weight[4];
    const float* ln_bias[4];
    const float* att_mix;
    float* g_low;   int64_t ld_g_low;
    float* g_high;  int64_t ld_g_high;
    float* g_mlp;   int64_t ld_g_mlp;
    float* g_struc; int64_t ld_g_struc;
    float* d_att_vec[4];
    float* d_ln_weight[4];
    float* d_ln_bias[4];
    float* d_att_mix;
    const float* post_scale; int64_t ld_post_scale;
    int32_t post_relu;
    const float* g_scale;
    acm_dropout_t post_drop;
    acm_reduce_list_t* defer;
} acm_conv_bwd_local_t;

int acm_conv_bwd_local_workspace_bytes(int64_t n_rows, int f_out, int n_channels, size_t* bytes);
int acm_conv_bwd_local(int64_t n_rows, const acm_conv_bwd_local_t* p,
                       void* workspace, size_t workspace_bytes, acm_stream_t stream);

int acm_conv_aggw_bwd_workspace_bytes(int64_t n_rows, int64_t f_pad, size_t* bytes);
int acm_conv_aggw_bwd(int64_t n_rows, int64_t f_in, int64_t f_pad, const float* agg, int64_t ld_agg, const float* xs,
                      int64_t ld_xs, const acm_conv_bwd_local_t* p, float* d_w_low, float* d_w_high, float* d_w_mlp,
                      int64_t ld_dw, void* workspace, size_t workspace_bytes, acm_stream_t stream);

typedef struct {
    int32_t f_out;
    int64_t row_offset;
    const float* g_low;   int64_t ld_g_low;
    const float* g_high;  int64_t ld_g_high;
    const float* g_struc; int64_t ld_g_struc;
    const float* s_high;  int64_t ld_s_high;
    const float* s_struc; int64_t ld_s_struc;
    const float* inv_deg;
    const float* mask_low;  int64_t ld_mask_low;
    const float* mask_high; int64_t ld_mask_high;
    float* dz_low;   int64_t ld_dz_low;
    float* dz_high;  int64_t ld_dz_high;
    float* d_struc;  int64_t ld_d_struc;
    const float* self_scale;
    int32_t gather_bf16;
} acm_conv_bwd_spmm_t;

int acm_conv_bwd_spmm(const acm_csr_t* a_low_t, const acm_conv_bwd_spmm_t* p,
                      void* workspace, size_t workspace_bytes, acm_stream_t stream);


typedef struct {
    int32_t f_in, f_pad;
    int32_t f_out, relu_after, relu_mlp, layernorm;
    float   scale;
    const float* xg; int64_t ld_xg;
    const float* xs; int64_t ld_xs;
    const float* w_low; const float* w_high; const float* w_mlp; int64_t ld_w;
    const float* att_vec[4];
    const float* ln_weight[4];
    const float* ln_bias[4];
    const float* att_mix;
    float* out; int64_t ld_out;
    float* agg; int64_t ld_agg;
    float* att;
    const float* post_scale; int64_t ld_post_scale;
    int32_t post_relu;
    int32_t n_channels;
    const void*  sg; int64_t ld_sg;
    int32_t sg_bf16;
    const float* ss; int64_t ld_ss;
    const float* deg;
    float* ps; int64_t ld_ps;
    const float* row_scale;
    acm_dropout_t post_drop;
    float* head_stats; int64_t ld_head_stats;
    const float* next_w_low; const float* next_w_high; const float* next_w_mlp; int64_t next_ld_w;
    int32_t next_f, next_relu;
    float* next_zlh; int64_t ld_next_zlh;
    float* next_zi;  int64_t ld_next_zi;
    int32_t agg_given;
    int32_t reserved0;
    float* agg_copy; int64_t ld_agg_copy;
    float* xs_copy;  int64_t ld_xs_copy;
    const float* next_x; int64_t ld_next_x;
    acm_dropout_t next_drop;
} acm_conv_agg_fwd_t;

int acm_conv_agg_fwd(const acm_csr_t* a_low, const acm_conv_agg_fwd_t* p,
                     void* workspace, size_t workspace_bytes, acm_stream_t stream);

typedef struct {
    int32_t f_in, f_pad, f_out, relu_after, relu_mlp, layernorm;
    float   scale;
    const float* grad_out; int64_t ld_grad_out;
    const float* agg; int64_t ld_agg;
    const float* xs;  int64_t ld_xs;
    const float* w_low; const float* w_high; const float* w_mlp; int64_t ld_w;
    const float* att_vec[4];
    const float* ln_weight[4];
    const float* ln_bias[4];
    const float* att_mix;
    float* d_params;
    const float* post_scale; int64_t ld_post_scale;
    int32_t post_relu;
    int32_t n_channels;
    const float* ps; int64_t ld_ps;
    const float* ss; int64_t ld_ss;
    const float* deg;
    float* g_struc; int64_t ld_g_struc;
    const float* g_struc_scale;
    acm_dropout_t post_drop;
    acm_reduce_list_t* defer;
    const float* head_stats; int64_t ld_head_stats;
    const float* out; int64_t ld_out;
    const acm_csr_t* next_a;
    const float* next_xg; int64_t ld_next_xg;
    const float* next_row_scale;
    float* next_agg; int64_t ld_next_agg;
    const float* proj_dz; int64_t ld_proj_dz;
    const float* proj_w_low; const float* proj_w_high; const float* proj_w_mlp; int64_t proj_ld_w;
    int32_t proj_f;
    float* proj_d_w;
} acm_conv_agg_bwd_t;

int acm_conv_agg_bwd_workspace_bytes(int64_t n_rows, int f_in, int f_out, size_t* bytes);
int acm_conv_agg_bwd(int64_t n_rows, const acm_conv_agg_bwd_t* p,
                     void* workspace, size_t workspace_bytes, acm_stream_t stream);

typedef struct {
    int32_t f_in, f_pad, f_out;
    int32_t layernorm;
    float   scale;
    const float* xg; int64_t ld_xg;
    const float* xs; int64_t ld_xs;
    const float* w_low; const float* w_high; const float* w_mlp; int64_t ld_w;
    const float* att_vec[4];
    const float* ln_weight[4];
    const float* ln_bias[4];
    const float* att_mix;
    float* out; int64_t ld_out;
    float* pre; int64_t ld_pre;
    float* att;
    float* zlh; int64_t ld_zlh;
    float* zi;  int64_t ld_zi;
    const float* post_scale; int64_t ld_post_scale;
    int32_t post_relu;
    const float* row_scale;
    acm_dropout_t post_drop;
    int32_t n_channels;
    const float* ps; int64_t ld_ps;
    const float* ss; int64_t ld_ss;
    const float* deg;
} acm_conv_acmii_fwd_t;

int acm_conv_acmii_fwd_workspace_bytes(const acm_csr_t* a_low, size_t* bytes);
int acm_conv_acmii_fwd(const acm_csr_t* a_low, const acm_conv_acmii_fwd_t* p,
                       void* workspace, size_t workspace_bytes, acm_stream_t stream);

typedef struct {
    int32_t f_in;
    const void* table;
    const float* g_low;  int64_t ld_g_low;
    const float* g_high; int64_t ld_g_high;
    const float* g_mlp;  int64_t ld_g_mlp;
    const float* x; int64_t ld_x;
    int64_t self_offset;
    const float* row_scale;
    float* d_w_low; float* d_w_high; float* d_w_mlp; int64_t ld_dw;
    acm_reduce_list_t* defer;
} acm_conv_acmii_bwd_t;

int acm_acmii_table_bytes(int64_t n_rows, size_t* bytes);
int acm_acmii_table(int64_t n_rows, int f_in, const float* x, int64_t ld_x, const float* w_low, const float* w_high,
                    int64_t ld_w, void* table, size_t table_bytes, acm_stream_t stream);
int acm_conv_acmii_v_fwd(const acm_csr_t* a_low, const acm_conv_acmii_fwd_t* p, const void* table,
                         void* workspace, size_t workspace_bytes, acm_stream_t stream);
int acm_conv_acmii_v_bwd_workspace_bytes(const acm_csr_t* a_low, size_t* bytes);
int acm_conv_acmii_v_bwd(const acm_csr_t* a_low, const acm_conv_acmii_bwd_t* p,
                         void* workspace, size_t workspace_bytes, acm_stream_t stream);

int acm_nll_loss_workspace_bytes(int64_t n_rows, size_t* bytes);
int acm_nll_loss(int64_t n_rows, int n_classes, const float* logits, int64_t ld_logits,
                 const int64_t* labels, const float* row_weight,
                 float* loss, float* dlogits, int64_t ld_dlogits,
                 void* workspace, size_t workspace_bytes, acm_reduce_list_t* defer, acm_stream_t stream);

int acm_eval_metrics_workspace_bytes(int64_t n_rows, int n_sets, size_t* bytes);
int acm_eval_metrics(int64_t n_rows, int n_classes, const float* logits, int64_t ld_logits, const int64_t* labels,
                     const float* weights, int64_t ld_weights, int n_sets, int loss_set, float* out,
                     void* workspace, size_t workspace_bytes, acm_stream_t stream);

typedef struct {
    const float*   logits;
    const float*   weights;
    const int64_t* labels;
    float*         out;
    void*          workspace;
} acm_eval_metrics_slot_t;

int acm_eval_metrics_batch(int64_t n_rows, int n_classes, int64_t ld_logits, int64_t ld_weights, int n_sets, int loss_set,
                           int32_t n_slots, const acm_eval_metrics_slot_t* table, size_t workspace_bytes, acm_stream_t stream);

int acm_bce_loss_workspace_bytes(int64_t n_rows, size_t* bytes);
int acm_bce_loss(int64_t n_rows, int n_classes, const float* logits, int64_t ld_logits,
                 const int64_t* labels, const float* row_weight,
                 float* loss, float* dlogits, int64_t ld_dlogits,
                 void* workspace, size_t workspace_bytes, acm_reduce_list_t* defer, acm_stream_t stream);

int acm_rocauc_scores(int64_t n_rows, int n_classes, const float* logits, int64_t ld_logits, float* scores,
                      acm_stream_t stream);
int acm_rocauc_workspace_bytes(int64_t n_rows, int n_sets, size_t* bytes);
int acm_rocauc(int64_t n_rows, const float* sorted_scores, const int64_t* order, const int64_t* labels,
               const float* weights, int64_t ld_weights, int n_sets, int64_t* counts, double* auc,
               void* workspace, size_t workspace_bytes, acm_stream_t stream);

typedef struct {
    int32_t n_classes;
    const int64_t* labels;
    const float*   row_weight;
    float* loss;
    float* dlogits; int64_t ld_dlogits;
} acm_loss_t;

int acm_conv_fwd_tail_workspace_bytes(int64_t n_rows, int f_out, int n_channels, size_t* bytes);
int acm_conv_fwd_tail(const acm_csr_t* a_low, const acm_conv_fwd_t* fwd, const acm_loss_t* loss,
                      const acm_conv_bwd_local_t* bwd, void* workspace, size_t workspace_bytes,
                      void* tail_workspace, size_t tail_workspace_bytes, acm_stream_t stream);

int acm_conv_fwd_tail_rows(const acm_csr_t* a_low, const acm_conv_fwd_t* fwd, const acm_loss_t* loss,
                           const acm_conv_bwd_local_t* bwd, void* workspace, size_t workspace_bytes,
                           void* tail_workspace, size_t tail_workspace_bytes, acm_stream_t stream);

typedef struct {
    float*       param;
    const float* grad;
    float*       exp_avg;
    float*       exp_avg_sq;
    float*       step;
    int64_t      numel;
} acm_adam_tensor_t;

typedef struct {
    double  lr, beta1, beta2, eps, weight_decay;
    int32_t decoupled;
    int64_t* also_advance;
    int32_t* arrive;
    acm_reduce_list_t* pending;
} acm_adam_config_t;

int acm_adam_step(int32_t n_tensors, const acm_adam_tensor_t* tensors, const acm_adam_config_t* cfg,
                  acm_stream_t stream);

#define ACM_SMALL_ROLES 17
enum {
    ACM_SR_W_LOW = 0, ACM_SR_W_HIGH, ACM_SR_W_MLP,
    ACM_SR_V_LOW, ACM_SR_V_HIGH, ACM_SR_V_MLP, ACM_SR_V_STRUC,
    ACM_SR_LNW_LOW, ACM_SR_LNW_HIGH, ACM_SR_LNW_MLP, ACM_SR_LNW_STRUC,
    ACM_SR_LNB_LOW, ACM_SR_LNB_HIGH, ACM_SR_LNB_MLP, ACM_SR_LNB_STRUC,
    ACM_SR_MIX,
    ACM_SR_STRUC
};

typedef struct {
    int32_t n_classes;
    int32_t n_channels;
    int32_t relu_before;
    int32_t layernorm;
    float   scale;
    int32_t train;
    int32_t update;
    int32_t hidden;
    acm_adam_tensor_t t[2][ACM_SMALL_ROLES];
    const float* x_vals;
    const int32_t* xt_src_pos;
    const float* xt_vals;
    int32_t f_in;
    int32_t reserved1;
    acm_dropout_t drop_in;
    acm_dropout_t drop_hidden;
    const float* row_scale;
    const int64_t* labels;
    const float* row_weight;
    float* loss;
    float* logits;
    float* att1; float* att2;
    double  lr, beta1, beta2, eps, weight_decay;
    int32_t decoupled;
    int64_t* also_advance;
    int32_t* arrive;
    void*   workspace;
    size_t  workspace_bytes;
} acm_small_step_t;

int acm_small_step_workspace_bytes(const acm_csr_t* a_low, const acm_csr_t* x, const acm_csr_t* x_t, size_t* bytes);
int acm_small_step(const acm_csr_t* a_low, const acm_csr_t* x, const acm_csr_t* x_t, const acm_small_step_t* p,
                   acm_stream_t stream);
int acm_small_step_has_hidden(int32_t hidden);

#define ACM_SMALL_BATCH_MAX 32
int acm_small_batch_table_bytes(int32_t n_slots, size_t* bytes);
int acm_small_batch_bind(const acm_csr_t* a_low, const acm_csr_t* x, const acm_csr_t* x_t, int32_t n_slots,
                         const acm_small_step_t* const* slots, void* table, size_t table_bytes, acm_stream_t stream);
int acm_small_batch_step(const acm_csr_t* a_low, const acm_csr_t* x, const acm_csr_t* x_t, int32_t n_slots,
                         const acm_small_step_t* shape, const void* table, acm_stream_t stream);

int acm_homophily_workspace_bytes(int64_t n_rows, int64_t n_cols, int n_classes, size_t* bytes);
int acm_homophily_census(const acm_csr_t* a, const int64_t* labels, int64_t row_offset, int n_classes,
                         int64_t* counts, double* node_sum, int32_t* row_same, int32_t* row_deg,
                         void* workspace, size_t workspace_bytes, acm_stream_t stream);
int acm_class_means_workspace_bytes(int64_t n_rows, int n_features, int n_classes, size_t* bytes);
int acm_class_means(int64_t n_rows, int n_features, int n_classes, const float* z, int64_t ld_z,
                    const int64_t* labels, float* mu, int64_t ld_mu, int64_t* class_count,
                    void* workspace, size_t workspace_bytes, acm_stream_t stream);
int acm_class_score(int64_t n_rows, int n_features, int n_classes, const float* z, int64_t ld_z,
                    const float* mu, int64_t ld_mu, const int64_t* class_count, const int64_t* labels,
                    uint8_t* row_hit, int64_t* counts, acm_stream_t stream);

#define ACM_SYNTH_PAIR 0
#define ACM_SYNTH_RECT 1
#define ACM_SYNTH_RANGE 2
#define ACM_SYNTH_SHORT 1
#define ACM_SYNTH_OVER 2
#define ACM_SYNTH_MAX_DEGREE 256
#define ACM_SYNTH_MAX_FEATURES 262144
int acm_synth_regular(int n_classes, int64_t nodes_per_class, int64_t degree_intra, int64_t degree_inter, uint64_t seed,
                      uint64_t graph_index, int64_t row_begin, int64_t row_end, int32_t* indices, acm_stream_t stream);
int acm_synth_uniform(int64_t n_rows, int64_t n_features, uint64_t seed, uint64_t graph_index, int64_t row_begin, float* out,
                      int64_t ld_out, acm_stream_t stream);
int acm_synth_random_plan(int n_classes, int64_t nodes_per_class, int64_t degree_intra, double edge_homo, int64_t* plan);
int acm_synth_draw(int kind, int64_t a, int64_t b, int block_first, int n_segments, uint64_t seed, uint64_t graph_index,
                   int64_t n_draws, int64_t* keys, acm_stream_t stream);
int acm_synth_select_workspace_bytes(int n_segments, int64_t n_draws, size_t* bytes);
int acm_synth_select(int n_segments, int64_t n_draws, const int64_t* keys, const int64_t* sorted_keys, const int64_t* perm,
                     const int64_t* m, int64_t out_cap, int64_t* out, int64_t* found, int32_t* status, void* workspace,
                     size_t workspace_bytes, acm_stream_t stream);
int acm_synth_inter_count(int n_classes, int cls, double t_edges, const int64_t* block_counts, int64_t* m_out,
                          acm_stream_t stream);
int acm_synth_emit(int kind, int n_classes, int64_t nodes_per_class, int class_first, int n_segments, const int64_t* selected,
                   const int64_t* found, int64_t cap, int64_t* edge_keys, int64_t* block_counts, acm_stream_t stream);

typedef struct {
    int32_t width;
    int32_t relu;
    const float* z; int64_t ld_z;
    float* y; int64_t ld_y;
    const float* row_scale;
    acm_dropout_t drop;
    int32_t f_next;
    int32_t reserved;
    const float* w_next; int64_t ld_w_next;
    float* z_next; int64_t ld_z_next;
} acm_gcn_fwd_t;

typedef struct {
    int32_t width;
    int32_t hidden;
    const float* dy; int64_t ld_dy;
    const float* h; int64_t ld_h;
    const float* w2; int64_t ld_w2;
    float keep_scale;
    int32_t relu;
    float* g; int64_t ld_g;
    float* dz; int64_t ld_dz;
    float* d_w2; int64_t ld_dw2;
    acm_reduce_list_t* defer;
} acm_gcn_bwd_t;

int acm_gcn_fwd(const acm_csr_t* a, const acm_gcn_fwd_t* p, void* workspace, size_t workspace_bytes, acm_stream_t stream);
int acm_gcn_bwd_workspace_bytes(const acm_csr_t* a_t, int width, int hidden, size_t* bytes);
int acm_gcn_bwd(const acm_csr_t* a_t, const acm_gcn_bwd_t* p, void* workspace, size_t workspace_bytes, acm_stream_t stream);

int acm_gemm_act(int64_t n_rows, int64_t f_in, int64_t f_out, const float* X, int64_t ldx, const float* W, int64_t ldw,
                 int relu, const acm_dropout_t* drop, float* Y, int64_t ldy, void* workspace, size_t workspace_bytes,
                 acm_stream_t stream);

typedef struct {
    int32_t rule;
    int32_t early_stopping;
    int32_t epochs;
    int32_t reserved;
    const float*  result;
    const double* result_f64;
    const float*  train_loss;
    int32_t* ctrl;
    double*  best;
    double*  history;
} acm_select_t;

int acm_select_step(const acm_select_t* p, acm_stream_t stream);

int acm_select_step_batch(int32_t n_slots, const acm_select_t* table, acm_stream_t stream);

typedef struct {
    const void* src;
    void*       dst;
    int64_t     numel;
} acm_copy_tensor_t;

int acm_copy_if(int32_t n_tensors, const acm_copy_tensor_t* tensors, const int32_t* flag, acm_stream_t stream);

int acm_bnorm_stats_workspace_bytes(int64_t n_rows, int f, size_t* bytes);
int acm_bnorm_stats(int64_t n_rows, int f, const float* H, int64_t ldh, const float* gamma, const float* beta, float eps,
                    float momentum, int train, float* running_mean, float* running_var, int64_t* num_batches,
                    float* stats, void* workspace, size_t workspace_bytes, acm_stream_t stream);
int acm_bnorm_fold(int f_out, int f_in, const float* W, int64_t ldw, const float* bias, const float* stats, float* W_folded,
                   int64_t ldwf, float* bias_folded, acm_stream_t stream);
int acm_bnorm_param_bwd(int f_out, int f_in, const float* M, int64_t ldm, const float* s, const float* W, int64_t ldw,
                        const float* stats, float* dW, int64_t lddw, float* d_beta, float* d_gamma, acm_stream_t stream);
int acm_bnorm_bwd_workspace_bytes(int64_t n_rows, int f, size_t* bytes);
int acm_bnorm_bwd(int64_t n_rows, int f, const float* dZ, int64_t lddz, const float* H, int64_t ldh, const float* stats,
                  const float* d_beta, const float* d_gamma, float keep_scale, int relu, float* G, int64_t ldg,
                  float* d_bias, void* workspace, size_t workspace_bytes, acm_reduce_list_t* defer, acm_stream_t stream);

#ifdef __cplusplus
}
#endif
#endif
```

Before: 50.04 billion edges/s.

## Spread high-degree rows across item stream with in-kernel last-piece reduction

Adds a 'spread' item list (default on) in which mid-to-high degree rows that are not handled as full windows are split into pieces. The pieces are interleaved among the short-row items, so the narrow sixteen-lane gather balances load across blocks. Each piece writes a partial to a slot and bumps an atomic counter; the last piece to arrive sums all partials via bpermute and runs the epilogue. This removes the separate partial-flush pass for those rows, at the cost of atomics, fences and padding items.

```diff
diff --git a/acm_gnn_amd/_lib.py b/acm_gnn_amd/_lib.py
--- a/acm_gnn_amd/_lib.py
+++ b/acm_gnn_amd/_lib.py
@@ -32,7 +32,7 @@
     "acm_small_batch_table_bytes", "acm_small_batch_bind", "acm_small_batch_step", "acm_eval_metrics_batch", "acm_select_step_batch",
     "acm_bnorm_stats_workspace_bytes", "acm_bnorm_stats", "acm_bnorm_fold", "acm_bnorm_param_bwd", "acm_bnorm_bwd_workspace_bytes", "acm_bnorm_bwd",
     "acm_proj_blocks_fwd", "acm_proj_blocks_bwd_workspace_bytes", "acm_proj_blocks_bwd",
-    "acm_csr_build_loss_rows", "acm_csr_loss_rows_info", "acm_conv_fwd_tail_rows",
+    "acm_csr_build_loss_rows", "acm_csr_loss_rows_info", "acm_conv_fwd_tail_rows", "acm_csr_spread_info",
 )
 LOSS_ROWS_SYMBOLS = ("acm_csr_build_loss_rows", "acm_csr_loss_rows_info", "acm_conv_fwd_tail_rows")
 
@@ -373,6 +373,8 @@
     lib.acm_conv_fwd_tail.argtypes = [vp, C.POINTER(ConvFwd), C.POINTER(Loss), C.POINTER(ConvBwdLocal), vp, sz, vp, sz, vp]
     lib.acm_csr_build_loss_rows.argtypes = [vp, vp]
     lib.acm_csr_loss_rows_info.argtypes = [vp, C.POINTER(C.c_int64)]
+    if hasattr(lib, "acm_csr_spread_info"):
+        lib.acm_csr_spread_info.argtypes = [vp, C.POINTER(C.c_int64)]
     lib.acm_conv_fwd_tail_rows.argtypes = lib.acm_conv_fwd_tail.argtypes
     lib.acm_small_step_workspace_bytes.argtypes = [vp, vp, vp, C.POINTER(sz)]
     lib.acm_small_step.argtypes = [vp, vp, vp, C.POINTER(SmallStep), vp]
diff --git a/acm_gnn_amd/csrc/acm_common.h b/acm_gnn_amd/csrc/acm_common.h
--- a/acm_gnn_amd/csrc/acm_common.h
+++ b/acm_gnn_amd/csrc/acm_common.h
@@ -66,6 +66,7 @@
     int32_t n_waves;
 };
 
+struct AcmSpreadList;
 struct AcmLossRows {
     AcmItem* items;
     AcmLongRow* long_rows;
@@ -73,6 +74,19 @@
     int64_t n_items, n_long, n_slots, n_windows, n_multi;
     uint8_t* keep;
     int64_t kept_rows, kept_edges;
+    AcmSpreadList* spread;
+};
+
+#define ACM_SPREAD_SLOT_FLOATS 24
+struct AcmSpreadList {
+    AcmItem* items;
+    AcmLongRow* long_rows;
+    int32_t* long_index;
+    int32_t* counters;
+    float* slots;
+    int64_t n_items, n_long, n_slots, n_windows, n_multi;
+    int64_t n_spread_rows, n_spread;
+    int64_t launches;
 };
 
 struct acm_csr {
@@ -94,6 +108,7 @@
     AcmItemStreams* item_streams;
     AcmLossRows* loss_rows;
     int device;
+    AcmSpreadList* spread;
 };
 
 struct StreamView {
diff --git a/acm_gnn_amd/csrc/acm_csr.cpp b/acm_gnn_amd/csrc/acm_csr.cpp
--- a/acm_gnn_amd/csrc/acm_csr.cpp
+++ b/acm_gnn_amd/csrc/acm_csr.cpp
@@ -27,11 +27,12 @@
 extern "C" const char* acm_last_error(void) { return g_err; }
 
 namespace {
-const acm_tuning_t kTuningDefaults = {0, 0, -1, 7, 1, 7, {0}};
+const acm_tuning_t kTuningDefaults = {0, 0, -1, 7, 1, 7, 1, {0}};
 struct TuningField { const char* name; int32_t acm_tuning_t::*field; };
 const TuningField kTuningFields[] = {{"chunk", &acm_tuning_t::chunk},           {"wide_form", &acm_tuning_t::wide_form},
                                      {"bwd_split", &acm_tuning_t::bwd_split},   {"rows16", &acm_tuning_t::rows16},
-                                     {"agg_fused", &acm_tuning_t::agg_fused},   {"gemm_forms", &acm_tuning_t::gemm_forms}};
+                                     {"agg_fused", &acm_tuning_t::agg_fused},   {"gemm_forms", &acm_tuning_t::gemm_forms},
+                                     {"spread", &acm_tuning_t::spread}};
 const char* const kHostKeys[] = {"rewrites", "implicit", "relabel", "pipeline", "csr_features", "small_step", "mlp_stack", "loss_rows"};
 
 const char* tuning_invalid(const acm_tuning_t& t) {
@@ -41,6 +42,7 @@
     if (t.rows16 < 0 || t.rows16 > 7) return "rows16";
     if (t.agg_fused < 0 || t.agg_fused > 1) return "agg_fused";
     if (t.gemm_forms < 0 || t.gemm_forms > 15) return "gemm_forms";
+    if (t.spread < 0 || t.spread > 2) return "spread";
     return nullptr;
 }
 
@@ -115,8 +117,16 @@
     delete t;
 }
 
+void free_spread(AcmSpreadList* t) {
+    if (!t) return;
+    for (void* q : {(void*)t->items, (void*)t->long_rows, (void*)t->long_index, (void*)t->counters, (void*)t->slots})
+        if (q) (void)hipFree(q);
+    delete t;
+}
+
 void free_loss_rows(AcmLossRows* t) {
     if (!t) return;
+    free_spread(t->spread);
     for (void* q : {(void*)t->items, (void*)t->long_rows, (void*)t->long_index, (void*)t->keep})
         if (q) (void)hipFree(q);
     delete t;
@@ -125,6 +135,7 @@
 void free_handle(acm_csr* a) {
     if (!a) return;
     free_loss_rows(a->loss_rows);
+    free_spread(a->spread);
     if (a->indptr) (void)hipFree(a->indptr);
     if (a->indices) (void)hipFree(a->indices);
     if (a->vals) (void)hipFree(a->vals);
@@ -137,6 +148,60 @@
     delete a;
 }
 
+
+template <class T>
+int upload(T** dev, const std::vector<T>& host, size_t min_elems = 1) {
+    const size_t n = std::max(host.size(), min_elems);
+    ACM_CHECK_HIP(hipMalloc((void**)dev, n * sizeof(T)));
+    if (!host.empty()) ACM_CHECK_HIP(hipMemcpy(*dev, host.data(), host.size() * sizeof(T), hipMemcpyHostToDevice));
+    return ACM_OK;
+}
+
+int build_spread_list(const std::vector<int32_t>& indptr, int chunk, const uint8_t* keep, AcmSpreadList** out) {
+    *out = nullptr;
+    const int mode = acm_tuning().spread;
+    if (!mode) return ACM_OK;
+    const int64_t bar = (int64_t)(mode == 2 ? ACM_WINDOW / 2 : ACM_WINDOW) * chunk;
+    bool any = false;
+    for (size_t r = 0; r + 1 < indptr.size() && !any; ++r) any = indptr[r + 1] - indptr[r] > bar && !(keep && !keep[r]);
+    if (!any) return ACM_OK;
+    std::vector<AcmItem> items;
+    std::vector<AcmLongRow> longs;
+    int64_t n_slots = 0, n_windows = 0, n_multi = 0, n_spread = 0;
+    int32_t max_deg = 0;
+    build_items(indptr, chunk, items, longs, n_slots, max_deg, n_windows, n_multi, keep, bar, &n_spread);
+    if (!n_spread) return ACM_OK;
+    AcmSpreadList* t = new (std::nothrow) AcmSpreadList();
+    ACM_REQUIRE(t, ACM_ENOMEM, "spread list: host allocation failed");
+    memset(t, 0, sizeof(*t));
+    t->n_items = (int64_t)items.size();
+    t->n_long = (int64_t)longs.size();
+    t->n_slots = n_slots;
+    t->n_windows = n_windows;
+    t->n_multi = n_multi;
+    t->n_spread = n_spread;
+    std::vector<int32_t> index(indptr.size() - 1, -1);
+    for (size_t i = 0; i < longs.size(); ++i) {
+        index[(size_t)longs[i].row] = (int32_t)i;
+        t->n_spread_rows += !longs[i].windows && indptr[(size_t)longs[i].row + 1] - indptr[(size_t)longs[i].row] > bar;
+    }
+    int st = upload(&t->items, items);
+    if (st == ACM_OK) st = upload(&t->long_rows, longs);
+    if (st == ACM_OK) st = upload(&t->long_index, index);
+    if (st == ACM_OK && (hipMalloc((void**)&t->counters, longs.size() * sizeof(int32_t)) != hipSuccess ||
+                         hipMemset(t->counters, 0, longs.size() * sizeof(int32_t)) != hipSuccess ||
+                         hipMalloc((void**)&t->slots, (size_t)n_slots * ACM_SPREAD_SLOT_FLOATS * sizeof(float)) != hipSuccess ||
+                         hipMemset(t->slots, 0, (size_t)n_slots * ACM_SPREAD_SLOT_FLOATS * sizeof(float)) != hipSuccess)) {
+        acm_set_error("spread list: device allocation failed");
+        st = ACM_EHIP;
+    }
+    if (st != ACM_OK) {
+        free_spread(t);
+        return st;
+    }
+    *out = t;
+    return ACM_OK;
+}
 
 int finish_handle(acm_csr* a, const std::vector<int32_t>& h_indptr, int chunk) {
     const int env_chunk = acm_tuning().chunk;
@@ -162,7 +227,7 @@
         ACM_CHECK_HIP(hipMalloc((void**)&a->long_index, index.size() * sizeof(int32_t)));
         ACM_CHECK_HIP(hipMemcpy(a->long_index, index.data(), index.size() * sizeof(int32_t), hipMemcpyHostToDevice));
     }
-    return ACM_OK;
+    return build_spread_list(h_indptr, a->chunk, nullptr, &a->spread);
 }
 
 acm_csr* new_handle(int64_t n_rows, int64_t n_cols, int64_t nnz) {
@@ -355,18 +420,6 @@
 }
 
 
-namespace {
-
-template <class T>
-int upload(T** dev, const std::vector<T>& host, size_t min_elems = 1) {
-    const size_t n = std::max(host.size(), min_elems);
-    ACM_CHECK_HIP(hipMalloc((void**)dev, n * sizeof(T)));
-    if (!host.empty()) ACM_CHECK_HIP(hipMemcpy(*dev, host.data(), host.size() * sizeof(T), hipMemcpyHostToDevice));
-    return ACM_OK;
-}
-
-}
-
 extern "C" int acm_csr_build_streams(acm_csr_t* a, int n_waves, int lmax) {
     ACM_REQUIRE(a, ACM_EINVAL, "acm_csr_build_streams: NULL handle");
     if (a->streams) return ACM_OK;
@@ -633,6 +686,7 @@
     if (st == ACM_OK) st = upload(&t->items, h.items);
     if (st == ACM_OK && !h.longs.empty()) st = upload(&t->long_rows, h.longs);
     if (st == ACM_OK && !h.longs.empty()) st = upload(&t->long_index, h.long_index);
+    if (st == ACM_OK) st = build_spread_list(ip, a->chunk, keep.data(), &t->spread);
     if (st != ACM_OK) {
         free_loss_rows(t);
         return st;
@@ -649,6 +703,26 @@
     out[1] = t ? t->n_items : 0;
     out[2] = t ? t->n_slots : 0;
     out[3] = t ? t->kept_edges : 0;
+    return ACM_OK;
+}
+
+extern "C" int acm_csr_spread_info(const acm_csr_t* a, int64_t* out) {
+    ACM_REQUIRE(a && out, ACM_EINVAL, "acm_csr_spread_info: NULL argument");
+    const AcmSpreadList* lists[2] = {a->spread, a->loss_rows ? a->loss_rows->spread : nullptr};
+    for (int i = 0; i < 2; ++i) {
+        const AcmSpreadList* t = lists[i];
+        int64_t* o = out + 5 * i;
+        o[0] = t ? t->n_spread_rows : 0;
+        o[1] = t ? t->n_spread : 0;
+        o[2] = t ? t->n_items : 0;
+        o[3] = t ? t->launches : 0;
+        o[4] = 0;
+        if (!t) continue;
+        ACM_CHECK_HIP(hipDeviceSynchronize());
+        std::vector<int32_t> c((size_t)t->n_long);
+        ACM_CHECK_HIP(hipMemcpy(c.data(), t->counters, c.size() * sizeof(int32_t), hipMemcpyDeviceToHost));
+        for (int32_t x : c) o[4] += x != 0;
+    }
     return ACM_OK;
 }
 
diff --git a/acm_gnn_amd/csrc/acm_gather_device.h b/acm_gnn_amd/csrc/acm_gather_device.h
--- a/acm_gnn_amd/csrc/acm_gather_device.h
+++ b/acm_gnn_amd/csrc/acm_gather_device.h
@@ -380,10 +380,15 @@
 
 constexpr int NARROW_MAX_BLOCKS = 8192;
 constexpr int NARROW_U = 2;
-
-template <int FP, int NG, int GS, bool MERGED, class Epi, int U = NARROW_U>
+#ifndef ACM_SPREAD_U
+#define ACM_SPREAD_U 2
+#endif
+constexpr int NARROW_SPREAD_U = ACM_SPREAD_U;
+
+template <int FP, int NG, int GS, bool MERGED, class Epi, int U = NARROW_U, bool SPREAD = false>
 __global__ __launch_bounds__(256) void spmm_narrow_kernel(CsrView csr, GatherSrc g, int F, int vecmask,
-                                                               typename Epi::Args ea, float* __restrict__ partial) {
+                                                               typename Epi::Args ea, float* __restrict__ partial,
+                                                               int32_t* __restrict__ spread_counters) {
     constexpr int GPB = 256 / GS;
     constexpr bool COOP = GS == ACM_WINDOW && GPB == ACM_WINDOW;
     __shared__ float coop_lds[COOP ? ACM_WINDOW * NG * FP : 1];
@@ -462,6 +467,51 @@
         for (int c = 0; c < NG; ++c)
 #pragma unroll
             for (int f = 0; f < FP; ++f) acc[c][f] = acm_group_sum<GS>(acc[c][f]);
+        bool own = it.slot < 0;
+        if (SPREAD) {
+            static_assert(!SPREAD || GS == ACM_WINDOW, "the spread list is the sixteen-lane gather's");
+            own = own && it.row >= 0;
+            if (it.slot >= 0 && w / ACM_WINDOW >= csr.n_windows) {
+                const int li = csr.long_index[it.row];
+                const AcmLongRow lr = csr.long_rows[li];
+                const int pieces = lr.slot_end - lr.slot_begin;
+                if (gl == 0) {
+                    float* ps = partial + (long)it.slot * (NG * F);
+#pragma unroll
+                    for (int c = 0; c < NG; ++c)
+#pragma unroll
+                        for (int f = 0; f < FP; ++f)
+                            if (f < F) __hip_atomic_store(ps + c * F + f, acc[c][f], __ATOMIC_RELAXED, __HIP_MEMORY_SCOPE_AGENT);
+                }
+                __builtin_amdgcn_fence(__ATOMIC_RELEASE, "agent");
+                int old = 0;
+                if (gl == 0) old = __hip_atomic_fetch_add(spread_counters + li, 1, __ATOMIC_RELAXED, __HIP_MEMORY_SCOPE_AGENT);
+                old = acm_row_bcast(old, 0);
+                if (old == pieces - 1) {
+                    __builtin_amdgcn_fence(__ATOMIC_ACQUIRE, "agent");
+                    if (gl == 0) __hip_atomic_store(spread_counters + li, 0, __ATOMIC_RELAXED, __HIP_MEMORY_SCOPE_AGENT);
+                    const float* ps = partial + (long)(lr.slot_begin + (gl < pieces ? gl : 0)) * (NG * F);
+                    float mine[NG][FP];
+#pragma unroll
+                    for (int c = 0; c < NG; ++c)
+#pragma unroll
+                        for (int f = 0; f < FP; ++f) {
+                            mine[c][f] = f < F ? __hip_atomic_load(ps + c * F + f, __ATOMIC_RELAXED, __HIP_MEMORY_SCOPE_AGENT) : 0.f;
+                            acc[c][f] = 0.f;
+                        }
+                    const int first = (int)(threadIdx.x & 63u & ~15u);
+#pragma unroll 1
+                    for (int q = 0; q < pieces; ++q) {
+#pragma unroll
+                        for (int c = 0; c < NG; ++c)
+#pragma unroll
+                            for (int f = 0; f < FP; ++f)
+                                acc[c][f] += __int_as_float(__builtin_amdgcn_ds_bpermute((first + q) << 2, __float_as_int(mine[c][f])));
+                    }
+                    own = true;
+                }
+            }
+        }
         if (COOP && w / ACM_WINDOW < csr.n_windows) {
             const int g = threadIdx.x / GS;
             if (gl == 0) {
@@ -496,10 +546,10 @@
                 }
             }
             __syncthreads();
-        } else if (it.slot < 0) {
+        } else if (own) {
             LaySerial<FP> lay{gl == 0};
             Epi::template apply<LaySerial<FP>, NG>(ea, it.row, lay, F, acc);
-        } else if (gl == 0) {
+        } else if (!SPREAD && gl == 0) {
             float* ps = partial + (long)it.slot * (NG * F);
 #pragma unroll
             for (int c = 0; c < NG; ++c)
@@ -766,7 +816,7 @@
     float* partial = (float*)workspace;
     CsrView v = over ? over->view : acm_view(a);
     if (vals_override) v.vals = vals_override;
-    const int64_t n_items = v.n_items, n_long = v.n_long;
+    int64_t n_items = v.n_items, n_long = v.n_long;
     if (n_items == 0) return ACM_OK;
     ACM_REQUIRE(!bf16 || (F > 8 && F <= 64 && F % 2 == 0), ACM_EUNSUPPORTED,
                 "%s: bf16 gathered operands are implemented for even 8 < F <= 64", who);
@@ -781,6 +831,19 @@
     auto wide = [&](auto kernel) { hipLaunchKernelGGL(kernel, dim3((int)((n_items + 3) / 4)), dim3(256), 0, st, v, g, F, ea, partial); };
     if constexpr (epi_wide_only<Epi>::value)
         ACM_REQUIRE(F > 8, ACM_EUNSUPPORTED, "%s: this epilogue exists for more than 8 columns (got %d)", who, F);
+    AcmSpreadList* sp = nullptr;
+    if (form.kind == GatherForm::NARROW && form.lanes == ACM_WINDOW && acm_tuning().spread && NG * F <= ACM_SPREAD_SLOT_FLOATS) {
+        if (!over) sp = a->spread;
+        else if (a->loss_rows && over->view.items == a->loss_rows->items) sp = a->loss_rows->spread;
+    }
+    if (sp) {
+        v.items = sp->items, v.n_items = (int)sp->n_items;
+        v.long_rows = sp->long_rows, v.long_index = sp->long_index, v.n_long = (int)sp->n_long;
+        v.n_windows = (int)sp->n_windows, v.n_multi = (int)sp->n_multi;
+        n_items = sp->n_items, n_long = sp->n_long;
+        partial = sp->slots;
+        ++sp->launches;
+    }
     int rc = ACM_OK;
     switch (form.kind) {
     case GatherForm::PAIR3: {
@@ -799,12 +862,22 @@
             constexpr int FP = decltype(fp)::value, GS = decltype(gs)::value, gpb = 256 / GS;
             int grid = (int)((n_items + gpb - 1) / gpb);
             if (grid > NARROW_MAX_BLOCKS) grid = NARROW_MAX_BLOCKS;
+            int32_t* const none = nullptr;
+            if constexpr (GS == ACM_WINDOW) {
+                if (sp && form.merged)
+                    hipLaunchKernelGGL((spmm_narrow_kernel<FP, NG, GS, (NG >= 2), Epi, NARROW_SPREAD_U, true>), dim3(grid), dim3(256), 0, st, v,
+                                       g, F, form.vecmask, ea, partial, sp->counters);
+                else if (sp)
+                    hipLaunchKernelGGL((spmm_narrow_kernel<FP, NG, GS, false, Epi, NARROW_SPREAD_U, true>), dim3(grid), dim3(256), 0, st, v, g,
+                                       F, form.vecmask, ea, partial, sp->counters);
+                if (sp) return ACM_OK;
+            }
             if (form.merged)
                 hipLaunchKernelGGL((spmm_narrow_kernel<FP, NG, GS, (NG >= 2), Epi>), dim3(grid), dim3(256), 0, st, v, g, F,
-                                   form.vecmask, ea, partial);
+                                   form.vecmask, ea, partial, none);
             else
                 hipLaunchKernelGGL((spmm_narrow_kernel<FP, NG, GS, false, Epi>), dim3(grid), dim3(256), 0, st, v, g, F,
-                                   form.vecmask, ea, partial);
+                                   form.vecmask, ea, partial, none);
             return ACM_OK;
         }, acm_fp_of(F), acm_lanes_of(form.lanes));
         break;
diff --git a/acm_gnn_amd/csrc/acm_gcn.hip b/acm_gnn_amd/csrc/acm_gcn.hip
--- a/acm_gnn_amd/csrc/acm_gcn.hip
+++ b/acm_gnn_amd/csrc/acm_gcn.hip
@@ -230,7 +230,7 @@
             constexpr int FP = decltype(fp)::value, GS = decltype(gs)::value;
             if constexpr (!(FP == 8 && GS == 16))
                 hipLaunchKernelGGL((spmm_narrow_kernel<FP, 1, GS, false, EpiGcnBwd>), dim3(pl.grid), dim3(256), 0, s, v, g, F,
-                                   form.vecmask, ea, partial);
+                                   form.vecmask, ea, partial, (int32_t*)nullptr);
             return ACM_OK;
         }, acm_fp_of(F), acm_lanes_of(pl.gs));
         ACM_REQUIRE(rc == ACM_OK, ACM_EUNSUPPORTED, "acm_gcn_bwd: no narrow gather for %d lanes per item", pl.gs);
diff --git a/acm_gnn_amd/csrc/acm_items.h b/acm_gnn_amd/csrc/acm_items.h
--- a/acm_gnn_amd/csrc/acm_items.h
+++ b/acm_gnn_amd/csrc/acm_items.h
@@ -15,10 +15,12 @@
 
 inline void build_items(const std::vector<int32_t>& indptr, int chunk, std::vector<AcmItem>& items,
                         std::vector<AcmLongRow>& longs, int64_t& n_slots, int32_t& max_deg, int64_t& n_windows, int64_t& n_multi,
-                        const uint8_t* keep = nullptr) {
+                        const uint8_t* keep = nullptr, int64_t spread_bar = 0, int64_t* n_spread = nullptr) {
     const int64_t n = (int64_t)indptr.size() - 1;
     items.clear();
     longs.clear();
+    struct SpreadRow { int32_t row, deg, pieces; };
+    std::vector<SpreadRow> spread_rows;
     items.reserve(n + n / 8);
     n_slots = 0;
     max_deg = 0;
@@ -36,6 +38,10 @@
             pieces = windows * ACM_WINDOW;
         } else if (pieces > ACM_WINDOW) {
             pieces = ACM_WINDOW;
+        }
+        if (spread_bar > 0 && !windows && deg > spread_bar) {
+            spread_rows.push_back({(int32_t)r, deg, pieces});
+            continue;
         }
         const int32_t room = ACM_WINDOW - (int32_t)(items.size() % ACM_WINDOW);
         if ((room < pieces || windows) && room < ACM_WINDOW) {
@@ -59,8 +65,30 @@
         prev.slot_end = (int32_t)n_slots;
     }
     n_windows = (int64_t)items.size() / ACM_WINDOW;
-    for (int64_t r = 0; r < n; ++r)
-        if (indptr[r + 1] - indptr[r] <= chunk && !(keep && !keep[r])) items.push_back({(int32_t)r, indptr[r], indptr[r + 1], -1});
+    std::stable_sort(spread_rows.begin(), spread_rows.end(), [](const SpreadRow& x, const SpreadRow& y) { return x.deg > y.deg; });
+    std::vector<AcmItem> spread;
+    for (const SpreadRow& sr : spread_rows) {
+        const int32_t b = indptr[sr.row], e = indptr[sr.row + 1];
+        const int32_t per = (sr.deg + sr.pieces - 1) / sr.pieces;
+        AcmLongRow lr = {sr.row, (int32_t)n_slots, 0, 0};
+        for (int32_t q = 0; q < sr.pieces; ++q) {
+            const int32_t s = std::min(e, b + q * per);
+            spread.push_back({sr.row, s, std::min(e, s + per), (int32_t)n_slots++});
+        }
+        lr.slot_end = (int32_t)n_slots;
+        longs.push_back(lr);
+    }
+    if (n_spread) *n_spread = (int64_t)spread.size();
+    size_t next_piece = 0;
+    for (int64_t r = 0; r < n; ++r) {
+        if (indptr[r + 1] - indptr[r] > chunk || (keep && !keep[r])) continue;
+        if (next_piece < spread.size() && items.size() % ACM_WINDOW == 0) items.push_back(spread[next_piece++]);
+        items.push_back({(int32_t)r, indptr[r], indptr[r + 1], -1});
+    }
+    while (next_piece < spread.size()) {
+        while (items.size() % ACM_WINDOW) items.push_back({-1, 0, 0, -1});
+        items.push_back(spread[next_piece++]);
+    }
 }
 
 struct AcmLossRowsHost {
diff --git a/acm_gnn_amd/tuning.py b/acm_gnn_amd/tuning.py
--- a/acm_gnn_amd/tuning.py
+++ b/acm_gnn_amd/tuning.py
@@ -4,6 +4,8 @@
 import threading
 
 KERNEL_KEYS = ("chunk", "wide_form", "bwd_split", "rows16", "agg_fused", "gemm_forms")
+LIST_KEYS = ("spread",)
+ALL_KERNEL_KEYS = KERNEL_KEYS + LIST_KEYS
 HOST_DEFAULTS = {"rewrites": 15, "implicit": 1, "relabel": -1, "pipeline": 8192, "csr_features": 256, "small_step": 16384,
                  "mlp_stack": 1, "loss_rows": 1}
 HOST_RANGES = {"rewrites": (0, 15), "implicit": (0, 1), "relabel": (-1, 1), "pipeline": (0, 1 << 31), "csr_features": (0, 1 << 31),
@@ -18,7 +20,7 @@
 
 
 class Tuning(C.Structure):
-    _fields_ = [(k, C.c_int32) for k in KERNEL_KEYS] + [("reserved", C.c_int32 * 10)]
+    _fields_ = [(k, C.c_int32) for k in ALL_KERNEL_KEYS] + [("reserved", C.c_int32 * 9)]
 
 
 class _Host:
@@ -45,7 +47,7 @@
             v = int(val, 0)
         except ValueError:
             raise ValueError(f"ACM_TUNING: '{item}': the value must be an integer") from None
-        if key in KERNEL_KEYS:
+        if key in ALL_KERNEL_KEYS:
             kern[key] = v
         elif key in HOST_DEFAULTS:
             lo, hi = HOST_RANGES[key]
@@ -53,7 +55,7 @@
                 raise ValueError(f"ACM_TUNING: {key}={v} outside {lo}..{hi}")
             host[key] = v
         else:
-            raise ValueError(f"ACM_TUNING: unknown key '{key}' (known: {', '.join(KERNEL_KEYS + tuple(HOST_DEFAULTS))})")
+            raise ValueError(f"ACM_TUNING: unknown key '{key}' (known: {', '.join(ALL_KERNEL_KEYS + tuple(HOST_DEFAULTS))})")
     return kern, host
 
 
@@ -101,7 +103,7 @@
         from . import _lib
         t = Tuning()
         _lib.check(_lib.load().acm_tuning_get(C.byref(t)), "acm_tuning_get")
-        _kernel_cache = {k: int(getattr(t, k)) for k in KERNEL_KEYS}
+        _kernel_cache = {k: int(getattr(t, k)) for k in ALL_KERNEL_KEYS}
     return _kernel_cache
 
 
@@ -112,7 +114,7 @@
         _kernel_touched = True
         cur = dict(kernel())
         for k, v in kw.items():
-            if k not in KERNEL_KEYS:
+            if k not in ALL_KERNEL_KEYS:
                 raise KeyError(k)
             cur[k] = int(v)
         t = Tuning()
@@ -124,7 +126,7 @@
 
 def apply(**kw):
     host_kw = {k: v for k, v in kw.items() if k in HOST_DEFAULTS}
-    kern_kw = {k: v for k, v in kw.items() if k in KERNEL_KEYS}
+    kern_kw = {k: v for k, v in kw.items() if k in ALL_KERNEL_KEYS}
     unknown = set(kw) - set(host_kw) - set(kern_kw)
     if unknown:
         raise KeyError(f"unknown tuning switch(es): {sorted(unknown)}")
@@ -163,7 +165,7 @@
 @contextlib.contextmanager
 def override(**kw):
     host_kw = {k: v for k, v in kw.items() if k in HOST_DEFAULTS}
-    kern_kw = {k: v for k, v in kw.items() if k in KERNEL_KEYS}
+    kern_kw = {k: v for k, v in kw.items() if k in ALL_KERNEL_KEYS}
     unknown = set(kw) - set(host_kw) - set(kern_kw)
     if unknown:
         raise KeyError(f"unknown tuning switch(es): {sorted(unknown)}")
diff --git a/include/acm_hip.h b/include/acm_hip.h
--- a/include/acm_hip.h
+++ b/include/acm_hip.h
@@ -32,7 +32,8 @@
     int32_t rows16;
     int32_t agg_fused;
     int32_t gemm_forms;
-    int32_t reserved[10];
+    int32_t spread;
+    int32_t reserved[9];
 } acm_tuning_t;
 int acm_tuning_get(acm_tuning_t* out);
 int acm_tuning_set(const acm_tuning_t* in);
@@ -75,6 +76,8 @@
 
 int acm_csr_build_loss_rows(acm_csr_t* a, const uint8_t* keep_dev);
 int acm_csr_loss_rows_info(const acm_csr_t* a, int64_t* out);
+
+int acm_csr_spread_info(const acm_csr_t* a, int64_t* out);
 
 int acm_spmm_workspace_bytes(const acm_csr_t* a, int width, size_t* bytes);
 
```

After: 48.74 billion edges/s. -2.6%, worse.
